# HKUST-Aerial-Robotics/A-LOAM

Measured on AMD Instinct MI355X. Metric: HDL-64 scans/sec (whole node), higher is better.
Workload: dtype f32 features / f64 solve

## Files before the change

a-loam_amd/csrc/aloam_capi.hip:

```cpp
#include <algorithm>
#include <cstdio>
#include <cstdlib>
#include <cstring>

#include "capi_internal.hpp"

namespace aloam {

hipEvent_t prof_event(aloam_ctx* c) {
  if (!c->prof_free.empty()) { hipEvent_t e = c->prof_free.back(); c->prof_free.pop_back(); return e; }
  Event e;
  (void)hipEventCreate(&e.h);
  c->prof_events.push_back(std::move(e));
  return c->prof_events.back();
}

int stage_ints(aloam_ctx* c, const int* src, int n, int* dst) {
  const int ns = c->h_nin_slot;
  c->h_nin_slot = (ns + 1) % kNinSlots;
  int* slot = c->h_nin.get() + (size_t)ns * c->B;
  if (c->nin_used[ns]) HIP_TRY(c, hipEventSynchronize(c->nin_done[ns]));
  std::memcpy(slot, src, sizeof(int) * n);
  HIP_TRY(c, hipMemcpyAsync(dst, slot, sizeof(int) * n, hipMemcpyHostToDevice, c->stream));
  HIP_TRY(c, hipEventRecord(c->nin_done[ns], c->stream));
  c->nin_used[ns] = true;
  return ALOAM_OK;
}

int stage_mask(aloam_ctx* c, DevBuf<int>& dst, const int** out) {
  *out = nullptr;
  if (c->all_active) return ALOAM_OK;
  if (!dst && dmalloc(c, dst, c->B)) return ALOAM_E_HIP;
  if (const int rc = stage_ints(c, c->active.data(), c->B, dst.get())) return rc;
  *out = dst.get();
  return ALOAM_OK;
}

int check_seq(aloam_ctx* c, int seq) {
  if (!c) return ALOAM_E_ARG;
  if (seq < 0 || seq >= c->B) { c->err = "sequence index out of range"; return ALOAM_E_ARG; }
  return ALOAM_OK;
}

int require_stage(aloam_ctx* c, int stage) {
  if (c->stages & stage) return ALOAM_OK;
  c->err = std::string("this context was created without ") +
           (stage == ALOAM_STAGE_REGISTRATION ? "ALOAM_STAGE_REGISTRATION" : stage == ALOAM_STAGE_ODOMETRY ? "ALOAM_STAGE_ODOMETRY" : "ALOAM_STAGE_MAPPING");
  return ALOAM_E_STATE;
}

int check_ids(aloam_ctx* c, const int* ids, int n) {
  if (n < 0 || n > c->B || (n > 0 && !ids)) { c->err = "bad sequence list"; return ALOAM_E_ARG; }
  std::vector<char> seen(c->B, 0);
  for (int i = 0; i < n; ++i) {
    if (ids[i] < 0 || ids[i] >= c->B || seen[ids[i]]) { c->err = "sequence index out of range or repeated"; return ALOAM_E_ARG; }
    seen[ids[i]] = 1;
  }
  return ALOAM_OK;
}

int queue_reset(aloam_ctx* c, const int* seqs, int n) {
  if (n == 0) return ALOAM_OK;
  if (!c->d_reset_ids && dmalloc(c, c->d_reset_ids, c->B)) return ALOAM_E_HIP;
  if (const int rc = stage_ints(c, seqs, n, c->d_reset_ids.get())) return rc;
  ResetArgs r{};
  r.seqs = c->d_reset_ids.get(); r.n = n; r.R = c->R;
  r.meta = c->d_meta.get(); r.ringstart = c->d_ringstart.get(); r.state = c->d_state.get();
  r.edges = c->d_edges.get(); r.planes = c->d_planes.get();
  for (int k = 0; k < 2; ++k) r.grid_flags[k] = c->d_grid_flags[k].get();
  for (int k = 0; k < 2; ++k) { r.less_sharp[k] = c->d_less_sharp[k].get(); r.less_flat[k] = c->d_less_flat[k].get(); }
  r.cap = c->cap;
  if (c->map_on) { r.mapseq = c->d_mapseq.get(); r.cubes = c->d_cubes.get(); r.addcnt = c->d_addcnt.get(); r.live = c->d_map_live.get(); r.grid_sig = c->d_grid_sig.get(); }
  launch_reset_sequences(r, c->stream);
  HIP_TRY(c, hipGetLastError());
  for (int i = 0; i < n; ++i) { c->parity[seqs[i]] = 0; c->inited[seqs[i]] = 0; c->needs_odom[seqs[i]] = 0; c->map_err_seen[seqs[i]] = 0; clear_scorable(c, seqs[i]); place_sweep_dropped(c, seqs[i]); }
  for (int i = 0; i < n; ++i) if (const int rc = mark_window_stale(c, seqs[i])) return rc;
  return ALOAM_OK;
}

}

namespace {

void prof_resolve(aloam_ctx* c) {
  for (ProfRec& r : c->prof_pending) {
    float ms = 0.f;
    (void)hipEventSynchronize(r.e1);
    (void)hipEventElapsedTime(&ms, r.e0, r.e1);
    c->prof_ms[r.kernel] += ms;
    c->prof_launches[r.kernel] += 1;
    c->prof_free.push_back(r.e0);
    c->prof_free.push_back(r.e1);
  }
  c->prof_pending.clear();
}

}

extern "C" {

void aloam_default_config(aloam_config* cfg) {
  cfg->n_scans = 64;
  cfg->min_range = 5.0f;
  cfg->ring_from_field = 0;
  cfg->batch = 1;
  cfg->max_points = 140000;
  cfg->max_ring_points = 4107;
  cfg->device = 0;
  cfg->lm_max_iterations = 4;
  cfg->outer_iterations = 2;
  cfg->distortion = 0;
}

int aloam_create(const aloam_config* cfg, aloam_ctx** out) { return aloam_create_stages(cfg, ALOAM_STAGE_ALL, out); }

int aloam_create_stages(const aloam_config* cfg, int stages, aloam_ctx** out) {
  if (!cfg || !out) return ALOAM_E_ARG;
  *out = nullptr;
  aloam_ctx* c = new aloam_ctx();
  c->cfg = *cfg;
  c->stages = stages;
  { const char* e = std::getenv("ALOAM_DEBUG_SYNC"); c->debug_sync = e && e[0] == '1'; }
  *out = c;
  if ((stages & ~ALOAM_STAGE_ALL) || !(stages & ALOAM_STAGE_ALL)) { c->err = "stages must be a non-empty combination of ALOAM_STAGE_*"; return ALOAM_E_ARG; }
  if (cfg->batch < 1 || cfg->max_points < 32 || cfg->max_points > 400000 || cfg->lm_max_iterations < 0 || cfg->outer_iterations < 1 ||
      cfg->outer_iterations > 64) { c->err = "bad configuration value"; return ALOAM_E_ARG; }
  if (!cfg->ring_from_field && cfg->n_scans != 16 && cfg->n_scans != 32 && cfg->n_scans != 64) {
    c->err = "only support velodyne with 16, 32 or 64 scan line (or ring_from_field)";
    return ALOAM_E_SCAN_LINES;
  }
  if (cfg->n_scans < 1 || cfg->n_scans > kMaxRings) { c->err = "n_scans out of range"; return ALOAM_E_ARG; }
  if (cfg->max_ring_points < 17 || cfg->max_ring_points > 4107) { c->err = "max_ring_points must be in [17, 4107]"; return ALOAM_E_ARG; }
  int ndev = 0;
  if (hipGetDeviceCount(&ndev) != hipSuccess || ndev <= 0) { c->err = "no HIP device available (this library has no CPU fallback)"; return ALOAM_E_HIP; }
  if (cfg->device < 0 || cfg->device >= ndev) { c->err = "device ordinal out of range"; return ALOAM_E_ARG; }
  DeviceScope device_scope(c);
  HIP_TRY(c, hipStreamCreateWithFlags(&c->stream.h, hipStreamNonBlocking));
  HIP_TRY(c, hipStreamCreateWithFlags(&c->copy_stream.h, hipStreamNonBlocking));
  for (int k = 0; k < 2; ++k) {
    HIP_TRY(c, hipEventCreateWithFlags(&c->in_copied[k].h, hipEventDisableTiming));
    HIP_TRY(c, hipEventCreateWithFlags(&c->in_consumed[k].h, hipEventDisableTiming));
  }
  c->B = cfg->batch; c->max_points = cfg->max_points; c->R = cfg->n_scans;
  c->active.assign(c->B, 1); c->parity.assign(c->B, 0); c->inited.assign(c->B, 0); c->needs_odom.assign(c->B, 0); c->frozen.assign(c->B, 0); c->scorable.assign(c->B, 0); c->pl_has_sweep.assign(c->B, 0); c->pl_desc_valid.assign(c->B, 0);
  c->map_err_seen.assign(c->B, 0);
  c->cap = cfg->max_points + (((cfg->max_points / 32 + 15) & ~15) + 16);
  { const char* e = std::getenv("ALOAM_GRAPH_MAX_BATCH"); c->use_graph = c->B <= (e ? std::atoi(e) : 0); }
  c->NB = (c->cap + kBlockPts - 1) / kBlockPts;
  c->npad = cfg->max_ring_points <= 2059 ? 2048 : 4096;
  const size_t B = c->B, cap = c->cap, R = c->R, NB = c->NB;
  int rc = 0;
  { int* p = nullptr; HIP_TRY(c, hipHostMalloc((void**)&p, sizeof(int) * B * kNinSlots, hipHostMallocDefault)); c->h_nin.reset(p); }
  for (Event& e : c->nin_done) HIP_TRY(c, hipEventCreateWithFlags(&e.h, hipEventDisableTiming));
  const bool reg = stages & ALOAM_STAGE_REGISTRATION, odo = stages & ALOAM_STAGE_ODOMETRY, map = stages & ALOAM_STAGE_MAPPING;
  c->grid_H[0] = R > 64 ? 8192 : 4096;
  c->grid_H[1] = c->max_points > 160000 ? 32768 : 16384;
  if ((rc = dmalloc(c, c->d_nin, B))) return rc;
  if ((rc = dmalloc(c, c->d_meta, B))) return rc;
  if ((rc = dmalloc(c, c->d_state, B))) return rc;
  if ((rc = dmalloc(c, c->d_cloud, B * cap))) return rc;
  if ((rc = dmalloc(c, c->d_exp_cnt, B * ALOAM_EXPORT_MAX_IDS))) return rc;
  if ((rc = dmalloc(c, c->d_exp_chunk, B * ALOAM_EXPORT_MAX_IDS + 1))) return rc;
  if ((rc = dmalloc(c, c->d_exp_off, B * ALOAM_EXPORT_MAX_IDS + 1))) return rc;
  { int cus = 0; if (hipDeviceGetAttribute(&cus, hipDeviceAttributeMultiprocessorCount, cfg->device) == hipSuccess && cus > 0) c->gather_blocks = 8 * cus; }
  if (reg) {
    c->slab = c->npad + 16;
    if ((rc = dmalloc(c, c->d_slabs, B * R * (size_t)c->slab))) return rc;
    if ((rc = dmalloc(c, c->d_front_lb, B * NB * (size_t)kFrontSlots))) return rc;
    if ((rc = dmalloc(c, c->d_front_ticket, B))) return rc;
    if ((rc = dmalloc(c, c->d_ringstart, B * (R + 1)))) return rc;
    if ((rc = dmalloc(c, c->d_curv, B * cap))) return rc;
    if ((rc = dmalloc(c, c->d_label, B * cap))) return rc;
    if ((rc = dmalloc(c, c->d_lookback, B * 4 * R))) return rc;
    if ((rc = dmalloc(c, c->d_ring_ticket, B))) return rc;
  }
  if (reg || odo) {
    if ((rc = dmalloc(c, c->d_sharp, B * R * kSharpPerRing))) return rc;
    if ((rc = dmalloc(c, c->d_flat, B * R * kFlatPerRing))) return rc;
  }
  for (int k = 0; k < 2; ++k) {
    if (!(odo || (k == 0 && reg) || (k == 1 && map))) continue;
    if ((rc = dmalloc(c, c->d_less_sharp[k], B * R * kLessSharpPerRing))) return rc;
    if ((rc = dmalloc(c, c->d_less_flat[k], B * cap))) return rc;
  }
  if (odo) {
    for (int k = 0; k < 2; ++k) {
      const size_t per = k == 0 ? R * kLessSharpPerRing : cap;
      if ((rc = dmalloc(c, c->d_grid_sorted3[k], B * per))) return rc;
      if ((rc = dmalloc(c, c->d_grid_sorted2[k], B * per))) return rc;
      if ((rc = dmalloc(c, c->d_grid_start3[k], B * (c->grid_H[k] + 1)))) return rc;
      if ((rc = dmalloc(c, c->d_grid_start2[k], B * (c->grid_H[k] + 1)))) return rc;
      if ((rc = dmalloc(c, c->d_grid_sorted3c[k], B * per))) return rc;
      if ((rc = dmalloc(c, c->d_grid_start3c[k], B * (c->grid_H[k] + 1)))) return rc;
      if ((rc = dmalloc(c, c->d_grid_flags[k], B * 4))) return rc;
      if ((rc = dmalloc(c, c->d_grid_walk[k], B * 2 * (R + 8)))) return rc;
    }
    if ((rc = dmalloc(c, c->d_edges, B * R * kSharpPerRing))) return rc;
    if ((rc = dmalloc(c, c->d_planes, B * R * kFlatPerRing))) return rc;
    if ((rc = dmalloc(c, c->d_sel_sharp, B * R * kSharpPerRing))) return rc;
    if ((rc = dmalloc(c, c->d_sel_flat, B * R * kFlatPerRing))) return rc;
    if ((rc = prepare_build_grids(c->grid_H[1]))) { c->err = "k_build_grids: dynamic LDS size rejected"; return ALOAM_E_HIP; }
  }
  std::vector<OdomState> init(B);
  std::memset(init.data(), 0, sizeof(OdomState) * B);
  for (size_t b = 0; b < B; ++b) { init[b].para_q[3] = 1.0; init[b].q_w[3] = 1.0; }
  HIP_TRY(c, hipMemcpyAsync(c->d_state.get(), init.data(), sizeof(OdomState) * B, hipMemcpyHostToDevice, c->stream));
  HIP_TRY(c, hipStreamSynchronize(c->stream));
  return ALOAM_OK;
}

void aloam_destroy(aloam_ctx* c) {
  DeviceScope device_scope(c);
  if (!c) return;
  if (c->stream) (void)hipStreamSynchronize(c->stream);
  if (c->copy_stream) (void)hipStreamSynchronize(c->copy_stream);
  prof_resolve(c);
  delete c;
}

const char* aloam_last_error(const aloam_ctx* c) { return c ? c->err.c_str() : "null context"; }
void* aloam_stream(aloam_ctx* c) { return c ? (void*)c->stream : nullptr; }

int aloam_synchronize(aloam_ctx* c) {
  DeviceScope device_scope(c);
  if (!c) return ALOAM_E_ARG;
  HIP_TRY(c, hipStreamSynchronize(c->stream));
  std::vector<SeqMeta> m(c->B);
  HIP_TRY(c, hipMemcpy(m.data(), c->d_meta.get(), sizeof(SeqMeta) * c->B, hipMemcpyDeviceToHost));
  for (int b = 0; b < c->B; ++b) {
    if (m[b].err & kErrEmpty) { c->err = "sequence " + std::to_string(b) + ": no point survives the NaN / minimum-range filter"; return ALOAM_E_EMPTY; }
    if (m[b].err & (kErrRingCap | kErrPointCap)) { c->err = "sequence " + std::to_string(b) + ": a ring exceeds max_ring_points or the scan exceeds max_points"; return ALOAM_E_CAPACITY; }
    if (m[b].err & kErrInternal) { c->err = "sequence " + std::to_string(b) + ": internal error, a ring workgroup of k_ring_features never published its counts (look-back wait timed out)"; return ALOAM_E_HIP; }
  }
  if (c->map_on) {
    std::vector<MapSeq> ms(c->B);
    int vc[4] = {0, 0, 0, 0};
    HIP_TRY(c, hipMemcpy(ms.data(), c->d_mapseq.get(), sizeof(MapSeq) * c->B, hipMemcpyDeviceToHost));
    HIP_TRY(c, hipMemcpy(vc, c->d_vox_counters.get(), sizeof(vc), hipMemcpyDeviceToHost));
    long long fresh_pool = 0;
    int first_seq = -1;
    for (int b = 0; b < c->B; ++b) {
      const long long n = ms[b].err_steps + ((ms[b].err & kMapErrPool) ? 1 : 0);
      if (n > c->map_err_seen[b]) { fresh_pool += n - c->map_err_seen[b]; if (first_seq < 0) first_seq = b; }
      c->map_err_seen[b] = n;
    }
    const long long vox = vc[3] + (vc[1] ? 1 : 0), fresh_vox = vox > c->map_err_reported ? vox - c->map_err_reported : 0;
    c->map_err_reported = vox;
    if (fresh_pool + fresh_vox > 0) {
      c->err = "mapping, since the last aloam_synchronize:";
      if (fresh_pool) c->err += " " + std::to_string(fresh_pool) + " (sequence, step) pair(s) ran out of map pool (first: sequence " + std::to_string(first_seq) + ")";
      if (fresh_vox) c->err += std::string(fresh_pool ? " and" : "") + " " + std::to_string(fresh_vox) + " step(s) ran out of voxel-filter scratch";
      c->err += "; the points that did not fit were not inserted (raise pool_points)";
      return ALOAM_E_CAPACITY;
    }
    long long fresh_spill = 0;
    if (const int rc = spill_dropped_since(c, &fresh_spill)) return rc;
    if (fresh_spill > 0) {
      c->err = "map spill full: " + std::to_string(fresh_spill) + " tile(s) dropped since the last aloam_synchronize (drain more often or raise max_tiles / max_points)";
      return ALOAM_E_CAPACITY;
    }
    if (c->d_rl_bad) {
      int bad = 0;
      HIP_TRY(c, hipMemcpy(&bad, c->d_rl_bad.get(), sizeof(bad), hipMemcpyDeviceToHost));
      const long long fresh = bad - c->rl_bad_reported;
      c->rl_bad_reported = bad;
      if (fresh > 0) {
        c->err = "aloam_apply_map_corrections, since the last aloam_synchronize: " + std::to_string(fresh) + " choice(s) outside 0 .. K-1; those sequences were left untouched";
        return ALOAM_E_ARG;
      }
    }
  }
  return ALOAM_OK;
}

int aloam_set_active(aloam_ctx* c, const int* active) {
  DeviceScope device_scope(c);
  if (!c) return ALOAM_E_ARG;
  std::vector<int> m(c->B, 1);
  if (active) for (int b = 0; b < c->B; ++b) m[b] = active[b] != 0 ? 1 : 0;
  if (c->reg_pending && (c->stages & ALOAM_STAGE_REGISTRATION) && m != c->reg_active) {
    c->err = "the mask may not change between a registration and the odometry step that consumes it";
    return ALOAM_E_STATE;
  }
  c->all_active = std::find(m.begin(), m.end(), 0) == m.end();
  c->active = std::move(m);
  return ALOAM_OK;
}

int aloam_reset_sequences(aloam_ctx* c, const int* seqs, int n) {
  DeviceScope device_scope(c);
  if (!c) return ALOAM_E_ARG;
  if (const int rc = check_ids(c, seqs, n)) return rc;
  return queue_reset(c, seqs, n);
}

int aloam_profile_enable(aloam_ctx* c, int on) {
  DeviceScope device_scope(c);
  if (!c) return ALOAM_E_ARG;
  HIP_TRY(c, hipStreamSynchronize(c->stream));
  prof_resolve(c);
  if (on) { for (int k = 0; k < K_COUNT; ++k) { c->prof_ms[k] = 0; c->prof_launches[k] = 0; } }
  c->prof_on = on != 0;
  return ALOAM_OK;
}
int aloam_profile_kernel_count(void) { return K_COUNT; }
const char* aloam_profile_kernel_name(int k) { return (k >= 0 && k < K_COUNT) ? kKernelNames[k] : ""; }

int aloam_profile_get(aloam_ctx* c, int kernel, double* total_ms, long long* launches, double* algorithmic_bytes) {
  DeviceScope device_scope(c);
  if (!c || kernel < 0 || kernel >= K_COUNT) return ALOAM_E_ARG;
  HIP_TRY(c, hipStreamSynchronize(c->stream));
  prof_resolve(c);
  if (total_ms) *total_ms = c->prof_ms[kernel];
  if (launches) *launches = c->prof_launches[kernel];
  if (algorithmic_bytes && kernel == K_EXPORT) {
    long long total = 0;
    HIP_TRY(c, hipMemcpy(&total, c->d_exp_off.get() + c->exp_last_segs, sizeof(total), hipMemcpyDeviceToHost));
    *algorithmic_bytes = 32.0 * total + 16.0 * c->exp_last_segs;
  } else if (algorithmic_bytes && (kernel == K_SAVE || kernel == K_LOAD)) {
    long long units = 0;
    if (kernel == K_SAVE && c->d_ck_uoff) HIP_TRY(c, hipMemcpy(&units, c->d_ck_uoff.get() + c->ck_save_n, sizeof(units), hipMemcpyDeviceToHost));
    *algorithmic_bytes = 2.0 * (kernel == K_SAVE ? 16.0 * units : (double)c->ck_load_bytes);
  } else if (algorithmic_bytes) {
    std::vector<SeqMeta> m(c->B);
    HIP_TRY(c, hipMemcpy(m.data(), c->d_meta.get(), sizeof(SeqMeta) * c->B, hipMemcpyDeviceToHost));
    std::vector<MapSeq> ms(c->map_on ? c->B : 0);
    if (c->map_on) HIP_TRY(c, hipMemcpy(ms.data(), c->d_mapseq.get(), sizeof(MapSeq) * c->B, hipMemcpyDeviceToHost));
    double bytes = 0;
    for (int b = 0; b < c->B; ++b) {
      const double Nin = m[b].n_in, N = m[b].n_cloud, Fc = m[b].n_sharp, Lc = m[b].n_less_sharp, Fs = m[b].n_flat, Ls = m[b].n_less_flat;
      const double Lcl = m[b].n_corner_last, Lsl = m[b].n_surf_last;
      switch (kernel) {
        case K_FIND_ENDS: bytes += 2 * 256 * 16; break;
        case K_FRONT: bytes += 16 * Nin + 16 * N + 16.0 * (c->R + 1) * ((Nin + kBlockPts - 1) / kBlockPts); break;
        case K_RING_STARTS: bytes += 12.0 * c->R; break;
        case K_DENSE_CLOUD: bytes += 32 * N; break;
        case K_RING_FEATURES: bytes += 16 * N + (c->debug_arrays ? 5 * N : 0) + 16 * (Fc + Lc + Fs + Ls); break;
        case K_BUILD_GRIDS: bytes += 16 * (Lcl + Lsl) + 48 * (Lcl + Lsl) + 12.0 * (c->grid_H[0] + c->grid_H[1]); break;
        case K_TRANSFORM: bytes += 32 * (Fc + Fs); break;
        case K_ASSOC_CORNER: bytes += 16 * (Fc + Lcl) + 48 * Fc; break;
        case K_ASSOC_PLANE: bytes += 16 * (Fs + Lsl) + 64 * Fs; break;
        case K_SOLVE: bytes += 9.0 * (48 * Fc + 64 * Fs); break;
        default: break;
      }
      if (c->map_on && kernel >= K_MAP_BEGIN) {
        const double Sc = ms[b].n_stack[0], Ss = ms[b].n_stack[1], Mc = ms[b].from_total[0], Ms = ms[b].from_total[1];
        const double Fc = ms[b].factor_num[1][0], Fs = ms[b].factor_num[1][1];
        switch (kernel) {
          case K_MAP_BEGIN: bytes += 2.0 * kMapValidMax * sizeof(CubeDesc) + sizeof(MapSeq); break;
          case K_MAP_VOXEL_STACK: bytes += 16 * (Lcl + Lsl) + 16 * (Sc + Ss); break;
          case K_MAP_GRID: bytes += 32 * (Mc + Ms) + 16.0 * c->map.H; break;
          case K_MAP_ASSOC: bytes += 16 * (Sc + Ss) + 80 * (Sc + Ss) + sizeof(MapEdgeRec) * Sc + sizeof(MapNormRec) * Ss; break;
          case K_MAP_SOLVE: bytes += 9.0 * (sizeof(MapEdgeRec) * Fc + sizeof(MapNormRec) * Fs); break;
          case K_MAP_INSERT: bytes += 32 * (Sc + Ss); break;
          case K_MAP_VOXEL_CUBES: bytes += 32 * (Mc + Ms + Sc + Ss); break;
          case K_MAP_REGISTER: bytes += 32 * N; break;
          default: break;
        }
      }
    }
    if (c->map_on && kernel == K_SCORE) {
      bytes = 64.0 * c->rl_last_K + 32.0 * c->rl_last_seqs.size() * c->rl_last_K;
      for (const int b : c->rl_last_seqs) bytes += 16.0 * (ms[b].n_stack[0] + ms[b].n_stack[1]) + 16.0 * (ms[b].from_total[0] + ms[b].from_total[1]) + 8.0 * c->map.H;
    }
    if (kernel == K_APPLY) bytes = c->rl_apply_n * (4.0 + 4.0 + 64.0 + 56.0);
    *algorithmic_bytes = bytes;
  }
  return ALOAM_OK;
}

}
```

a-loam_amd/csrc/aloam_device.hpp:

```cpp
#pragma once
#include <hip/hip_runtime.h>
#include <stdint.h>
#include "aloam_atan.hpp"

namespace aloam {

constexpr int kFrontSlots = 128 + 8;
constexpr int kBlockPts = 1024;
constexpr int kMaxRings = 128;
constexpr int kSectors = 6;
constexpr int kSharpPerSector = 2;
constexpr int kLessSharpPerSector = 20;
constexpr int kFlatPerSector = 4;
constexpr int kSharpPerRing = kSectors * kSharpPerSector;
constexpr int kLessSharpPerRing = kSectors * kLessSharpPerSector;
constexpr int kFlatPerRing = kSectors * kFlatPerSector;
constexpr int kNnTile = 1024;

enum ErrBits { kErrEmpty = 1, kErrRingCap = 2, kErrPointCap = 4, kErrInternal = 8 };

struct alignas(16) SeqMeta {
  int n_in;
  int first_kept, last_kept;
  int half_idx;
  float start_ori, end_ori;
  int n_cloud;
  int err;
  int n_sharp, n_less_sharp, n_flat, n_less_flat;
  int n_corner_last, n_surf_last;
  int parity;
  int pad1;
};

struct alignas(16) OdomState {
  double para_q[4];
  double para_t[3];
  double q_w[4];
  double t_w[3];
  int corner_corr[2], plane_corr[2];
  int lm_iterations[2], lm_successful[2];
  double initial_cost[2], final_cost[2];
  int termination[2];
  int inited;
  int pad;
};

enum SeqBits { kSeqActive = 1, kSeqSolve = 2, kSeqMapGrow = 4 };
__device__ __forceinline__ bool seq_idle(const int* active, int b, int bit = kSeqActive) { return active && !(active[b] & bit); }

struct EdgeRec { float cp[3], a[3], b[3]; int valid; int pad[2]; };
struct PlaneRec { float cp[3], j[3], l[3], m[3]; int valid; int pad[3]; };

struct RegArgs {
  const char* in;
  long long seq_stride;
  int pt_stride;
  int B, cap, R, NB;
  int ring_from_field;
  float min_range;
  SeqMeta* meta;
  float4* slabs;
  int slab;
  unsigned long long* front_lb;
  int* front_ticket;
  int* ringstart;
  float4* cloud;
  float* curv;
  int8_t* label;
  unsigned long long* lookback;
  unsigned epoch;
  int* ring_ticket;
  int store_debug;
  float4* sharp;
  float4* less_sharp[2];
  float4* flat;
  float4* less_flat[2];
  const int* active;
};

struct OdomArgs {
  int B, cap, R;
  SeqMeta* meta;
  OdomState* state;
  const float4* sharp;
  const float4* flat;
  const float4* less_sharp[2];
  const float4* less_flat[2];
  const int* active;
  float4* grid_sorted3[2];
  float4* grid_sorted2[2];
  int* grid_start3[2];
  int* grid_start2[2];
  float4* grid_sorted3c[2];
  int* grid_start3c[2];
  int* grid_flags[2];
  int* grid_walk[2];
  int grid_H_corner, grid_H_surf;
  float4* sel_sharp;
  float4* sel_flat;
  EdgeRec* edges;
  PlaneRec* planes;
  int outer;
  int last_outer;
  int lm_max_iterations;
  int distortion;
};

template <typename T>
__device__ __forceinline__ T* row_of(T* const (&buf)[2], int k, int b, long long per) { return (k ? buf[1] : buf[0]) + b * per; }
__device__ __forceinline__ const float4* corner_last(const OdomArgs& a, int b, int parity) { return row_of(a.less_sharp, parity ^ 1, b, (long long)a.R * kLessSharpPerRing); }
__device__ __forceinline__ const float4* surf_last(const OdomArgs& a, int b, int parity) { return row_of(a.less_flat, parity ^ 1, b, (long long)a.cap); }

struct GridView {
  int H;
  float4 *sorted3, *sorted2, *sorted3c;
  int *start3, *start2, *start3c, *flags, *walk;
};
__device__ __forceinline__ GridView grid_view(const OdomArgs& a, int b, int which) {
  GridView g;
  g.H = which == 0 ? a.grid_H_corner : a.grid_H_surf;
  const long long per = which == 0 ? (long long)a.R * kLessSharpPerRing : (long long)a.cap;
  g.sorted3 = a.grid_sorted3[which] + b * per;
  g.sorted2 = a.grid_sorted2[which] + b * per;
  g.start3 = a.grid_start3[which] + (long long)b * (g.H + 1);
  g.start2 = a.grid_start2[which] + (long long)b * (g.H + 1);
  g.sorted3c = a.grid_sorted3c[which] + b * per;
  g.start3c = a.grid_start3c[which] + (long long)b * (g.H + 1);
  g.flags = a.grid_flags[which] + b * 4;
  g.walk = a.grid_walk[which] + (long long)b * 2 * (a.R + 8);
  return g;
}

__device__ __forceinline__ float4 load_point(const char* base, long long i, int stride) {
  const float* p = reinterpret_cast<const float*>(base + i * (long long)stride);
  if ((stride & 15) == 0) return *reinterpret_cast<const float4*>(p);
  if (stride == 12) return make_float4(p[0], p[1], p[2], 0.f);
  return make_float4(p[0], p[1], p[2], p[3]);
}

__device__ __forceinline__ bool point_kept(const float4& p, float thres) {
  if (!(isfinite(p.x) && isfinite(p.y) && isfinite(p.z))) return false;
  const float r2 = p.x * p.x + p.y * p.y + p.z * p.z;
  return !(r2 < thres * thres);
}

__device__ __forceinline__ double shfl_down_f64(double v, int d) {
  int lo = __double2loint(v), hi = __double2hiint(v);
  lo = __shfl_down(lo, d, 64);
  hi = __shfl_down(hi, d, 64);
  return __hiloint2double(hi, lo);
}

template <int D>
__device__ __forceinline__ unsigned xor_lane_u32(unsigned v, int lane) {
  if constexpr (D == 1) return (unsigned)__builtin_amdgcn_mov_dpp((int)v, 0xB1, 0xF, 0xF, true);
  else if constexpr (D == 2) return (unsigned)__builtin_amdgcn_mov_dpp((int)v, 0x4E, 0xF, 0xF, true);
  else {
    const unsigned up = (unsigned)__builtin_amdgcn_mov_dpp((int)v, 0x100 + D, 0xF, 0xF, true);
    const unsigned dn = (unsigned)__builtin_amdgcn_mov_dpp((int)v, 0x110 + D, 0xF, 0xF, true);
    return (lane & D) ? dn : up;
  }
}
template <int D, bool MAX>
__device__ __forceinline__ unsigned long long row_step_u64(unsigned long long v, int lane) {
  const unsigned lo = xor_lane_u32<D>((unsigned)v, lane), hi = xor_lane_u32<D>((unsigned)(v >> 32), lane);
  const unsigned long long o = ((unsigned long long)hi << 32) | lo;
  return MAX ? (o > v ? o : v) : (o < v ? o : v);
}
template <bool MAX>
__device__ __forceinline__ unsigned long long wave_extreme_u64(unsigned long long v, int lane) {
  v = row_step_u64<1, MAX>(v, lane);
  v = row_step_u64<2, MAX>(v, lane);
  v = row_step_u64<4, MAX>(v, lane);
  v = row_step_u64<8, MAX>(v, lane);
  unsigned long long best = MAX ? 0ull : ~0ull;
#pragma unroll
  for (int q = 0; q < 4; ++q) {
    const unsigned lo = (unsigned)__builtin_amdgcn_readlane((int)(unsigned)v, 16 * q), hi = (unsigned)__builtin_amdgcn_readlane((int)(unsigned)(v >> 32), 16 * q);
    const unsigned long long o = ((unsigned long long)hi << 32) | lo;
    best = MAX ? (o > best ? o : best) : (o < best ? o : best);
  }
  return best;
}

template <bool MAX>
__device__ __forceinline__ unsigned wave_reduce_u32(unsigned v) {
  constexpr int identity = MAX ? 0 : -1;
  auto op = [](unsigned a, unsigned b) { return MAX ? (a > b ? a : b) : (a < b ? a : b); };
  v = op(v, (unsigned)__builtin_amdgcn_update_dpp(identity, (int)v, 0x111, 0xF, 0xF, false));
  v = op(v, (unsigned)__builtin_amdgcn_update_dpp(identity, (int)v, 0x112, 0xF, 0xF, false));
  v = op(v, (unsigned)__builtin_amdgcn_update_dpp(identity, (int)v, 0x114, 0xF, 0xF, false));
  v = op(v, (unsigned)__builtin_amdgcn_update_dpp(identity, (int)v, 0x118, 0xF, 0xF, false));
  v = op(v, (unsigned)__builtin_amdgcn_update_dpp(identity, (int)v, 0x142, 0xA, 0xF, false));
  v = op(v, (unsigned)__builtin_amdgcn_update_dpp(identity, (int)v, 0x143, 0xC, 0xF, false));
  return (unsigned)__builtin_amdgcn_readlane((int)v, 63);
}
__device__ __forceinline__ unsigned long long wave_min_packed(unsigned long long v) {
  const unsigned hi = (unsigned)(v >> 32), lo = (unsigned)v;
  const unsigned mh = wave_reduce_u32<false>(hi);
  const unsigned long long tie = __ballot(hi == mh);
  unsigned ml;
  if (__popcll(tie) == 1) ml = (unsigned)__builtin_amdgcn_readlane((int)lo, __ffsll((long long)tie) - 1);
  else ml = wave_reduce_u32<false>(hi == mh ? lo : 0xffffffffu);
  return ((unsigned long long)mh << 32) | ml;
}

template <bool MAX>
__device__ __forceinline__ int wave_scan_i32(int v) {
  constexpr int identity = MAX ? (int)0x80000000 : 0;
  auto op = [](int a, int b) { return MAX ? (a > b ? a : b) : a + b; };
  v = op(v, __builtin_amdgcn_update_dpp(identity, v, 0x111, 0xF, 0xF, false));
  v = op(v, __builtin_amdgcn_update_dpp(identity, v, 0x112, 0xF, 0xF, false));
  v = op(v, __builtin_amdgcn_update_dpp(identity, v, 0x114, 0xF, 0xF, false));
  v = op(v, __builtin_amdgcn_update_dpp(identity, v, 0x118, 0xF, 0xF, false));
  v = op(v, __builtin_amdgcn_update_dpp(identity, v, 0x142, 0xA, 0xF, false));
  v = op(v, __builtin_amdgcn_update_dpp(identity, v, 0x143, 0xC, 0xF, false));
  return v;
}


__device__ __forceinline__ int pow2ceil(int v) { int p = 1; while (p < v) p <<= 1; return p; }
template <typename K>
__device__ __forceinline__ void bitonic_cx(K& a, K& b) {
  const K lo = a < b ? a : b, hi = a < b ? b : a;
  a = lo; b = hi;
}
template <bool FIRST, typename K>
__device__ __forceinline__ void bitonic_groups_of_eight(K* keys, int n, int tid) {
  constexpr K kInf = (K)~(K)0;
  for (int g = tid * 8; g < n; g += 2048) {
    K v[8];
#pragma unroll
    for (int u = 0; u < 8; ++u) v[u] = g + u < n ? keys[g + u] : kInf;
    if (FIRST) {
#pragma unroll
      for (int b = 0; b < 8; b += 2) bitonic_cx(v[b], v[b + 1]);
#pragma unroll
      for (int b = 0; b < 8; b += 4) { bitonic_cx(v[b], v[b + 3]); bitonic_cx(v[b + 1], v[b + 2]); }
#pragma unroll
      for (int b = 0; b < 8; b += 2) bitonic_cx(v[b], v[b + 1]);
#pragma unroll
      for (int o = 0; o < 4; ++o) bitonic_cx(v[o], v[7 - o]);
    } else {
#pragma unroll
      for (int o = 0; o < 4; ++o) bitonic_cx(v[o], v[o + 4]);
    }
#pragma unroll
    for (int b = 0; b < 8; b += 4) { bitonic_cx(v[b], v[b + 2]); bitonic_cx(v[b + 1], v[b + 3]); }
#pragma unroll
    for (int b = 0; b < 8; b += 2) bitonic_cx(v[b], v[b + 1]);
#pragma unroll
    for (int u = 0; u < 8; ++u) if (g + u < n) keys[g + u] = v[u];
  }
  __syncthreads();
}
template <typename K>
__device__ __forceinline__ void bitonic_sort_keys(K* keys, int n, int tid) {
  const int npad = pow2ceil(n);
  bitonic_groups_of_eight<true, K>(keys, n, tid);
  for (int k = 16; k <= npad; k <<= 1) {
    const int hk = k >> 1;
    for (int t = tid; t < (npad >> 1); t += 256) {
      const int base = (t / hk) * k, off = t & (hk - 1);
      const int i = base + off, l = base + (k - 1 - off);
      if (l < n) {
        const K x = keys[i], y = keys[l];
        if (x > y) { keys[i] = y; keys[l] = x; }
      }
    }
    __syncthreads();
    for (int j = k >> 2; j > 4; j >>= 1) {
      for (int t = tid; t < (npad >> 1); t += 256) {
        const int i = ((t & ~(j - 1)) << 1) | (t & (j - 1));
        const int l = i + j;
        if (l < n) {
          const K x = keys[i], y = keys[l];
          if (x > y) { keys[i] = y; keys[l] = x; }
        }
      }
      __syncthreads();
    }
    bitonic_groups_of_eight<false, K>(keys, n, tid);
  }
}
__device__ __forceinline__ void bitonic_sort_u64(unsigned long long* keys, int n, int tid) { bitonic_sort_keys<unsigned long long>(keys, n, tid); }


}
```

a-loam_amd/csrc/capi_internal.hpp:

```cpp
#pragma once
#include <hip/hip_runtime.h>

#include <cstdio>
#include <memory>
#include <string>
#include <utility>
#include <vector>

#include "../../include/aloam_mi355x.h"
#include "aloam_device.hpp"
#include "atlas_kernels.hpp"
#include "checkpoint_kernels.hpp"
#include "export_kernels.hpp"
#include "mapping_kernels.hpp"
#include "odometry_kernels.hpp"
#include "places_kernels.hpp"
#include "registration_kernels.hpp"
#include "relocalize_kernels.hpp"

using namespace aloam;

namespace aloam {
enum KernelId { K_FIND_ENDS = 0, K_FRONT, K_RING_STARTS, K_DENSE_CLOUD, K_RING_FEATURES, K_BUILD_GRIDS, K_TRANSFORM, K_ASSOC_CORNER,
                K_ASSOC_PLANE, K_SOLVE, K_ADVANCE, K_MAP_BEGIN, K_MAP_VOXEL_STACK, K_MAP_GRID, K_MAP_ASSOC, K_MAP_SOLVE, K_MAP_INSERT,
                K_MAP_VOXEL_CUBES, K_MAP_REGISTER, K_EXPORT, K_SAVE, K_LOAD, K_SCORE, K_APPLY, K_COUNT };
const char* const kKernelNames[] = {"k_find_ends", "k_front", "k_ring_starts", "k_dense_cloud", "k_ring_features",
                                    "k_build_grids", "k_transform_queries", "k_associate[corner]", "k_associate[plane]",
                                    "k_solve", "k_advance", "map_begin", "map_voxel[stacks]", "map_grid", "map_associate", "map_solve",
                                    "map_insert", "map_voxel[cubes]", "map_register", "export_clouds", "save_sequences",
                                    "load_sequences", "score_corrections", "apply_corrections"};
static_assert(sizeof(kKernelNames) / sizeof(kKernelNames[0]) == K_COUNT, "one name per KernelId, in the same order");
struct ProfRec { int kernel; hipEvent_t e0, e1; };
constexpr int kNinSlots = 8;

struct DeviceFree { void operator()(void* p) const { (void)hipFree(p); } };
struct PinnedFree { void operator()(const volatile void* p) const { (void)hipHostFree(const_cast<void*>(p)); } };
template <typename T> using DevBuf = std::unique_ptr<T[], DeviceFree>;
template <typename T> using PinnedBuf = std::unique_ptr<T[], PinnedFree>;
template <typename H, hipError_t (*Destroy)(H)>
struct Handle {
  H h = nullptr;
  Handle() = default;
  Handle(Handle&& o) noexcept : h(std::exchange(o.h, nullptr)) {}
  ~Handle() { reset(); }
  void reset() { if (h) (void)Destroy(h); h = nullptr; }
  operator H() const { return h; }
};
using Stream = Handle<hipStream_t, hipStreamDestroy>;
using Event = Handle<hipEvent_t, hipEventDestroy>;
using GraphExec = Handle<hipGraphExec_t, hipGraphExecDestroy>;

template <typename T>
hipError_t dalloc(DevBuf<T>& p, size_t count) {
  T* raw = nullptr;
  const hipError_t e = hipMalloc((void**)&raw, count * sizeof(T));
  p.reset(raw);
  return e;
}

struct MapPool {
  int points = 0, H = 0;
  int cube_levels = 0, tile_cap = 0, tile_bound = 0;
  long long key_cap = 0;
  DevBuf<float4> pool[2], grid_sorted[2], voxtmp;
  DevBuf<int> grid_start[2], tile_seg, tile_heads, tile_pref;
  DevBuf<unsigned long long> keys[2];
};
}

struct aloam_ctx {
  Stream stream, copy_stream;
  Event in_copied[2], in_consumed[2], nin_done[kNinSlots], map_step_done[4];
  std::vector<Event> prof_events;
  GraphExec odom_graph[2];
  aloam_config cfg{};
  int stages = ALOAM_STAGE_ALL;
  int B = 0, cap = 0, R = 0, NB = 0, npad = 0;
  int max_points = 0;
  std::string err;
  DevBuf<char> d_in[2]; size_t d_in_bytes[2] = {0, 0};
  int in_slot = 0;
  bool in_used[2] = {false, false};
  DevBuf<int> d_nin;
  PinnedBuf<int> h_nin; int h_nin_slot = 0;
  bool nin_used[kNinSlots] = {};
  std::vector<int> active;
  bool all_active = true;
  std::vector<int> reg_active;
  bool reg_pending = false;
  const int* reg_mask = nullptr;
  std::vector<int> parity, inited;
  std::vector<char> needs_odom;
  std::vector<char> frozen;
  bool any_frozen = false;
  DevBuf<int> d_mask_reg, d_mask_odo, d_mask_map, d_reset_ids;
  DevBuf<SeqMeta> d_meta;
  DevBuf<float4> d_slabs; int slab = 0;
  DevBuf<unsigned long long> d_front_lb; DevBuf<int> d_front_ticket;
  bool dense_valid = true;
  DevBuf<int> d_ringstart;
  DevBuf<float4> d_cloud; DevBuf<float> d_curv; DevBuf<int8_t> d_label;
  DevBuf<unsigned long long> d_lookback; unsigned reg_epoch = 0;
  DevBuf<int> d_ring_ticket;
  bool debug_arrays = false;
  DevBuf<float4> d_sharp, d_flat;
  DevBuf<float4> d_less_sharp[2], d_less_flat[2];
  DevBuf<OdomState> d_state;
  DevBuf<float4> d_grid_sorted3[2], d_grid_sorted2[2];
  DevBuf<int> d_grid_start3[2], d_grid_start2[2];
  DevBuf<float4> d_grid_sorted3c[2];
  DevBuf<int> d_grid_start3c[2];
  DevBuf<int> d_grid_flags[2], d_grid_walk[2];
  int grid_H[2] = {4096, 16384};
  DevBuf<EdgeRec> d_edges; DevBuf<PlaneRec> d_planes;
  DevBuf<float4> d_sel_sharp, d_sel_flat;
  bool map_on = false;
  long long map_err_reported = 0;
  std::vector<long long> map_err_seen;
  float map_line_res = 0.4f, map_plane_res = 0.8f;
  int map_levels = 0, map_stack_tile_bound = 0, map_nsegs_max = 0;
  MapPool map;
  int map_pool_limit = 1 << 26;
  int map_growths = 0;
  long long map_steps = 0;
  int nin_max = 0;
  int inject_max = 0;
  PinnedBuf<volatile int> h_map_report;
  int* d_map_report_host = nullptr;
  DevBuf<int> d_map_report, d_map_live;
  DevBuf<MapSeq> d_mapseq; DevBuf<CubeDesc> d_cubes; DevBuf<int> d_maptab;
  DevBuf<MapGridSig> d_grid_sig;
  DevBuf<float4> d_stack[2], d_stack_world[2]; DevBuf<int> d_stack_cube[2];
  DevBuf<int> d_addcnt, d_cursor, d_compact_flag;
  DevBuf<MapEdgeRec> d_medges; DevBuf<MapNormRec> d_mnorms; DevBuf<float4> d_registered, d_knn;
  DevBuf<int> d_vox_lists;
  DevBuf<int> d_rec_tiles; int rec_tiles_corner = 0, rec_tiles_per_seq = 0;
  DevBuf<VoxSeg> d_segs; DevBuf<int> d_vox_counters, d_bbox;
  DevBuf<int> d_exp_cnt, d_exp_chunk; DevBuf<long long> d_exp_off;
  DevBuf<int> d_exp_pref[2];
  int exp_last_segs = 0;
  int gather_blocks = 2048;
  DevBuf<float4> d_exp_tmp; long long exp_tmp_cap = 0;
  DevBuf<long long> d_exp_tmp_off;
  DevBuf<int> d_ck_seqs, d_ck_info, d_ck_units, d_ck_chunk, d_ck_pref; DevBuf<long long> d_ck_uoff;
  PinnedBuf<char> h_ck; char* d_ck_host = nullptr;
  DevBuf<char> d_ck_load;
  DevBuf<char> d_ck_stage; size_t ck_stage_bytes = 0;
  int ck_save_n = 0; long long ck_load_bytes = 0;
  std::vector<char> scorable;
  DevBuf<int> d_rl_seqs, d_rl_bad;
  DevBuf<ScorePartial> d_rl_part; long long rl_part_cap = 0;
  DevBuf<aloam_map_correction> d_rl_cand; long long rl_cand_cap = 0;
  long long rl_bad_reported = 0;
  std::vector<int> rl_last_seqs; int rl_last_K = 0;
  int rl_apply_n = 0;
  bool spill_on = false;
  int spill_max_tiles = 0, spill_max_points = 0;
  DevBuf<aloam_map_tile> d_sp_tiles; DevBuf<float4> d_sp_points;
  DevBuf<int> d_sp_counters;
  DevBuf<int> d_sp_seqs, d_sp_cnt, d_sp_chunk; DevBuf<long long> d_sp_off;
  bool atlas_on = false;
  std::vector<char> attached; bool any_attached = false;
  DevBuf<int> d_at_attached, d_at_stale;
  DevBuf<AtlasEntry> d_at_dir[2]; int at_dir_mask[2] = {0, 0};
  DevBuf<float4> d_at_points[2];
  long long at_info[12] = {0};
  long long spill_dropped_reported = 0;
  bool places_on = false;
  int pl_capacity = 0, pl_count = 0;
  float pl_max_range = 80.f, pl_height = 2.f;
  std::vector<char> pl_has_sweep, pl_desc_valid;
  DevBuf<PlaceDesc> d_pl_desc;
  DevBuf<aloam_place> d_pl_store;
  DevBuf<float> d_pl_unit; DevBuf<unsigned long long> d_pl_masks;
  DevBuf<int> d_pl_seqs, d_pl_wanted, d_pl_lo, d_pl_hi;
  DevBuf<int2> d_pl_pairs; long long pl_pairs_cap = 0;
  int sum_order = 0;
  bool use_graph = false;
  bool have_features = false;
  bool prof_on = false;
  bool debug_sync = false;
  std::vector<ProfRec> prof_pending;
  std::vector<hipEvent_t> prof_free;
  double prof_ms[K_COUNT] = {0};
  long long prof_launches[K_COUNT] = {0};
};

#define HIP_TRY(ctx, expr)                                                                                   \
  do {                                                                                                       \
    hipError_t e__ = (expr);                                                                                 \
    if (e__ != hipSuccess) {                                                                                 \
      (ctx)->err = std::string(#expr) + ": " + hipGetErrorString(e__);                                       \
      return ALOAM_E_HIP;                                                                                    \
    }                                                                                                        \
  } while (0)

namespace aloam {

template <typename T>
int dmalloc(aloam_ctx* c, DevBuf<T>& p, size_t count) {
  HIP_TRY(c, dalloc(p, count));
  HIP_TRY(c, hipMemsetAsync(p.get(), 0, count * sizeof(T), c->stream));
  return ALOAM_OK;
}

hipEvent_t prof_event(aloam_ctx* c);
struct ProfScope {
  aloam_ctx* c; int k; hipEvent_t e0 = nullptr;
  ProfScope(aloam_ctx* c_, int k_) : c(c_), k(k_) {
    if (c->prof_on) { e0 = prof_event(c); (void)hipEventRecord(e0, c->stream); }
  }
  ~ProfScope() {
    if (c->prof_on) { hipEvent_t e1 = prof_event(c); (void)hipEventRecord(e1, c->stream); c->prof_pending.push_back({k, e0, e1}); }
    if (c->debug_sync) {
      const hipError_t e = hipStreamSynchronize(c->stream);
      std::fprintf(stderr, "[aloam] %-22s %s\n", kKernelNames[k], e == hipSuccess ? "ok" : hipGetErrorString(e));
    }
  }
};
struct DeviceScope {
  int prev = -1;
  explicit DeviceScope(const aloam_ctx* c) {
    int cur = -1;
    if (c && hipGetDevice(&cur) == hipSuccess && cur != c->cfg.device && hipSetDevice(c->cfg.device) == hipSuccess) prev = cur;
  }
  ~DeviceScope() { if (prev >= 0) (void)hipSetDevice(prev); }
  DeviceScope(const DeviceScope&) = delete;
  DeviceScope& operator=(const DeviceScope&) = delete;
};

template <typename T>
int read_seq(aloam_ctx* c, const T* dev, T* out) {
  HIP_TRY(c, hipStreamSynchronize(c->stream));
  HIP_TRY(c, hipMemcpy(out, dev, sizeof(T), hipMemcpyDeviceToHost));
  return ALOAM_OK;
}

template <typename T, typename Edit>
int edit_seq(aloam_ctx* c, T* dev, Edit edit) {
  T v;
  if (const int rc = read_seq(c, dev, &v)) return rc;
  edit(v);
  HIP_TRY(c, hipMemcpy(dev, &v, sizeof(T), hipMemcpyHostToDevice));
  return ALOAM_OK;
}

template <typename T, typename N>
int grow_scratch(aloam_ctx* c, DevBuf<T>& p, N& have, N need) {
  if (have >= need) return ALOAM_OK;
  have = 0;
  p.reset();
  HIP_TRY(c, dalloc(p, (size_t)need));
  have = need;
  return ALOAM_OK;
}

inline float4* cloud_row(const aloam_ctx* c, const ExportSrc& s, int seq) {
  const int r = s.sel == kSelFixed ? 0 : s.sel == kSelCurrent ? c->parity[seq] : 1 - c->parity[seq];
  return s.base[r] ? const_cast<float4*>(s.base[r]) + (size_t)seq * s.stride : nullptr;
}

int stage_ints(aloam_ctx* c, const int* src, int n, int* dst);
int stage_mask(aloam_ctx* c, DevBuf<int>& dst, const int** out);
int check_seq(aloam_ctx* c, int seq);
int require_stage(aloam_ctx* c, int stage);
int check_ids(aloam_ctx* c, const int* ids, int n);
int queue_reset(aloam_ctx* c, const int* seqs, int n);
int ensure_dense(aloam_ctx* c);
long long cloud_desc(const aloam_ctx* c, int id, ExportSrc* s);
int find_cloud(aloam_ctx* c, int seq, int id, const float4** ptr, int* n);
inline void clear_scorable(aloam_ctx* c, int seq) { c->scorable[seq] = 0; }
int grow_map_pool(aloam_ctx* c, long long want, bool clamp);
void queue_map_spill(aloam_ctx* c, const int* mask);
int spill_dropped_since(aloam_ctx* c, long long* fresh);
int mark_window_stale(aloam_ctx* c, int seq);
int atlas_step_check(aloam_ctx* c);
bool queue_atlas_window(aloam_ctx* c, const int* mask);
inline void place_sweep_registered(aloam_ctx* c, int seq) { c->pl_has_sweep[seq] = 1; c->pl_desc_valid[seq] = 0; }
inline void place_sweep_dropped(aloam_ctx* c, int seq) { c->pl_has_sweep[seq] = 0; c->pl_desc_valid[seq] = 0; }
VoxArgs vox_args(aloam_ctx* c, int n_segs, int levels);
enum CallerMem { kMemPageable, kMemDevice, kMemPinned, kMemManaged, kMemOtherDevice };
CallerMem classify_pointer(const aloam_ctx* c, const void* p, void** dev);
int export_target(aloam_ctx* c, const void* p, size_t align, const char* what, void** out);
int get_cube_list(aloam_ctx* c, int seq, int which, float* out, int cap_points);

}
```

a-loam_amd/csrc/capi_odometry.hip:

```cpp
#include <algorithm>
#include <cstring>

#include "capi_internal.hpp"

namespace {

RegArgs reg_args(aloam_ctx* c, const void* d_scans, long long seq_stride, int pt_stride) {
  RegArgs a{};
  a.in = (const char*)d_scans; a.seq_stride = seq_stride; a.pt_stride = pt_stride;
  a.B = c->B; a.cap = c->cap; a.R = c->R; a.NB = c->NB;
  a.ring_from_field = c->cfg.ring_from_field; a.min_range = c->cfg.min_range;
  a.meta = c->d_meta.get(); a.slabs = c->d_slabs.get(); a.slab = c->slab; a.front_lb = c->d_front_lb.get(); a.front_ticket = c->d_front_ticket.get();
  a.ringstart = c->d_ringstart.get(); a.cloud = c->d_cloud.get(); a.curv = c->d_curv.get(); a.label = c->d_label.get();
  a.lookback = c->d_lookback.get(); a.epoch = c->reg_epoch; a.store_debug = c->debug_arrays ? 1 : 0; a.ring_ticket = c->d_ring_ticket.get();
  a.sharp = c->d_sharp.get(); a.flat = c->d_flat.get();
  for (int k = 0; k < 2; ++k) { a.less_sharp[k] = c->d_less_sharp[k].get(); a.less_flat[k] = c->d_less_flat[k].get(); }
  a.active = c->reg_mask;
  return a;
}

OdomArgs odom_args(aloam_ctx* c) {
  OdomArgs a{};
  a.B = c->B; a.cap = c->cap; a.R = c->R;
  a.meta = c->d_meta.get(); a.state = c->d_state.get();
  a.sharp = c->d_sharp.get(); a.flat = c->d_flat.get();
  for (int k = 0; k < 2; ++k) { a.less_sharp[k] = c->d_less_sharp[k].get(); a.less_flat[k] = c->d_less_flat[k].get(); }
  for (int k = 0; k < 2; ++k) {
    a.grid_sorted3[k] = c->d_grid_sorted3[k].get(); a.grid_sorted2[k] = c->d_grid_sorted2[k].get(); a.grid_start3[k] = c->d_grid_start3[k].get();
    a.grid_sorted3c[k] = c->d_grid_sorted3c[k].get(); a.grid_start3c[k] = c->d_grid_start3c[k].get();
    a.grid_start2[k] = c->d_grid_start2[k].get();
    a.grid_flags[k] = c->d_grid_flags[k].get(); a.grid_walk[k] = c->d_grid_walk[k].get();
  }
  a.grid_H_corner = c->grid_H[0]; a.grid_H_surf = c->grid_H[1];
  a.edges = c->d_edges.get(); a.planes = c->d_planes.get();
  a.sel_sharp = c->d_sel_sharp.get(); a.sel_flat = c->d_sel_flat.get();
  a.lm_max_iterations = c->cfg.lm_max_iterations;
  a.distortion = c->cfg.distortion != 0;
  return a;
}

int check_batch(aloam_ctx* c, const int* n_in, int stride_bytes) {
  if (const int rc = require_stage(c, ALOAM_STAGE_REGISTRATION)) return rc;
  if (stride_bytes < 12 || (stride_bytes & 3)) { c->err = "stride_bytes must be 12 (x, y, z only) or >= 16, and a multiple of 4"; return ALOAM_E_ARG; }
  if (stride_bytes == 12 && c->cfg.ring_from_field) { c->err = "ring_from_field needs the 4th float of every record: stride_bytes >= 16"; return ALOAM_E_ARG; }
  for (int b = 0; b < c->B; ++b) {
    if (n_in[b] < 0) { c->err = "negative point count"; return ALOAM_E_ARG; }
    if (n_in[b] > c->max_points) { c->err = "scan exceeds max_points"; return ALOAM_E_CAPACITY; }
  }
  return ALOAM_OK;
}

int register_launch(aloam_ctx* c, const void* d_scans, long long seq_stride, const int* n_in, int stride_bytes, int slot = -1, bool debug_arrays = true) {
  int rc = ALOAM_OK;
  if (!c->all_active && (rc = ensure_dense(c))) return rc;
  c->nin_max = 0;
  for (int b = 0; b < c->B; ++b) if (c->all_active || c->active[b]) c->nin_max = std::max(c->nin_max, n_in[b]);
  if ((rc = stage_ints(c, n_in, c->B, c->d_nin.get()))) return rc;
  if ((rc = stage_mask(c, c->d_mask_reg, &c->reg_mask))) return rc;
  if (c->stages & ALOAM_STAGE_ODOMETRY) { c->reg_active = c->active; c->reg_pending = true; }
  c->debug_arrays = debug_arrays || c->sum_order != 0;
  if (((++c->reg_epoch) & 0x7fffffffu) == 0) ++c->reg_epoch;
  const RegArgs a = reg_args(c, d_scans, seq_stride, stride_bytes);
  { ProfScope p(c, K_FIND_ENDS); launch_find_ends(a, c->d_nin.get(), c->stream); }
  { ProfScope p(c, K_FRONT); launch_front(a, c->stream); }
  { ProfScope p(c, K_RING_STARTS); launch_ring_starts(a, c->stream); }
  c->dense_valid = false;
  for (int b = 0; b < c->B; ++b) if (c->all_active || c->active[b]) place_sweep_registered(c, b);
  if (slot >= 0) { HIP_TRY(c, hipEventRecord(c->in_consumed[slot], c->stream)); c->in_used[slot] = true; }
  { ProfScope p(c, K_RING_FEATURES); launch_ring_features(a, c->npad, 0.2f, c->stream);
    if (c->sum_order) launch_less_flat_reference_order(reg_args(c, d_scans, seq_stride, stride_bytes), c->npad, 0.2f, c->stream); }
  HIP_TRY(c, hipGetLastError());
  c->have_features = true;
  return ALOAM_OK;
}

}

namespace aloam {

int ensure_dense(aloam_ctx* c) {
  if (c->dense_valid) return ALOAM_OK;
  { ProfScope p(c, K_DENSE_CLOUD); launch_dense_cloud(reg_args(c, nullptr, 0, 16), c->stream); }
  HIP_TRY(c, hipGetLastError());
  c->dense_valid = true;
  return ALOAM_OK;
}

long long cloud_desc(const aloam_ctx* c, int id, ExportSrc* s) {
  const int* meta = reinterpret_cast<const int*>(c->d_meta.get());
  const int* mseq = reinterpret_cast<const int*>(c->d_mapseq.get());
  const int meta_ints = sizeof(SeqMeta) / sizeof(int), map_ints = sizeof(MapSeq) / sizeof(int);
  const long long sharp = (long long)c->R * kSharpPerRing, flat = (long long)c->R * kFlatPerRing, feat = (long long)c->R * kLessSharpPerRing;
  const long long cap = c->cap, pts = c->max_points;
  long long capacity = 0;
  auto set = [&](const float4* b0, const float4* b1, long long stride, long long row_cap, const int* count, int count_stride, int sel) {
    *s = ExportSrc{{b0, b1}, stride, count, count_stride, sel, kExportPlain, 0};
    capacity = row_cap;
  };
#define META_FIELD(f) (meta + offsetof(SeqMeta, f) / sizeof(int)), meta_ints
  switch (id) {
    case ALOAM_CLOUD_FULL: set(c->d_cloud.get(), nullptr, cap, pts, META_FIELD(n_cloud), kSelFixed); break;
    case ALOAM_CLOUD_SHARP: set(c->d_sharp.get(), nullptr, sharp, sharp, META_FIELD(n_sharp), kSelFixed); break;
    case ALOAM_CLOUD_FLAT: set(c->d_flat.get(), nullptr, flat, flat, META_FIELD(n_flat), kSelFixed); break;
    case ALOAM_CLOUD_LESS_SHARP: set(c->d_less_sharp[0].get(), c->d_less_sharp[1].get(), feat, feat, META_FIELD(n_less_sharp), kSelCurrent); break;
    case ALOAM_CLOUD_LESS_FLAT: set(c->d_less_flat[0].get(), c->d_less_flat[1].get(), cap, pts, META_FIELD(n_less_flat), kSelCurrent); break;
    case ALOAM_CLOUD_CORNER_LAST: set(c->d_less_sharp[0].get(), c->d_less_sharp[1].get(), feat, feat, META_FIELD(n_corner_last), kSelLast); break;
    case ALOAM_CLOUD_SURF_LAST: set(c->d_less_flat[0].get(), c->d_less_flat[1].get(), cap, pts, META_FIELD(n_surf_last), kSelLast); break;
    case ALOAM_EXPORT_MAP + ALOAM_MAP_REGISTERED: set(c->d_registered.get(), nullptr, cap, pts, META_FIELD(n_cloud), kSelFixed); break;
    case ALOAM_EXPORT_MAP + ALOAM_MAP_CORNER_STACK: set(c->d_stack[0].get(), nullptr, feat, feat, mseq + offsetof(MapSeq, n_stack) / sizeof(int), map_ints, kSelFixed); break;
    case ALOAM_EXPORT_MAP + ALOAM_MAP_SURF_STACK: set(c->d_stack[1].get(), nullptr, cap, pts, mseq + offsetof(MapSeq, n_stack) / sizeof(int) + 1, map_ints, kSelFixed); break;
    default: break;
  }
#undef META_FIELD
  return capacity;
}

int find_cloud(aloam_ctx* c, int seq, int id, const float4** ptr, int* n) {
  int rc = check_seq(c, seq);
  if (rc || (id == ALOAM_CLOUD_FULL && (rc = ensure_dense(c)))) return rc;
  ExportSrc s;
  if (!cloud_desc(c, id, &s)) { c->err = "unknown cloud id"; return ALOAM_E_ARG; }
  if ((rc = read_seq(c, s.count + (size_t)seq * s.count_stride, n))) return rc;
  if (!(*ptr = cloud_row(c, s, seq))) { c->err = "this context holds no such cloud (see aloam_create_stages)"; return ALOAM_E_STATE; }
  return ALOAM_OK;
}

}

extern "C" {

int aloam_scan_register_device(aloam_ctx* c, const void* d_scans, long long seq_stride_bytes, const int* n_in, int stride_bytes) {
  DeviceScope device_scope(c);
  if (!c || !d_scans || !n_in) return ALOAM_E_ARG;
  if (const int rc = check_batch(c, n_in, stride_bytes)) return rc;
  return register_launch(c, d_scans, seq_stride_bytes, n_in, stride_bytes);
}

static int acquire_slab(aloam_ctx* c, size_t need, int* slot_out) {
  const int s = c->in_slot;
  c->in_slot ^= 1;
  if (c->in_used[s]) HIP_TRY(c, hipEventSynchronize(c->in_consumed[s]));
  if (const int rc = grow_scratch(c, c->d_in[s], c->d_in_bytes[s], need)) return rc;
  *slot_out = s;
  return ALOAM_OK;
}

int aloam_scan_register(aloam_ctx* c, const void* const* scans, const int* n_in, int stride_bytes) {
  DeviceScope device_scope(c);
  if (!c || !scans || !n_in) return ALOAM_E_ARG;
  int rc = check_batch(c, n_in, stride_bytes);
  if (rc) return rc;
  const size_t seq_stride = (size_t)c->cap * stride_bytes;
  int slot = 0;
  if ((rc = acquire_slab(c, seq_stride * c->B, &slot))) return rc;
  char* d_in = c->d_in[slot].get();
  for (int b = 0; b < c->B; ++b)
    if (n_in[b] > 0) HIP_TRY(c, hipMemcpyAsync(d_in + b * seq_stride, scans[b], (size_t)n_in[b] * stride_bytes, hipMemcpyHostToDevice, c->stream));
  if ((rc = register_launch(c, d_in, (long long)seq_stride, n_in, stride_bytes, slot))) return rc;
  HIP_TRY(c, hipStreamSynchronize(c->stream));
  return ALOAM_OK;
}

static int stage_and_register(aloam_ctx* c, const void* h_scans, long long seq_stride_bytes, const int* n_in, int stride_bytes, bool debug_arrays) {
  if (!c || !h_scans || !n_in) return ALOAM_E_ARG;
  int rc = check_batch(c, n_in, stride_bytes);
  if (rc) return rc;
  if (seq_stride_bytes < 0) { c->err = "bad stride"; return ALOAM_E_ARG; }
  const size_t row = (size_t)*std::max_element(n_in, n_in + c->B) * stride_bytes;
  if (c->B > 1 && (size_t)seq_stride_bytes < row) { c->err = "seq_stride_bytes smaller than a scan"; return ALOAM_E_ARG; }
  const size_t d_seq_stride = (size_t)c->cap * stride_bytes;
  int slot = 0;
  if ((rc = acquire_slab(c, d_seq_stride * c->B, &slot))) return rc;
  char* d_in = c->d_in[slot].get();
  if (row > 0) {
    if (c->B > 1) HIP_TRY(c, hipMemcpy2DAsync(d_in, d_seq_stride, h_scans, (size_t)seq_stride_bytes, row, (size_t)c->B - 1, hipMemcpyHostToDevice, c->copy_stream));
    const size_t last = (size_t)n_in[c->B - 1] * stride_bytes;
    if (last > 0) HIP_TRY(c, hipMemcpyAsync(d_in + (size_t)(c->B - 1) * d_seq_stride, (const char*)h_scans + (size_t)(c->B - 1) * (size_t)seq_stride_bytes, last, hipMemcpyHostToDevice, c->copy_stream));
  }
  HIP_TRY(c, hipEventRecord(c->in_copied[slot], c->copy_stream));
  HIP_TRY(c, hipStreamWaitEvent(c->stream, c->in_copied[slot], 0));
  return register_launch(c, d_in, (long long)d_seq_stride, n_in, stride_bytes, slot, debug_arrays);
}

int aloam_scan_register_host(aloam_ctx* c, const void* h_scans, long long seq_stride_bytes, const int* n_in, int stride_bytes) {
  DeviceScope device_scope(c);
  return stage_and_register(c, h_scans, seq_stride_bytes, n_in, stride_bytes, true);
}

int aloam_process_host(aloam_ctx* c, const void* h_scans, long long seq_stride_bytes, const int* n_in, int stride_bytes) {
  DeviceScope device_scope(c);
  const int rc = stage_and_register(c, h_scans, seq_stride_bytes, n_in, stride_bytes, false);
  if (rc) return rc;
  return aloam_odometry_step(c);
}

int aloam_input_consumed(aloam_ctx* c) {
  DeviceScope device_scope(c);
  if (!c) return ALOAM_E_ARG;
  for (int s = 0; s < 2; ++s) if (c->in_used[s]) HIP_TRY(c, hipEventSynchronize(c->in_consumed[s]));
  return ALOAM_OK;
}

int aloam_odometry_step(aloam_ctx* c) {
  DeviceScope device_scope(c);
  if (!c) return ALOAM_E_ARG;
  if (const int rc = require_stage(c, ALOAM_STAGE_ODOMETRY)) return rc;
  if (!c->have_features) { c->err = "aloam_odometry_step before any features were registered / set"; return ALOAM_E_STATE; }
  std::vector<int> bits(c->B);
  bool any_solve = false, all_solve = true;
  for (int b = 0; b < c->B; ++b) {
    const bool on = c->all_active || c->active[b];
    bits[b] = on ? (kSeqActive | (c->inited[b] ? kSeqSolve : 0)) : 0;
    any_solve |= (bits[b] & kSeqSolve) != 0;
    all_solve &= (bits[b] & kSeqSolve) != 0;
  }
  const int* mask = nullptr;
  if (!all_solve && (any_solve || !c->all_active)) {
    if (!c->d_mask_odo && dmalloc(c, c->d_mask_odo, c->B)) return ALOAM_E_HIP;
    if (const int rc = stage_ints(c, bits.data(), c->B, c->d_mask_odo.get())) return rc;
    mask = c->d_mask_odo.get();
  }
  auto launch_all = [&]() {
    OdomArgs a = odom_args(c);
    a.active = mask;
    { ProfScope p(c, K_BUILD_GRIDS); launch_build_grids(a, c->stream); }
    for (int outer = 0; outer < c->cfg.outer_iterations; ++outer) {
      a.outer = outer;
      a.last_outer = outer == c->cfg.outer_iterations - 1;
      { ProfScope p(c, K_TRANSFORM); launch_transform_queries(a, c->stream); }
      { ProfScope p(c, K_ASSOC_CORNER); launch_associate(a, false, c->stream); }
      { ProfScope p(c, K_ASSOC_PLANE); launch_associate(a, true, c->stream); }
      { ProfScope p(c, K_SOLVE); launch_solve(a, c->stream); }
    }
    { ProfScope p(c, K_ADVANCE); launch_advance(a, c->stream); }
  };
  if (!any_solve) {
    OdomArgs a = odom_args(c);
    a.active = mask;
    { ProfScope p(c, K_ADVANCE); launch_advance(a, c->stream); }
  } else if (c->use_graph && !c->prof_on && !c->debug_sync) {
    GraphExec& ge = c->odom_graph[mask ? 1 : 0];
    if (!ge) {
      hipGraph_t g = nullptr;
      hipError_t e = hipStreamBeginCapture(c->stream, hipStreamCaptureModeThreadLocal);
      if (e == hipSuccess) {
        launch_all();
        e = hipStreamEndCapture(c->stream, &g);
        if (e == hipSuccess) e = hipGraphInstantiate(&ge.h, g, nullptr, nullptr, 0);
        if (g) (void)hipGraphDestroy(g);
      }
      if (e != hipSuccess) {
        (void)hipGetLastError();
        ge.reset();
        c->use_graph = false;
      }
    }
    if (ge) HIP_TRY(c, hipGraphLaunch(ge, c->stream));
    else launch_all();
  } else {
    launch_all();
  }
  HIP_TRY(c, hipGetLastError());
  for (int b = 0; b < c->B; ++b) if (bits[b] & kSeqActive) { c->parity[b] ^= 1; c->inited[b] = 1; c->needs_odom[b] = 0; }
  c->reg_pending = false;
  return ALOAM_OK;
}

int aloam_process_device(aloam_ctx* c, const void* d_scans, long long seq_stride_bytes, const int* n_in, int stride_bytes) {
  DeviceScope device_scope(c);
  if (!c || !d_scans || !n_in) return ALOAM_E_ARG;
  int rc = check_batch(c, n_in, stride_bytes);
  if (rc || (rc = register_launch(c, d_scans, seq_stride_bytes, n_in, stride_bytes, -1, false))) return rc;
  return aloam_odometry_step(c);
}

int aloam_cloud_size(aloam_ctx* c, int seq, int which) {
  DeviceScope device_scope(c);
  const float4* p; int n;
  const int rc = find_cloud(c, seq, which < ALOAM_EXPORT_MAP ? which : -1, &p, &n);
  return rc ? rc : n;
}

int aloam_get_cloud(aloam_ctx* c, int seq, int which, float* out, int cap_points) {
  DeviceScope device_scope(c);
  const float4* p; int n;
  if (const int rc = find_cloud(c, seq, which < ALOAM_EXPORT_MAP ? which : -1, &p, &n)) return rc;
  const int k = n < cap_points ? n : cap_points;
  if (k > 0) HIP_TRY(c, hipMemcpy(out, p, sizeof(float4) * k, hipMemcpyDeviceToHost));
  return n;
}

int aloam_get_pose(aloam_ctx* c, int seq, double q_w[4], double t_w[3], double q_lc[4], double t_lc[3]) {
  DeviceScope device_scope(c);
  int rc = check_seq(c, seq);
  if (rc) return rc;
  OdomState s;
  if ((rc = read_seq(c, c->d_state.get() + seq, &s))) return rc;
  for (int k = 0; k < 4; ++k) { q_w[k] = s.q_w[k]; q_lc[k] = s.para_q[k]; }
  for (int k = 0; k < 3; ++k) { t_w[k] = s.t_w[k]; t_lc[k] = s.para_t[k]; }
  return ALOAM_OK;
}

int aloam_get_odom_stats(aloam_ctx* c, int seq, aloam_odom_stats* out) {
  DeviceScope device_scope(c);
  int rc = check_seq(c, seq);
  if (rc) return rc;
  OdomState s;
  if ((rc = read_seq(c, c->d_state.get() + seq, &s))) return rc;
  for (int k = 0; k < 2; ++k) {
    out->corner_corr[k] = s.corner_corr[k]; out->plane_corr[k] = s.plane_corr[k];
    out->lm_iterations[k] = s.lm_iterations[k]; out->lm_successful[k] = s.lm_successful[k];
    out->initial_cost[k] = s.initial_cost[k]; out->final_cost[k] = s.final_cost[k]; out->termination[k] = s.termination[k];
  }
  return ALOAM_OK;
}

int aloam_set_features(aloam_ctx* c, int seq, const float* sharp, int n_sharp, const float* less_sharp, int n_less_sharp,
                       const float* flat, int n_flat, const float* less_flat, int n_less_flat) {
  DeviceScope device_scope(c);
  int rc = check_seq(c, seq);
  if (rc) return rc;
  struct { int id, n; const float* pts; ExportSrc s; } in[4] = {
      {ALOAM_CLOUD_SHARP, n_sharp, sharp}, {ALOAM_CLOUD_LESS_SHARP, n_less_sharp, less_sharp}, {ALOAM_CLOUD_FLAT, n_flat, flat}, {ALOAM_CLOUD_LESS_FLAT, n_less_flat, less_flat}};
  for (auto& x : in) if (x.n < 0 || x.n > cloud_desc(c, x.id, &x.s)) { c->err = "feature cloud larger than the selection rules allow"; return ALOAM_E_CAPACITY; }
  for (auto& x : in) if (!cloud_row(c, x.s, seq)) { c->err = "this context has no feature buffers (created for the mapping stage only)"; return ALOAM_E_STATE; }
  c->inject_max = std::max(c->inject_max, std::max(n_less_sharp, n_less_flat));
  HIP_TRY(c, hipStreamSynchronize(c->stream));
  for (auto& x : in) if (x.n) HIP_TRY(c, hipMemcpy(cloud_row(c, x.s, seq), x.pts, sizeof(float4) * x.n, hipMemcpyHostToDevice));
  if ((rc = edit_seq(c, c->d_meta.get() + seq, [&](SeqMeta& m) { m.n_sharp = n_sharp; m.n_less_sharp = n_less_sharp; m.n_flat = n_flat; m.n_less_flat = n_less_flat; m.err = 0; }))) return rc;
  c->have_features = true;
  return ALOAM_OK;
}

int aloam_set_last(aloam_ctx* c, int seq, const float* corner_last, int n_corner, const float* surf_last, int n_surf) {
  DeviceScope device_scope(c);
  int rc = check_seq(c, seq);
  if (rc) return rc;
  struct { int id, n; const float* pts; ExportSrc s; } in[2] = {{ALOAM_CLOUD_CORNER_LAST, n_corner, corner_last}, {ALOAM_CLOUD_SURF_LAST, n_surf, surf_last}};
  for (auto& x : in) if (x.n < 0 || x.n > cloud_desc(c, x.id, &x.s)) { c->err = "last cloud too large"; return ALOAM_E_CAPACITY; }
  for (auto& x : in) if (!cloud_row(c, x.s, seq)) { c->err = "this context has no buffers for the last clouds (created for the registration stage only)"; return ALOAM_E_STATE; }
  c->inject_max = std::max(c->inject_max, std::max(n_corner, n_surf));
  HIP_TRY(c, hipStreamSynchronize(c->stream));
  for (auto& x : in) if (x.n) HIP_TRY(c, hipMemcpy(cloud_row(c, x.s, seq), x.pts, sizeof(float4) * x.n, hipMemcpyHostToDevice));
  return edit_seq(c, c->d_meta.get() + seq, [&](SeqMeta& m) { m.n_corner_last = n_corner; m.n_surf_last = n_surf; });
}

int aloam_set_state(aloam_ctx* c, int seq, const double para_q[4], const double para_t[3], const double q_w[4], const double t_w[3]) {
  DeviceScope device_scope(c);
  int rc = check_seq(c, seq);
  if (rc) return rc;
  return edit_seq(c, c->d_state.get() + seq, [&](OdomState& s) {
    for (int k = 0; k < 4; ++k) { s.para_q[k] = para_q[k]; s.q_w[k] = q_w[k]; }
    for (int k = 0; k < 3; ++k) { s.para_t[k] = para_t[k]; s.t_w[k] = t_w[k]; }
  });
}

int aloam_set_system_inited(aloam_ctx* c, int inited) {
  DeviceScope device_scope(c);
  if (!c) return ALOAM_E_ARG;
  std::fill(c->inited.begin(), c->inited.end(), inited != 0 ? 1 : 0);
  launch_set_inited(c->d_state.get(), c->B, inited != 0 ? 1 : 0, c->stream);
  HIP_TRY(c, hipGetLastError());
  return ALOAM_OK;
}

int aloam_set_full_cloud(aloam_ctx* c, int seq, const float* cloud, int n) {
  DeviceScope device_scope(c);
  int rc = check_seq(c, seq);
  if (rc) return rc;
  ExportSrc s;
  if (n < 0 || n > cloud_desc(c, ALOAM_CLOUD_FULL, &s)) { c->err = "cloud too large"; return ALOAM_E_CAPACITY; }
  if ((rc = ensure_dense(c))) return rc;
  HIP_TRY(c, hipStreamSynchronize(c->stream));
  if (n) HIP_TRY(c, hipMemcpy(cloud_row(c, s, seq), cloud, sizeof(float4) * n, hipMemcpyHostToDevice));
  return edit_seq(c, c->d_meta.get() + seq, [&](SeqMeta& m) { m.n_cloud = n; });
}

int aloam_get_ring_ranges(aloam_ctx* c, int seq, int* start, int* count) {
  DeviceScope device_scope(c);
  int rc = check_seq(c, seq);
  if (rc) return rc;
  if ((rc = require_stage(c, ALOAM_STAGE_REGISTRATION))) return rc;
  HIP_TRY(c, hipStreamSynchronize(c->stream));
  std::vector<int> rs(c->R + 1);
  HIP_TRY(c, hipMemcpy(rs.data(), c->d_ringstart.get() + (size_t)seq * (c->R + 1), sizeof(int) * (c->R + 1), hipMemcpyDeviceToHost));
  for (int r = 0; r < c->R; ++r) { start[r] = rs[r]; count[r] = rs[r + 1] - rs[r]; }
  return c->R;
}

int aloam_get_curvature(aloam_ctx* c, int seq, float* out, int cap) {
  DeviceScope device_scope(c);
  int rc = check_seq(c, seq);
  if (rc) return rc;
  if ((rc = require_stage(c, ALOAM_STAGE_REGISTRATION))) return rc;
  if (!c->debug_arrays) { c->err = "curvature is only kept by aloam_scan_register*; the throughput entries (aloam_process_*) skip it"; return ALOAM_E_STATE; }
  SeqMeta m;
  if ((rc = read_seq(c, c->d_meta.get() + seq, &m))) return rc;
  const int k = m.n_cloud < cap ? m.n_cloud : cap;
  if (k > 0) HIP_TRY(c, hipMemcpy(out, c->d_curv.get() + (size_t)seq * c->cap, sizeof(float) * k, hipMemcpyDeviceToHost));
  return m.n_cloud;
}

int aloam_get_labels(aloam_ctx* c, int seq, int* out, int cap) {
  DeviceScope device_scope(c);
  int rc = check_seq(c, seq);
  if (rc) return rc;
  if ((rc = require_stage(c, ALOAM_STAGE_REGISTRATION))) return rc;
  if (!c->debug_arrays) { c->err = "labels are only kept by aloam_scan_register*; the throughput entries (aloam_process_*) skip them"; return ALOAM_E_STATE; }
  SeqMeta m;
  if ((rc = read_seq(c, c->d_meta.get() + seq, &m))) return rc;
  const int k = m.n_cloud < cap ? m.n_cloud : cap;
  std::vector<int8_t> tmp(k > 0 ? k : 1);
  if (k > 0) HIP_TRY(c, hipMemcpy(tmp.data(), c->d_label.get() + (size_t)seq * c->cap, k, hipMemcpyDeviceToHost));
  for (int i = 0; i < k; ++i) out[i] = tmp[i];
  return m.n_cloud;
}

int aloam_get_last_cloud_order(aloam_ctx* c, int seq, int out[2]) {
  DeviceScope device_scope(c);
  int rc = check_seq(c, seq);
  if (rc) return rc;
  if (!c->d_grid_flags[0]) { c->err = "this context has no odometry stage"; return ALOAM_E_STATE; }
  HIP_TRY(c, hipStreamSynchronize(c->stream));
  for (int k = 0; k < 2; ++k) {
    int f[4];
    HIP_TRY(c, hipMemcpy(f, c->d_grid_flags[k].get() + (size_t)seq * 4, sizeof(f), hipMemcpyDeviceToHost));
    out[k] = f[0] ? -1 : f[1];
  }
  return ALOAM_OK;
}

int aloam_get_correspondences(aloam_ctx* c, int seq, float* edges, int cap_edges, int* n_edges, int* edge_query,
                              float* planes, int cap_planes, int* n_planes, int* plane_query) {
  DeviceScope device_scope(c);
  int rc = check_seq(c, seq);
  if (rc) return rc;
  SeqMeta m;
  if ((rc = read_seq(c, c->d_meta.get() + seq, &m))) return rc;
  std::vector<EdgeRec> E(m.n_sharp > 0 ? m.n_sharp : 1);
  std::vector<PlaneRec> P(m.n_flat > 0 ? m.n_flat : 1);
  if (m.n_sharp > 0) HIP_TRY(c, hipMemcpy(E.data(), c->d_edges.get() + (size_t)seq * c->R * kSharpPerRing, sizeof(EdgeRec) * m.n_sharp, hipMemcpyDeviceToHost));
  if (m.n_flat > 0) HIP_TRY(c, hipMemcpy(P.data(), c->d_planes.get() + (size_t)seq * c->R * kFlatPerRing, sizeof(PlaneRec) * m.n_flat, hipMemcpyDeviceToHost));
  int ne = 0, np = 0;
  for (int i = 0; i < m.n_sharp; ++i) {
    if (!E[i].valid) continue;
    if (ne < cap_edges) {
      float* o = edges + (size_t)ne * 9;
      for (int k = 0; k < 3; ++k) { o[k] = E[i].cp[k]; o[3 + k] = E[i].a[k]; o[6 + k] = E[i].b[k]; }
      if (edge_query) edge_query[ne] = i;
    }
    ++ne;
  }
  for (int i = 0; i < m.n_flat; ++i) {
    if (!P[i].valid) continue;
    if (np < cap_planes) {
      float* o = planes + (size_t)np * 12;
      for (int k = 0; k < 3; ++k) { o[k] = P[i].cp[k]; o[3 + k] = P[i].j[k]; o[6 + k] = P[i].l[k]; o[9 + k] = P[i].m[k]; }
      if (plane_query) plane_query[np] = i;
    }
    ++np;
  }
  *n_edges = ne;
  *n_planes = np;
  return ALOAM_OK;
}

}
```

a-loam_amd/csrc/mapping_kernels.hip:

```cpp
#include "mapping_kernels.hpp"

#include "lm_device.hpp"
#include "map_search_device.hpp"
#include "map_window_device.hpp"

namespace aloam {

namespace {

__device__ __forceinline__ int f2o(float f) { const int i = __float_as_int(f); return i >= 0 ? i : i ^ 0x7fffffff; }
__device__ __forceinline__ float o2f(int i) { return __int_as_float(i >= 0 ? i : i ^ 0x7fffffff); }

__device__ __forceinline__ float4 submap_point(const MapArgs& a, int b, int cls, const int* tab, int n_valid, int g) {
  const int* pref = tab + 80 + cls * 80;
  int lo = 0, hi = n_valid - 1;
  while (lo < hi) { const int mid = (lo + hi + 1) >> 1; if (pref[mid] <= g) lo = mid; else hi = mid - 1; }
  const CubeDesc d = cube_table(a, b, cls)[tab[lo]];
  return a.pool[cls][(long long)b * a.pool_cap + d.off + (g - pref[lo])];
}

}

__device__ __forceinline__ int compact_cap(int n, int mode) { return n <= 0 ? 0 : (mode == 1 ? n + n / 2 + 64 : n); }

// ... 1044 lines not shown
    return (lo << 8) + (d - pre[lo]);
  };
  for (int d0 = tid; d0 < n0; d0 += U * kMapSolveThreads) {
    MapEdgeRec e[U];
#pragma unroll
    for (int u = 0; u < U; ++u) { const int d = d0 + u * kMapSolveThreads; e[u] = E[locate(pre0, nt0, d < n0 ? d : d0)]; }
#pragma unroll
    for (int u = 0; u < U; ++u) if (d0 + u * kMapSolveThreads < n0) edge_term(e[u]);
  }
  auto norm_term = [&](const MapNormRec& p) {
    ++np;
    double rcp[3];
    quat_rotate(q, p.cp[0], p.cp[1], p.cp[2], rcp);
    const double r = (p.n[0] * (rcp[0] + t[0]) + p.n[1] * (rcp[1] + t[1]) + p.n[2] * (rcp[2] + t[2])) + p.d;
    double rho0, rho1;
    huber(r * r, &rho0, &rho1);
    acc[27] += 0.5 * rho0;
    if (WITH_JAC) {
      const double J[6] = {2.0 * (p.n[2] * rcp[1] - p.n[1] * rcp[2]), 2.0 * (p.n[0] * rcp[2] - p.n[2] * rcp[0]), 2.0 * (p.n[1] * rcp[0] - p.n[0] * rcp[1]),
                           p.n[0], p.n[1], p.n[2]};
      add_row(acc, J, r, rho1);
    }
  };
  for (int d0 = tid; d0 < n1; d0 += U * kMapSolveThreads) {
    MapNormRec pr[U];
#pragma unroll
    for (int u = 0; u < U; ++u) { const int d = d0 + u * kMapSolveThreads; pr[u] = P[locate(pre1, nt1, d < n1 ? d : d0)]; }
#pragma unroll
    for (int u = 0; u < U; ++u) if (d0 + u * kMapSolveThreads < n1) norm_term(pr[u]);
  }
  *n_edge = ne;
  *n_norm = np;
}

__global__ __launch_bounds__(kMapSolveThreads) void k_map_solve(MapArgs a, int iter, int last) {
  const int b = blockIdx.x, tid = threadIdx.x;
  __shared__ double s_red[(kMapSolveThreads / 64) * 28];
  extern __shared__ int s_pref[];
  if (seq_idle(a.active, b)) return;
  MapSeq& ms = a.seq[b];
  {
    const int nt0 = (ms.n_stack[0] + 255) >> 8, nt1 = (ms.n_stack[1] + 255) >> 8;
    const int* tc = a.rec_tiles + (long long)b * a.rec_tiles_per_seq;
    if (tid == 0) {
      int run = 0;
      for (int k = 0; k < nt0; ++k) { s_pref[k] = run; run += ms.gate ? tc[k] : 0; }
      s_pref[nt0] = run;
      run = 0;
      for (int k = 0; k < nt1; ++k) { s_pref[nt0 + 1 + k] = run; run += ms.gate ? tc[a.rec_tiles_corner + k] : 0; }
      s_pref[nt0 + 1 + nt1] = run;
    }
    __syncthreads();
  }
  double q[4] = {ms.par[0], ms.par[1], ms.par[2], ms.par[3]};
  double t[3] = {ms.par[4], ms.par[5], ms.par[6]};
  const LmResult lm = lm_solve_block<kMapSolveThreads / 64>([&](bool with_jac, const double* qq, const double* tt, double* acc, int* ne, int* np) {
    if (with_jac) map_evaluate<true>(a, b, s_pref, qq, tt, acc, ne, np); else map_evaluate<false>(a, b, s_pref, qq, tt, acc, ne, np);
  }, q, t, a.lm_max_iterations, s_red);
  if (tid == 0) {
    if (lm.termination == 5) {
      for (int k = 0; k < 4; ++k) q[k] = ms.par[k];
      for (int k = 0; k < 3; ++k) t[k] = ms.par[4 + k];
    }
    for (int k = 0; k < 4; ++k) ms.par[k] = q[k];
    for (int k = 0; k < 3; ++k) ms.par[4 + k] = t[k];
    ms.factor_num[iter][0] = lm.n_a;
    ms.factor_num[iter][1] = lm.n_b;
    ms.lm_iterations[iter] = lm.iterations;
    ms.lm_termination[iter] = lm.termination;
    if (last) {
      const double qo[4] = {ms.q_wodom[0], ms.q_wodom[1], ms.q_wodom[2], ms.q_wodom[3]};
      const double n2 = qo[0] * qo[0] + qo[1] * qo[1] + qo[2] * qo[2] + qo[3] * qo[3];
      const double inv[4] = {-qo[0] / n2, -qo[1] / n2, -qo[2] / n2, qo[3] / n2};
      double qm[4], rt[3];
      quat_mul(q, inv, qm);
      quat_rotate(qm, ms.t_wodom[0], ms.t_wodom[1], ms.t_wodom[2], rt);
      for (int k = 0; k < 4; ++k) ms.q_wmap_wodom[k] = qm[k];
      for (int k = 0; k < 3; ++k) ms.t_wmap_wodom[k] = t[k] - rt[k];
      ms.frame_count += 1;
    }
  }
}

__global__ __launch_bounds__(256) void k_map_cubeid(MapArgs a) {
  const int b = blockIdx.y, cls = blockIdx.z;
  if (seq_idle(a.active, b, kSeqMapGrow)) return;
  const MapSeq& ms = a.seq[b];
  const long long sb = (long long)b * (cls == 0 ? a.R * kLessSharpPerRing : a.cap);
  double par[7];
#pragma unroll
  for (int k = 0; k < 7; ++k) par[k] = ms.par[k];
  for (int i0 = blockIdx.x * 256; i0 < ms.n_stack[cls]; i0 += gridDim.x * 256) {
  const int i = i0 + threadIdx.x;
  const bool live = i < ms.n_stack[cls];
  const float4 w = associate_to_map(a.stack[cls][sb + (live ? i : 0)], par);
  const int ci = cube_coord((double)w.x, ms.cen[0]), cj = cube_coord((double)w.y, ms.cen[1]), ck = cube_coord((double)w.z, ms.cen[2]);
  int id = -1;
  if (live && ci >= 0 && ci < kMapW && cj >= 0 && cj < kMapH && ck >= 0 && ck < kMapD) id = ci + kMapW * cj + kMapW * kMapH * ck;
  unsigned long long todo = __ballot(id >= 0);
  while (todo) {
    const int leader = __ffsll((long long)todo) - 1;
    const int c = __shfl(id, leader, 64);
    const unsigned long long same = __ballot(id == c);
    if ((int)(threadIdx.x & 63) == leader) atomicAdd(&a.addcnt[((long long)b * 2 + cls) * kMapCubes + c], __popcll(same));
    todo &= ~same;
  }
  if (live) { a.stack_world[cls][sb + i] = w; a.stack_cube[cls][sb + i] = id; }
  }
}

__global__ __launch_bounds__(256) void k_map_reserve(MapArgs a) {
  const int b = blockIdx.x, cls = blockIdx.y, tid = threadIdx.x;
  if (seq_idle(a.active, b, kSeqMapGrow)) return;
  CubeDesc* T = cube_table(a, b, cls);
  int* add = a.addcnt + ((long long)b * 2 + cls) * kMapCubes;
  int* cur = a.cursor + ((long long)b * 2 + cls) * kMapCubes;
  float4* pool = a.pool[cls] + (long long)b * a.pool_cap;
  MapSeq& ms = a.seq[b];
  __shared__ int s_n;
  __shared__ int s_list[256][4];
  for (int base = 0; base < kMapCubes; base += 256) {
    if (tid == 0) s_n = 0;
    __syncthreads();
    const int c = base + tid;
    if (c < kMapCubes) {
      const int ad = add[c];
      if (ad > 0) {
        CubeDesc d = T[c];
        if (d.cnt + ad > d.cap) {
          int want = 2 * (d.cnt + ad);
          if (want < 256) want = 256;
          int off = atomicAdd(&ms.pool_used[cls], 0);
          for (;;) {
            if (off + want > a.pool_cap) { off = -1; break; }
            const int seen = atomicCAS(&ms.pool_used[cls], off, off + want);
            if (seen == off) break;
            off = seen;
          }
          if (off < 0) {
            atomicOr(&ms.err, kMapErrPool);
            add[c] = -1;
          } else {
            const int k = atomicAdd(&s_n, 1);
            s_list[k][0] = c; s_list[k][1] = d.off; s_list[k][2] = off; s_list[k][3] = d.cnt;
            d.off = off; d.cap = want;
            T[c] = d;
          }
        }
      }
    }
    __syncthreads();
    const int nmove = s_n;
    for (int k = 0; k < nmove; ++k)
      for (int i = tid; i < s_list[k][3]; i += 256) pool[s_list[k][2] + i] = pool[s_list[k][1] + i];
    __syncthreads();
    if (c < kMapCubes) {
      const int ad = add[c];
      cur[c] = T[c].cnt;
      if (ad > 0) T[c].cnt += ad;
    }
    __syncthreads();
  }
}

__global__ __launch_bounds__(64) void k_map_scatter(MapArgs a) {
  const int b = blockIdx.x, cls = blockIdx.y, lane = threadIdx.x;
  if (seq_idle(a.active, b, kSeqMapGrow)) return;
  const MapSeq& ms = a.seq[b];
  const int n = ms.n_stack[cls];
  const CubeDesc* T = cube_table(a, b, cls);
  int* add = a.addcnt + ((long long)b * 2 + cls) * kMapCubes;
  const int* cur = a.cursor + ((long long)b * 2 + cls) * kMapCubes;
  float4* pool = a.pool[cls] + (long long)b * a.pool_cap;
  const long long sb = (long long)b * (cls == 0 ? a.R * kLessSharpPerRing : a.cap);
  __shared__ int s_cur[kMapCubes];
  for (int c = lane; c < kMapCubes; c += 64) {
    const int ad = add[c];
    s_cur[c] = ad > 0 ? T[c].off + cur[c] : -1;
  }
  __syncthreads();
  constexpr int U = 4;
  for (int base0 = 0; base0 < n; base0 += 64 * U) {
    int ids[U];
    float4 ws[U];
#pragma unroll
    for (int u = 0; u < U; ++u) {
      const int i = base0 + u * 64 + lane;
      ids[u] = -1;
      ws[u] = make_float4(0.f, 0.f, 0.f, 0.f);
      if (i < n) { ids[u] = a.stack_cube[cls][sb + i]; ws[u] = a.stack_world[cls][sb + i]; }
    }
#pragma unroll
    for (int u = 0; u < U; ++u) {
      const int id = ids[u];
      const float4 w = ws[u];
      unsigned long long todo = __ballot(id >= 0);
      while (todo) {
        const int leader = __ffsll((long long)todo) - 1;
        const int c = __shfl(id, leader, 64);
        const unsigned long long same = __ballot(id == c);
        const int start = s_cur[c];
        if (id == c && start >= 0) pool[start + __popcll(same & ((1ull << lane) - 1ull))] = w;
        __syncthreads();
        if (lane == leader && start >= 0) s_cur[c] = start + __popcll(same);
        __syncthreads();
        todo &= ~same;
      }
    }
  }
  __syncthreads();
  for (int c = lane; c < kMapCubes; c += 64) add[c] = 0;
}

__global__ __launch_bounds__(256) void k_map_register(MapArgs a) {
  const int b = blockIdx.y, i = blockIdx.x * 256 + threadIdx.x;
  if (seq_idle(a.active, b) || i >= a.meta[b].n_cloud) return;
  const MapSeq& ms = a.seq[b];
  double par[7];
#pragma unroll
  for (int k = 0; k < 7; ++k) par[k] = ms.par[k];
  a.registered[(long long)b * a.cap + i] = associate_to_map(a.full[(long long)b * a.cap + i], par);
}

__global__ __launch_bounds__(256) void k_map_register_slabs(MapArgs a) {
  const int r = blockIdx.x, b = blockIdx.y;
  if (seq_idle(a.active, b)) return;
  const int start = a.ringstart[b * (a.R + 1) + r], n = a.ringstart[b * (a.R + 1) + r + 1] - start;
  const MapSeq& ms = a.seq[b];
  double par[7];
#pragma unroll
  for (int k = 0; k < 7; ++k) par[k] = ms.par[k];
  const float4* src = a.slabs + ((long long)b * a.R + r) * a.slab;
  float4* dst = a.registered + (long long)b * a.cap + start;
  for (int i = threadIdx.x; i < n; i += 256) dst[i] = associate_to_map(src[i], par);
}

__global__ __launch_bounds__(256) void k_map_report(MapArgs a, int step) {
  const int b = blockIdx.x, cls = blockIdx.y, tid = threadIdx.x;
  const CubeDesc* T = cube_table(a, b, cls);
  __shared__ int s_red[4][4];
  __shared__ int s_last;
  const bool idle = seq_idle(a.active, b);
  int live = 0;
  if (!idle) for (int c = tid; c < kMapCubes; c += 256) live += T[c].cnt;
#pragma unroll
  for (int d = 32; d >= 1; d >>= 1) live += __shfl_xor(live, d, 64);
  if ((tid & 63) == 0) s_red[0][tid >> 6] = live;
  __syncthreads();
  if (tid == 0) {
    live = s_red[0][0] + s_red[0][1] + s_red[0][2] + s_red[0][3];
    if (!idle) atomicExch(&a.live[b * 2 + cls], live);
    __threadfence();
    s_last = atomicAdd(&a.report_dev[0], 1) == (int)(gridDim.x * gridDim.y) - 1;
  }
  __syncthreads();
  if (!s_last) return;
  int m[4] = {0, 0, 0, 0};
  for (int i = tid; i < a.B; i += 256) {
    m[0] = max(m[0], atomicAdd(&a.live[i * 2], 0)); m[1] = max(m[1], atomicAdd(&a.live[i * 2 + 1], 0));
    m[2] = max(m[2], a.seq[i].n_stack[0]); m[3] = max(m[3], a.seq[i].n_stack[1]);
  }
#pragma unroll
  for (int k = 0; k < 4; ++k) {
#pragma unroll
    for (int d = 32; d >= 1; d >>= 1) m[k] = max(m[k], __shfl_xor(m[k], d, 64));
    if ((tid & 63) == 0) s_red[k][tid >> 6] = m[k];
  }
  __syncthreads();
  if (tid == 0) {
    for (int k = 0; k < 4; ++k) m[k] = max(max(s_red[k][0], s_red[k][1]), max(s_red[k][2], s_red[k][3]));
    a.report_dev[0] = 0;
    a.report_dev[1] = max(a.report_dev[1], m[2]);
    a.report_dev[2] = max(a.report_dev[2], m[3]);
    volatile int* h = a.report_host;
    h[1] = m[0]; h[2] = m[1]; h[3] = a.report_dev[1]; h[4] = a.report_dev[2];
    __threadfence_system();
    h[0] = step;
  }
}

__global__ __launch_bounds__(256) void k_reset_sequences(ResetArgs r) {
  const int b = r.seqs[blockIdx.x], tid = threadIdx.x;
  if (tid == 0) {
    r.meta[b] = SeqMeta{};
    OdomState st{};
    st.para_q[3] = 1.0; st.q_w[3] = 1.0;
    r.state[b] = st;
    if (r.mapseq) {
      MapSeq ms{};
      ms.par[3] = 1.0; ms.q_wmap_wodom[3] = 1.0;
      ms.cen[0] = 10; ms.cen[1] = 10; ms.cen[2] = 5;
      r.mapseq[b] = ms;
      r.live[2 * b] = 0; r.live[2 * b + 1] = 0;
    }
  }
  if (r.ringstart) for (int i = tid; i <= r.R; i += 256) r.ringstart[(long long)b * (r.R + 1) + i] = 0;
  for (int k = 0; k < 2; ++k) {
    if (r.less_sharp[k]) for (int i = tid; i < r.R * kLessSharpPerRing; i += 256) r.less_sharp[k][(long long)b * r.R * kLessSharpPerRing + i] = make_float4(0.f, 0.f, 0.f, 0.f);
    if (r.less_flat[k]) for (long long i = tid; i < r.cap; i += 256) r.less_flat[k][(long long)b * r.cap + i] = make_float4(0.f, 0.f, 0.f, 0.f);
  }
  if (r.edges) {
    for (int i = tid; i < r.R * kSharpPerRing; i += 256) r.edges[(long long)b * r.R * kSharpPerRing + i] = EdgeRec{};
    for (int i = tid; i < r.R * kFlatPerRing; i += 256) r.planes[(long long)b * r.R * kFlatPerRing + i] = PlaneRec{};
    if (tid < 8) r.grid_flags[tid >> 2][b * 4 + (tid & 3)] = 0;
  }
  if (r.mapseq) {
    for (int i = tid; i < 2 * kMapCubes; i += 256) {
      r.cubes[(long long)b * 2 * kMapCubes + i] = CubeDesc{0, 0, 0, 0};
      r.addcnt[(long long)b * 2 * kMapCubes + i] = 0;
    }
    if (tid < 2) { r.grid_sig[(long long)b * 2 + tid].valid = 0; r.grid_sig[(long long)b * 2 + tid].reuse = 0; }
  }
}
void launch_reset_sequences(const ResetArgs& r, hipStream_t s) { if (r.n > 0) hipLaunchKernelGGL(k_reset_sequences, dim3(r.n), dim3(256), 0, s, r); }

void launch_map_begin(const MapArgs& a, hipStream_t s) { hipLaunchKernelGGL(k_map_begin, dim3(a.B), dim3(256), 0, s, a); }
void launch_map_stack_segments(const MapArgs& a, const VoxArgs& v, hipStream_t s) {
  hipLaunchKernelGGL(k_map_stack_segments, dim3((a.B * 2 + 255) / 256), dim3(256), 0, s, a, v);
}
void launch_map_cube_segments(const MapArgs& a, const VoxArgs& v, hipStream_t s) {
  hipLaunchKernelGGL(k_map_cube_segments, dim3((a.B * 2 * kMapValidMax + 255) / 256), dim3(256), 0, s, a, v);
}
constexpr int kVoxSmallRuns = 8192, kVoxBigRuns = 24576;
constexpr int kVoxBigThreads = 1024;
constexpr size_t vox_lds_bytes(int nt, int capr, int capn) { return (size_t)capr * 6 + (size_t)capn / 8 + 2 * 128 * (size_t)(nt / 64) + sizeof(int) * ((size_t)(capr / nt) * (nt / 64) + 1 + 48) + sizeof(float) * 6 * (nt / 64) + 64; }
static_assert(vox_lds_bytes(kVoxBigThreads, kVoxBigRuns, kVoxBigN) <= 163840, "one workgroup may use the whole 160 KiB of a CU, not more");
int prepare_voxel_filter() {
  return hipFuncSetAttribute((const void*)k_vox_lds<kVoxBigThreads, kVoxBigRuns, kVoxBigN>, hipFuncAttributeMaxDynamicSharedMemorySize,
                             (int)vox_lds_bytes(kVoxBigThreads, kVoxBigRuns, kVoxBigN)) == hipSuccess ? 0 : -1;
}
void launch_voxel_filter(const VoxArgs& v, int tile_bound, hipStream_t s) {
  const int nsmall = v.n_segs < 4096 ? v.n_segs : 4096, nbig = v.n_segs < 1024 ? v.n_segs : 1024;
  hipLaunchKernelGGL((k_vox_lds<kVoxBigThreads, kVoxBigRuns, kVoxBigN>), dim3(nbig), dim3(kVoxBigThreads), vox_lds_bytes(kVoxBigThreads, kVoxBigRuns, kVoxBigN), s, v, 1);
  hipLaunchKernelGGL((k_vox_lds<256, kVoxSmallRuns, kVoxSmallN>), dim3(nsmall), dim3(256), vox_lds_bytes(256, kVoxSmallRuns, kVoxSmallN), s, v, 0);
  hipLaunchKernelGGL((k_vox_lds<64, kVoxTinyN, kVoxTinyN>), dim3(v.n_segs < 16384 ? v.n_segs : 16384), dim3(64), vox_lds_bytes(64, kVoxTinyN, kVoxTinyN), s, v, 2);
  if (tile_bound > 1024) tile_bound = 1024;
  hipLaunchKernelGGL(k_vox_setup, dim3(1), dim3(1024), 0, s, v);
  hipLaunchKernelGGL(k_vox_bbox, dim3(tile_bound), dim3(256), 0, s, v);
  hipLaunchKernelGGL(k_vox_keys_sort, dim3(tile_bound), dim3(256), 0, s, v);
  for (int level = 0; level < v.levels; ++level) hipLaunchKernelGGL(k_vox_merge, dim3(tile_bound), dim3(256), 0, s, v, level);
  hipLaunchKernelGGL(k_vox_heads, dim3(tile_bound), dim3(256), 0, s, v);
  hipLaunchKernelGGL(k_vox_scan, dim3(1), dim3(1024), 0, s, v);
  hipLaunchKernelGGL(k_vox_emit, dim3(tile_bound), dim3(256), 0, s, v);
  hipLaunchKernelGGL(k_vox_copyback, dim3(tile_bound), dim3(256), 0, s, v);
}
static size_t mapgrid_lds_bytes(int H) { return sizeof(int) * ((size_t)H + 1024 + 160); }
static_assert(sizeof(int) * ((size_t)kMapGridMaxH + 1024 + 160) <= 163840, "the bucket table of k_mapgrid_build must fit one CU's LDS");
int prepare_map_grid(int H) {
  if (H > kMapGridMaxH || H < 1024 || (H & (H - 1))) return -1;
  return hipFuncSetAttribute((const void*)k_mapgrid_build, hipFuncAttributeMaxDynamicSharedMemorySize, (int)mapgrid_lds_bytes(H)) == hipSuccess ? 0 : -1;
}
void launch_map_grid(const MapArgs& a, hipStream_t s) {
  hipLaunchKernelGGL(k_mapgrid_build, dim3(a.B, 2), dim3(1024), mapgrid_lds_bytes(a.grid_H), s, a);
}
void launch_map_associate(const MapArgs& a, int iter, hipStream_t s) {
  const int by = (a.B + 7) / 8 * 8;
  (void)iter;
  hipLaunchKernelGGL(k_map_search<0>, dim3(kMapSearchBlocks[0] * by), dim3(kMapSearchThreads), 0, s, a, kMapSearchBlocks[0]);
  hipLaunchKernelGGL(k_map_fit<0>, dim3(16, a.B), dim3(256), 0, s, a);
  hipLaunchKernelGGL(k_map_search<1>, dim3(kMapSearchBlocks[1] * by), dim3(kMapSearchThreads), 0, s, a, kMapSearchBlocks[1]);
  hipLaunchKernelGGL(k_map_fit<1>, dim3(48, a.B), dim3(256), 0, s, a);
}
void launch_map_solve(const MapArgs& a, int iter, bool last, hipStream_t s) {
  hipLaunchKernelGGL(k_map_solve, dim3(a.B), dim3(kMapSolveThreads), sizeof(int) * (size_t)(a.rec_tiles_per_seq + 2), s, a, iter, last ? 1 : 0);
}
void launch_map_insert(const MapArgs& a, float4* staging, hipStream_t s) {
  hipLaunchKernelGGL(k_map_cubeid, dim3(32, a.B, 2), dim3(256), 0, s, a);
  hipLaunchKernelGGL(k_map_compact_plan, dim3(a.B, 2), dim3(256), 0, s, a);
  hipLaunchKernelGGL(k_map_compact_move<0>, dim3(64, a.B, 2), dim3(256), 0, s, a, staging);
  hipLaunchKernelGGL(k_map_compact_move<1>, dim3(64, a.B, 2), dim3(256), 0, s, a, staging);
  hipLaunchKernelGGL(k_map_reserve, dim3(a.B, 2), dim3(256), 0, s, a);
  hipLaunchKernelGGL(k_map_scatter, dim3(a.B, 2), dim3(64), 0, s, a);
}
void launch_map_register(const MapArgs& a, hipStream_t s) {
  if (a.slabs) hipLaunchKernelGGL(k_map_register_slabs, dim3(a.R, a.B), dim3(256), 0, s, a);
  else hipLaunchKernelGGL(k_map_register, dim3((a.cap + 255) / 256, a.B), dim3(256), 0, s, a);
}
void launch_map_report(const MapArgs& a, int step, hipStream_t s) { hipLaunchKernelGGL(k_map_report, dim3(a.B, 2), dim3(256), 0, s, a, step); }

}
```

a-loam_amd/csrc/mapping_kernels.hpp:

```cpp
#pragma once
#include "aloam_device.hpp"

namespace aloam {

constexpr int kMapW = 21, kMapH = 21, kMapD = 11, kMapCubes = kMapW * kMapH * kMapD;
constexpr int kMapValidMax = 75;
constexpr int kMapGridMaxH = 32768;
constexpr int kVoxTile = 2048;
constexpr int kVoxTinyN = 2048, kVoxSmallN = 8192, kVoxBigN = 65536;

enum MapErrBits { kMapErrPool = 1, kMapErrKeys = 2, kMapErrSegment = 4 };

struct CubeDesc { int off, cnt, cap, pad; };

struct MapGridSig {
  int valid;
  int reuse;
  int n;
  int pad;
  int2 cube[kMapValidMax];
};

struct alignas(16) MapSeq {
  double par[7];
  double q_wmap_wodom[4], t_wmap_wodom[3];
  double q_wodom[4], t_wodom[3];
  int cen[3];
  int center[3];
  int frame_count;
  int n_valid;
  int from_total[2];
  int gate;
  int n_stack[2];
  int factor_num[2][2];
  int lm_iterations[2], lm_termination[2];
  int pool_used[2];
  int err;
  int compactions;
  int err_steps;
  int pad;
};

struct MapEdgeRec { double a[3], b[3]; float cp[3]; int pad; };
struct MapNormRec { double n[3], d; float cp[3]; int pad; };
static_assert(sizeof(MapEdgeRec) == 64 && sizeof(MapNormRec) == 48, "record sizes");

struct VoxSeg {
  const float4* in;
  float4* out;
  int* out_count;
  float4* final_out;
  int* final_count;
  int n;
  float leaf;
  int key_off, tile0, ntiles, pad;
};

struct VoxArgs {
  VoxSeg* segs;
  int n_segs;
  int* tile_seg;
  int* tile_heads;
  int* tile_pref;
  int* counters;
  int* lists;
  unsigned long long* keys[2];
  float4* tmp;
  int* bbox;
  int tile_cap;
  long long key_cap;
  int levels;
};

struct MapArgs {
  int B, cap, R;
  SeqMeta* meta;
  OdomState* odom;
  MapSeq* seq;
  float line_res, plane_res;
  const float4* less_sharp[2];
  const float4* less_flat[2];
  const int* active;
  const float4* full;
  const float4* slabs; int slab; const int* ringstart;
  float4* registered;
  CubeDesc* cubes;
  float4* pool[2];
  int pool_cap;
  int* tab;
  float4* stack[2];
  float4* stack_world[2];
  int* stack_cube[2];
  int* addcnt;
  int* cursor;
  int* compact_flag;
  float4* grid_sorted[2];
  int* grid_start[2];
  int grid_H;
  int* live;
  int* report_dev;
  int* report_host;
  float4* knn;
  MapEdgeRec* edges;
  MapNormRec* norms;
  int lm_max_iterations;
  int* rec_tiles;
  int rec_tiles_per_seq, rec_tiles_corner;
  int* vox_counters;
  MapGridSig* grid_sig;
};
constexpr int kTabInts = 256;

void launch_map_begin(const MapArgs& a, hipStream_t s);
void launch_map_stack_segments(const MapArgs& a, const VoxArgs& v, hipStream_t s);
void launch_map_cube_segments(const MapArgs& a, const VoxArgs& v, hipStream_t s);
void launch_voxel_filter(const VoxArgs& v, int tile_bound, hipStream_t s);
int prepare_voxel_filter();
int prepare_map_grid(int H);
void launch_map_grid(const MapArgs& a, hipStream_t s);
void launch_map_associate(const MapArgs& a, int iter, hipStream_t s);
void launch_map_solve(const MapArgs& a, int iter, bool last, hipStream_t s);
void launch_map_insert(const MapArgs& a, float4* staging, hipStream_t s);
void launch_map_register(const MapArgs& a, hipStream_t s);
void launch_map_report(const MapArgs& a, int step, hipStream_t s);

struct ResetArgs {
  const int* seqs; int n;
  int R;
  SeqMeta* meta; int* ringstart;
  OdomState* state;
  EdgeRec* edges; PlaneRec* planes;
  int* grid_flags[2];
  float4* less_sharp[2]; float4* less_flat[2]; int cap;
  MapSeq* mapseq; CubeDesc* cubes; int* addcnt; int* live;
  MapGridSig* grid_sig;
};
void launch_reset_sequences(const ResetArgs& r, hipStream_t s);
int prepare_reference_order();
void launch_voxel_filter_reference_order(const VoxArgs& v, const MapArgs& a, bool stacks, hipStream_t s);

}
```

a-loam_amd/csrc/odometry_kernels.hip:

```cpp
#include "aloam_device.hpp"
#include "aloam_trig.hpp"
#include "lm_device.hpp"
#include "odometry_kernels.hpp"

namespace aloam {

#define ALOAM_PHASE(name) asm volatile("; ##PHASE " name)
#ifdef ALOAM_PHASE_CLOCK
__device__ unsigned long long g_phase_clock_odo[2][32];
#define ALOAM_BG_CLOCK(slot) do { if (threadIdx.x == 0 && blockIdx.x == 1) { atomicAdd(&g_phase_clock_odo[0][slot], (unsigned long long)__builtin_readcyclecounter()); atomicAdd(&g_phase_clock_odo[1][slot], 1ull); } } while (0)
#else
#define ALOAM_BG_CLOCK(slot) do { } while (0)
#endif
#ifdef ALOAM_ASSOC_STATS
__device__ unsigned long long g_assoc_stats[2][32];
#define ALOAM_STAT(cls, i, v) do { if ((threadIdx.x & 63) == 0) atomicAdd(&g_assoc_stats[cls][i], (unsigned long long)(v)); } while (0)
#else
#define ALOAM_STAT(cls, i, v) do { } while (0)
#endif

__device__ __forceinline__ float4 transform_to_start(const float4& p, const OdomState& st) {
  double q[4] = {st.para_q[0], st.para_q[1], st.para_q[2], st.para_q[3]};
  if (q[3] < 0.0) { q[0] = -q[0]; q[1] = -q[1]; q[2] = -q[2]; q[3] = -q[3]; }
  double o[3];
  quat_rotate(q, (double)p.x, (double)p.y, (double)p.z, o);
  return make_float4((float)(o[0] + st.para_t[0]), (float)(o[1] + st.para_t[1]), (float)(o[2] + st.para_t[2]), p.w);
}

__device__ __forceinline__ double interpolation_ratio(float frac) { return (double)frac / 0.1; }

__device__ __forceinline__ void slerp_scales(double w, double s, double* c0, double* c1, double* dc0, double* dc1) {
  const double one = 1.0 - 2.220446049250313e-16;
  const double absD = fabs(w);
  if (absD >= one) { *c0 = 1.0 - s; *c1 = s; *dc0 = 0.0; *dc1 = 0.0; }
  else {
    const double theta = acos_port(absD), st = sin_port(theta), ct = cos_port(theta);
    const double a0 = (1.0 - s) * theta, a1 = s * theta;
    const double s0 = sin_port(a0), s1 = sin_port(a1);
    *c0 = s0 / st;
    *c1 = s1 / st;
    const double g = (w < 0.0 ? 1.0 : -1.0) / st;
    *dc0 = ((1.0 - s) * cos_port(a0) * st - s0 * ct) / (st * st) * g;
    *dc1 = (s * cos_port(a1) * st - s1 * ct) / (st * st) * g;
  }
  if (w < 0.0) { *c1 = -*c1; *dc1 = -*dc1; }
}

__device__ __forceinline__ void deskew_point(const double q[4], const double t[3], double s, double vx, double vy, double vz,
                                             double lp[3], double (*M)[4]) {
  double c0, c1, dc0, dc1;
  slerp_scales(q[3], s, &c0, &c1, &dc0, &dc1);
  const double u[3] = {c1 * q[0], c1 * q[1], c1 * q[2]}, w = c0 + c1 * q[3];
  const double v[3] = {vx, vy, vz};
  const double uv[3] = {2.0 * (u[1] * v[2] - u[2] * v[1]), 2.0 * (u[2] * v[0] - u[0] * v[2]), 2.0 * (u[0] * v[1] - u[1] * v[0])};
  lp[0] = v[0] + w * uv[0] + (u[1] * uv[2] - u[2] * uv[1]) + s * t[0];
  lp[1] = v[1] + w * uv[1] + (u[2] * uv[0] - u[0] * uv[2]) + s * t[1];
  lp[2] = v[2] + w * uv[2] + (u[0] * uv[1] - u[1] * uv[0]) + s * t[2];
  if (!M) return;
  double Du[3][3];
#pragma unroll
  for (int k = 0; k < 3; ++k) {
    double e[3] = {0.0, 0.0, 0.0};
    e[k] = 1.0;
    const double ev[3] = {2.0 * (e[1] * v[2] - e[2] * v[1]), 2.0 * (e[2] * v[0] - e[0] * v[2]), 2.0 * (e[0] * v[1] - e[1] * v[0])};
    Du[0][k] = w * ev[0] + (e[1] * uv[2] - e[2] * uv[1]) + (u[1] * ev[2] - u[2] * ev[1]);
    Du[1][k] = w * ev[1] + (e[2] * uv[0] - e[0] * uv[2]) + (u[2] * ev[0] - u[0] * ev[2]);
    Du[2][k] = w * ev[2] + (e[0] * uv[1] - e[1] * uv[0]) + (u[0] * ev[1] - u[1] * ev[0]);
  }
  const double dw = dc0 + dc1 * q[3] + c1;
#pragma unroll
  for (int r = 0; r < 3; ++r) {
    M[r][0] = c1 * Du[r][0];
    M[r][1] = c1 * Du[r][1];
    M[r][2] = c1 * Du[r][2];
    M[r][3] = dc1 * (Du[r][0] * q[0] + Du[r][1] * q[1] + Du[r][2] * q[2]) + uv[r] * dw;
  }
}

__device__ __forceinline__ void deskew_jacobian_row(const double a[3], const double (*M)[4], const double q[4], double s, double J[6]) {
  double g[4];
#pragma unroll
  for (int j = 0; j < 4; ++j) g[j] = a[0] * M[0][j] + a[1] * M[1][j] + a[2] * M[2][j];
  J[0] = g[0] * q[3] - g[1] * q[2] + g[2] * q[1] - g[3] * q[0];
  J[1] = g[0] * q[2] + g[1] * q[3] - g[2] * q[0] - g[3] * q[1];
  J[2] = -g[0] * q[1] + g[1] * q[0] + g[2] * q[3] - g[3] * q[2];
  J[3] = a[0] * s; J[4] = a[1] * s; J[5] = a[2] * s;
}

constexpr float kCell3Surf = 0.5f;
constexpr float kCell3Corner = 0.75f;
constexpr float kCell3CoarseFactor = 4.0f, kCell2 = 2.625f;
constexpr unsigned kIdxMask = (1u << 20) - 1u;
__device__ __forceinline__ float cell3_of(int which) { return which == 0 ? kCell3Corner : kCell3Surf; }

__device__ __forceinline__ unsigned hash3(int a, int b, int c) {
  return ((unsigned)a * 73856093u) ^ ((unsigned)b * 19349663u) ^ ((unsigned)c * 83492791u);
}

constexpr int kFusedMaxN = 65535, kFusedMaxH = 16384;
constexpr int kWalkKeys = kMaxRings + 8;

__device__ __forceinline__ void walk_tables(const float4* __restrict__ pts, int n, int R, int* __restrict__ walk, int* s_walk, int* s_flag, int tid) {
  const int S = R + 8, lane = tid & 63;
  int* s_first = s_walk;
  int* s_last = s_walk + kWalkKeys;
  for (int k = tid; k < kWalkKeys; k += 1024) { s_first[k] = 0x7fffffff; s_last[k] = -1; }
  __syncthreads();
  for (int base = 0; base < n; base += 1024) {
    const int i = base + tid;
    const int key = i < n ? (int)pts[i].w : -1;
    const int prev = __shfl_up(key, 1, 64), next = __shfl_down(key, 1, 64);
    if (key >= 0 && key < S) {
      if (lane == 0 || prev != key) atomicMin(&s_first[key], i);
      if (lane == 63 || next != key) atomicMax(&s_last[key], i);
    }
  }
  __syncthreads();
  if (tid == 0) {
    int run = n;
    for (int k = S - 1; k >= 0; --k) { run = min(run, s_first[k]); s_first[k] = run; walk[k] = run; }
    run = -1;
    for (int k = 0; k < S; ++k) { run = max(run, s_last[k]); s_last[k] = run; walk[S + k] = run; }
    bool nearly = true;
    for (int k = 3; k < S; ++k) nearly = nearly && s_last[k - 3] < s_first[k];
    s_flag[1] = nearly ? 1 : 2;
  }
  __syncthreads();
}
__host__ __device__ __forceinline__ bool fused_takes(int n, int H) { return n <= kFusedMaxN && H <= kFusedMaxH; }

__global__ __launch_bounds__(1024) void k_build_grids_fused(OdomArgs a) {
  constexpr int U = 4;
  const int b = blockIdx.y, which = blockIdx.x, tid = threadIdx.x, lane = tid & 63, wave = tid >> 6;
  if (seq_idle(a.active, b, kSeqSolve)) return;
  const SeqMeta m = a.meta[b];
  const int n = which == 0 ? m.n_corner_last : m.n_surf_last;
  const float4* pts = which == 0 ? corner_last(a, b, m.parity) : surf_last(a, b, m.parity);
  const GridView g = grid_view(a, b, which);
  const int H = g.H;
  if (!fused_takes(n, H)) return;
  extern __shared__ __attribute__((aligned(16))) int lds[];
  unsigned* tab = reinterpret_cast<unsigned*>(lds);
  int* s_part = lds + 3 * (H / 2);
  int* s_flag = s_part + 48;
  int* s_walk = s_flag + 8;
  int* const starts[3] = {g.start3, g.start3c, g.start2};
  if (n == 0) {
    for (int t = 0; t < 3; ++t) for (int h = tid; h <= H; h += 1024) starts[t][h] = 0;
    if (tid < 3) g.flags[tid] = 0;
    return;
  }
  ALOAM_BG_CLOCK(0);
  for (int w = tid; w < 3 * (H / 2); w += 1024) tab[w] = 0u;
  if (tid < 2) s_flag[tid] = 0;
  __syncthreads();
  ALOAM_BG_CLOCK(1);
  const float inv0 = 1.0f / cell3_of(which), inv1 = 1.0f / (cell3_of(which) * kCell3CoarseFactor), inv2 = 1.0f / kCell2;
  const unsigned hm = (unsigned)(H - 1);
  auto buckets = [&](const float4& p, int key, unsigned* h) {
    h[0] = hash3((int)floorf(p.x * inv0), (int)floorf(p.y * inv0), (int)floorf(p.z * inv0)) & hm;
    h[1] = hash3((int)floorf(p.x * inv1), (int)floorf(p.y * inv1), (int)floorf(p.z * inv1)) & hm;
    h[2] = hash3((int)floorf(p.x * inv2), (int)floorf(p.y * inv2), key) & hm;
  };
  auto fetch = [&](int base, float4* p) {
#pragma unroll
    for (int u = 0; u < U; ++u) { const int i = base + u * 1024 + tid; p[u] = pts[i < n ? i : n - 1]; }
  };
  {
    int bad = 0, unsorted = 0;
    for (int base = 0; base < n; base += U * 1024) {
      float4 p[U];
      float pw[U];
      fetch(base, p);
#pragma unroll
      for (int u = 0; u < U; ++u) { const int i = base + u * 1024 + tid; pw[u] = pts[i < n ? (i > 0 ? i - 1 : 0) : n - 1].w; }
#pragma unroll
      for (int u = 0; u < U; ++u) {
        if (base + u * 1024 + tid >= n) continue;
        const int key = (int)p[u].w;
        if (key < 0 || key > a.R || !(fabsf(p[u].x) < 4096.f && fabsf(p[u].y) < 4096.f && fabsf(p[u].z) < 4096.f)) bad = 1;
        if (key < (int)pw[u]) unsorted = 1;
        unsigned h[3];
        buckets(p[u], key, h);
#pragma unroll
        for (int t = 0; t < 3; ++t) atomicAdd(&tab[t * (H / 2) + (h[t] >> 1)], 1u << ((h[t] & 1u) * 16));
      }
    }
    if (bad) atomicOr(&s_flag[0], 1);
    if (unsorted) atomicOr(&s_flag[1], 1);
  }
  __syncthreads();
  ALOAM_BG_CLOCK(2);
  if (s_flag[1] && !s_flag[0]) walk_tables(pts, n, a.R, g.walk, s_walk, s_flag, tid);
  if (tid < 3) g.flags[tid] = tid == 2 ? 0 : s_flag[tid];
  ALOAM_BG_CLOCK(3);
  {
    const int wpt = H / 2048;
    int local[3], inc[3];
#pragma unroll
    for (int t = 0; t < 3; ++t) {
      local[t] = 0;
      for (int k = 0; k < wpt; ++k) { const unsigned w = tab[t * (H / 2) + tid * wpt + k]; local[t] += (int)(w & 0xffffu) + (int)(w >> 16); }
      inc[t] = wave_scan_i32<false>(local[t]);
      if (lane == 63) s_part[t * 16 + wave] = inc[t];
    }
    __syncthreads();
#pragma unroll
    for (int t = 0; t < 3; ++t) {
      int run = inc[t] - local[t];
#pragma unroll 1
      for (int w = 0; w < wave; ++w) run += s_part[t * 16 + w];
      int* st = starts[t] + tid * wpt * 2;
      for (int k = 0; k < wpt; ++k) {
        const unsigned w = tab[t * (H / 2) + tid * wpt + k];
        const int c0 = (int)(w & 0xffffu), c1 = (int)(w >> 16);
        st[2 * k] = run; st[2 * k + 1] = run + c0;
        tab[t * (H / 2) + tid * wpt + k] = (unsigned)run | ((unsigned)(run + c0) << 16);
        run += c0 + c1;
      }
      if (tid == 1023) starts[t][H] = run;
    }
  }
  __syncthreads();
  ALOAM_BG_CLOCK(4);
  for (int base = 0; base < n; base += U * 1024) {
    float4 p[U];
    fetch(base, p);
#pragma unroll
    for (int u = 0; u < U; ++u) {
      const int i = base + u * 1024 + tid;
      if (i >= n) continue;
      const int key = (int)p[u].w;
      unsigned h[3];
      buckets(p[u], key, h);
      unsigned pos[3];
#pragma unroll
      for (int t = 0; t < 3; ++t) {
        const unsigned sh = (h[t] & 1u) * 16;
        pos[t] = (atomicAdd(&tab[t * (H / 2) + (h[t] >> 1)], 1u << sh) >> sh) & 0xffffu;
      }
      const float4 e = make_float4(p[u].x, p[u].y, p[u].z, __uint_as_float((unsigned)i | ((unsigned)(key + 1) << 20)));
      g.sorted3[pos[0]] = e;
      g.sorted3c[pos[1]] = e;
      g.sorted2[pos[2]] = e;
    }
  }
  ALOAM_BG_CLOCK(5);
#ifdef ALOAM_PHASE_CLOCK
  __syncthreads();
  ALOAM_BG_CLOCK(6);
#endif
}

constexpr int kBgWaves = 4;
constexpr int kBgUnroll = 4;
__global__ __launch_bounds__(1024, kBgWaves) void k_build_grids(OdomArgs a) {
  constexpr int U = kBgUnroll;
  const int b = blockIdx.y, which = blockIdx.x / 3, tid = threadIdx.x;
  const int pass_lo = blockIdx.x % 3, pass_hi = pass_lo + 1;
  if (seq_idle(a.active, b, kSeqSolve)) return;
  const SeqMeta m = a.meta[b];
  const int n = which == 0 ? m.n_corner_last : m.n_surf_last;
  const float4* pts = which == 0 ? corner_last(a, b, m.parity) : surf_last(a, b, m.parity);
  const GridView g = grid_view(a, b, which);
  if (fused_takes(n, g.H)) return;
  extern __shared__ __attribute__((aligned(16))) int lds[];
  int* cnt = lds;
  int* part = lds + g.H;
  int* s_flag = part + 1024;
  if (tid < 2) s_flag[tid] = n >= (1 << 20) && tid == 0 ? 1 : 0;
  if (n == 0) {
    for (int pass = pass_lo; pass < pass_hi; ++pass) { int* st = pass == 0 ? g.start3 : pass == 1 ? g.start3c : g.start2; for (int h = tid; h <= g.H; h += 1024) st[h] = 0; }
    if (tid < 3 && pass_lo == 0) g.flags[tid] = 0;
    return;
  }
  auto fetch = [&](int base, float4* p) {
#pragma unroll
    for (int u = 0; u < U; ++u) { const int i = base + u * 1024 + tid; p[u] = pts[i < n ? i : n - 1]; }
  };
  for (int pass = pass_lo; pass < pass_hi; ++pass) {
    const bool g3 = pass < 2;
    const float cell = pass == 0 ? cell3_of(which) : pass == 1 ? cell3_of(which) * kCell3CoarseFactor : kCell2;
    const float inv = 1.0f / cell;
    int* start = pass == 0 ? g.start3 : pass == 1 ? g.start3c : g.start2;
    float4* sorted = pass == 0 ? g.sorted3 : pass == 1 ? g.sorted3c : g.sorted2;
    __syncthreads();
    for (int h = tid; h < g.H; h += 1024) cnt[h] = 0;
    __syncthreads();
    float4 p[U], pn[U];
    float pw[U], pwn[U];
    fetch(0, p);
    if (pass == 0) {
#pragma unroll
      for (int u = 0; u < U; ++u) { const int i = u * 1024 + tid; pw[u] = pts[i < n ? (i > 0 ? i - 1 : 0) : n - 1].w; }
    }
    int bad = 0, unsorted = 0;
    for (int base = 0; base < n; base += U * 1024) {
      if (base + U * 1024 < n) {
        fetch(base + U * 1024, pn);
        if (pass == 0) {
#pragma unroll
          for (int u = 0; u < U; ++u) { const int i = base + U * 1024 + u * 1024 + tid; pwn[u] = pts[i < n ? i - 1 : n - 1].w; }
        }
      }
#pragma unroll
      for (int u = 0; u < U; ++u) {
        if (base + u * 1024 + tid >= n) continue;
        const int key = (int)p[u].w;
        if (pass == 0) {
          if (key < 0 || key > a.R || !(fabsf(p[u].x) < 4096.f && fabsf(p[u].y) < 4096.f && fabsf(p[u].z) < 4096.f)) bad = 1;
          if (key < (int)pw[u]) unsorted = 1;
        }
        const int ix = (int)floorf(p[u].x * inv), iy = (int)floorf(p[u].y * inv);
        const int iz = g3 ? (int)floorf(p[u].z * inv) : key;
        atomicAdd(&cnt[hash3(ix, iy, iz) & (g.H - 1)], 1);
      }
#pragma unroll
      for (int u = 0; u < U; ++u) { p[u] = pn[u]; pw[u] = pwn[u]; }
    }
    if (pass == 0) {
      if (bad) atomicOr(&s_flag[0], 1);
      if (unsorted) atomicOr(&s_flag[1], 1);
    }
    __syncthreads();
    if (pass == 0 && tid < 3) g.flags[tid] = tid == 2 ? 0 : (tid == 1 ? 2 * s_flag[1] : s_flag[0]);
    const int per = g.H / 1024;
    int local = 0;
    for (int k = 0; k < per; ++k) local += cnt[tid * per + k];
    part[tid] = local;
    __syncthreads();
    for (int d = 1; d < 1024; d <<= 1) {
      const int v = tid >= d ? part[tid - d] : 0;
      __syncthreads();
      part[tid] += v;
      __syncthreads();
    }
    int run = part[tid] - local;
    for (int k = 0; k < per; ++k) { const int c = cnt[tid * per + k]; cnt[tid * per + k] = run; start[tid * per + k] = run; run += c; }
    if (tid == 1023) start[g.H] = run;
    __syncthreads();
    fetch(0, p);
    for (int base = 0; base < n; base += U * 1024) {
      if (base + U * 1024 < n) fetch(base + U * 1024, pn);
#pragma unroll
      for (int u = 0; u < U; ++u) {
        const int i = base + u * 1024 + tid;
        if (i >= n) continue;
        const int key = (int)p[u].w;
        const int ix = (int)floorf(p[u].x * inv), iy = (int)floorf(p[u].y * inv);
        const int iz = g3 ? (int)floorf(p[u].z * inv) : key;
        const int pos = atomicAdd(&cnt[hash3(ix, iy, iz) & (g.H - 1)], 1);
        sorted[pos] = make_float4(p[u].x, p[u].y, p[u].z, __uint_as_float((unsigned)i | ((unsigned)(key + 1) << 20)));
      }
#pragma unroll
      for (int u = 0; u < U; ++u) p[u] = pn[u];
    }
  }
}

__device__ __forceinline__ float walk_dist(const float4& p, const float4& sel) {
  return (p.x - sel.x) * (p.x - sel.x) + (p.y - sel.y) * (p.y - sel.y) + (p.z - sel.z) * (p.z - sel.z);
}

__device__ __forceinline__ unsigned long long wave_min_u64(unsigned long long v) {
  return wave_min_packed(v);
}

__device__ __forceinline__ void ring2d(int r, int t, int* dx, int* dy) {
  const int w = 2 * r + 1;
  if (t < w) { *dx = -r + t; *dy = -r; }
  else if (t < 2 * w) { *dx = -r + (t - w); *dy = r; }
  else { const int u = t - 2 * w, side = u / (w - 2); *dy = -r + 1 + u % (w - 2); *dx = side ? r : -r; }
}
__device__ __forceinline__ void shell3d(int r, int c, int* dx, int* dy, int* dz) {
  const int w = 2 * r + 1, nface = w * w;
  if (c < 2 * nface) { const int f = c / nface, q = c % nface; *dz = f ? r : -r; *dy = q / w - r; *dx = q % w - r; }
  else { const int q = c - 2 * nface; *dz = -r + 1 + q / (8 * r); ring2d(r, q % (8 * r), dx, dy); }
}

template <int kSweep> struct Kept { float4 p[kSweep]; bool a[kSweep]; bool ok; };

template <int kSweep, class F>
__device__ __forceinline__ void wave_sweep(const float4* __restrict__ sorted, int s0, int cnt, int lane, int* row, F&& f, Kept<kSweep>* keep = nullptr) {
  const int incl = wave_scan_i32<false>(cnt);
  const int total = __builtin_amdgcn_readlane(incl, 63);
  const int excl = incl - cnt;
  int carry = 0;
  for (int base = 0; base < total; base += kSweep * 64) {
    const int slot = excl - base;
    const int rows = total - base > (kSweep - 1) * 64 ? kSweep : (total - base + 63) >> 6;
#pragma unroll
    for (int u = 0; u < kSweep; ++u) if (u < rows) row[u * 64 + lane] = 0;
    __builtin_amdgcn_wave_barrier();
    if (cnt > 0 && slot >= 0 && slot < rows * 64) row[slot] = lane + 1;
    __builtin_amdgcn_wave_barrier();
    int own[kSweep];
#pragma unroll
    for (int u = 0; u < kSweep; ++u) own[u] = u < rows ? row[u * 64 + lane] : 0;
    __builtin_amdgcn_wave_barrier();
    float4 p[kSweep];
#pragma unroll
    for (int u = 0; u < kSweep; ++u) {
      p[u] = make_float4(0.f, 0.f, 0.f, 0.f);
      if (u < rows) {
        if (lane == 0 && carry > own[u]) own[u] = carry;
        own[u] = wave_scan_i32<true>(own[u]);
        carry = __builtin_amdgcn_readlane(own[u], 63);
        const int i = base + u * 64 + lane;
        const int os = __shfl(s0, own[u] - 1, 64), oe = __shfl(excl, own[u] - 1, 64);
        const int at = i < total ? os + (i - oe) : 0;
        p[u] = sorted[at];
      }
    }
#pragma unroll
    for (int u = 0; u < kSweep; ++u) {
      const bool act = u < rows && base + u * 64 + lane < total;
      if (keep) { keep->p[u] = p[u]; keep->a[u] = act; }
      if (act) f(p[u]);
    }
  }
  if (keep) keep->ok = total <= kSweep * 64;
}

__device__ __forceinline__ float cell_gap(float s, int c, float cell) {
  const float lo = (float)c * cell, hi = lo + cell;
  const float gap = s < lo ? lo - s : (s > hi ? s - hi : 0.f);
  return gap > 1e-3f ? gap - 1e-3f : 0.f;
}

struct Track { unsigned long long v; float x, y, z; };
__device__ __forceinline__ void track_take(Track& t, bool ok, unsigned long long v, const float4& p) {
  const bool k = ok && v < t.v;
  t.v = k ? v : t.v; t.x = k ? p.x : t.x; t.y = k ? p.y : t.y; t.z = k ? p.z : t.z;
}

template <int kSweep>
__device__ __forceinline__ unsigned long long wave_nn(const GridView& g, bool bad, int which, const float4* pts, int n, const float4& sel, int lane, int* row, Track& mine, Kept<kSweep>& kept) {
  unsigned long long best = ~0ull;
  auto visit = [&](const float4& p) {
    const float ddx = p.x - sel.x, ddy = p.y - sel.y, ddz = p.z - sel.z;
    const float d = (ddx * ddx + ddy * ddy) + ddz * ddz;
    const unsigned wb = __float_as_uint(p.w);
    track_take(mine, true, ((unsigned long long)__float_as_uint(d) << 32) | ((wb & kIdxMask) << 12) | (wb >> 20), p);
  };
  if (!bad) {
    const float cell = cell3_of(which);
    {
      const float inv = 1.0f / cell;
      const int cx = (int)floorf(sel.x * inv), cy = (int)floorf(sel.y * inv), cz = (int)floorf(sel.z * inv);
      int s0 = 0, cnt = 0;
      if (lane < 27) {
        const unsigned h = hash3(cx + lane % 3 - 1, cy + (lane % 9) / 3 - 1, cz + lane / 9 - 1) & (unsigned)(g.H - 1);
        s0 = g.start3[h];
        cnt = g.start3[h + 1] - s0;
      }
      wave_sweep<kSweep>(g.sorted3, s0, cnt, lane, row, visit, &kept);
      best = wave_min_u64(mine.v);
      const float bound = (1.0f - 0.01f) * cell;
      if (best != ~0ull && __uint_as_float((unsigned)(best >> 32)) <= bound * bound) return best;
    }
    const float cellc = cell * kCell3CoarseFactor, invc = 1.0f / cellc;
    const int ux = (int)floorf(sel.x * invc), uy = (int)floorf(sel.y * invc), uz = (int)floorf(sel.z * invc);
    for (int r = 1;; ++r) {
      const int ncell = r == 1 ? 27 : 24 * r * r + 2;
      const float limit = best != ~0ull ? fminf(__uint_as_float((unsigned)(best >> 32)), 25.0f) : 25.0f;
      for (int cb = 0; cb < ncell; cb += 64) {
        const int c = cb + lane;
        int s0 = 0, cnt = 0;
        if (c < ncell) {
          int dx, dy, dz;
          if (r == 1) { dz = c / 9 - 1; dy = (c % 9) / 3 - 1; dx = c % 3 - 1; }
          else shell3d(r, c, &dx, &dy, &dz);
          const float gx = cell_gap(sel.x, ux + dx, cellc), gy = cell_gap(sel.y, uy + dy, cellc), gz = cell_gap(sel.z, uz + dz, cellc);
          if (((gx * gx + gy * gy) + gz * gz) * 0.999f <= limit) {
            const unsigned h = hash3(ux + dx, uy + dy, uz + dz) & (unsigned)(g.H - 1);
            s0 = g.start3c[h];
            cnt = g.start3c[h + 1] - s0;
          }
        }
        wave_sweep<kSweep>(g.sorted3c, s0, cnt, lane, row, visit);
      }
      best = wave_min_u64(mine.v);
      const float bc = ((float)r - 0.01f) * cellc, b2 = bc * bc;
      if (best != ~0ull && __uint_as_float((unsigned)(best >> 32)) <= b2) break;
      if (b2 >= 25.0f) break;
    }
    return best;
  }
  for (int base = 0; base < n; base += 64) {
    const int j = base + lane;
    if (j < n) {
      const float4 p = pts[j];
      visit(make_float4(p.x, p.y, p.z, __uint_as_float((unsigned)j)));
    }
  }
  return wave_min_u64(mine.v);
}

template <bool DISTORT>
__global__ __launch_bounds__(256) void k_transform_queries(OdomArgs a) {
  const int b = blockIdx.y, i = blockIdx.x * 256 + threadIdx.x;
  if (seq_idle(a.active, b, kSeqSolve)) return;
  const SeqMeta m = a.meta[b];
  if (i >= m.n_sharp + m.n_flat) return;
  const bool plane = i >= m.n_sharp;
  const int qi = plane ? i - m.n_sharp : i;
  const long long o = plane ? (long long)b * a.R * kFlatPerRing + qi : (long long)b * a.R * kSharpPerRing + qi;
  const float4 raw = plane ? a.flat[o] : a.sharp[o];
  float4 sel;
  if (DISTORT) {
    const OdomState& st = a.state[b];
    const double q[4] = {st.para_q[0], st.para_q[1], st.para_q[2], st.para_q[3]}, t[3] = {st.para_t[0], st.para_t[1], st.para_t[2]};
    const float frac = raw.w - (float)(int)raw.w;
    double lp[3];
    deskew_point(q, t, interpolation_ratio(frac), (double)raw.x, (double)raw.y, (double)raw.z, lp, nullptr);
    sel = make_float4((float)lp[0], (float)lp[1], (float)lp[2], raw.w);
  } else sel = transform_to_start(raw, a.state[b]);
  (plane ? a.sel_flat : a.sel_sharp)[o] = sel;
}

constexpr int kAssocSweepWide = 6;
constexpr int kAssocSweepPlane = 3;
template <bool PLANE, bool WIDE> struct SweepRows { static constexpr int value = WIDE ? (PLANE ? kAssocSweepWide : 3) : (PLANE ? kAssocSweepPlane : 2); };

template <bool PLANE, bool WIDE>
__device__ __forceinline__ void associate_one(const OdomArgs& a, int b, int qi, const SeqMeta& m, const GridView& g, int lane, int* row) {
  constexpr int kSweep = SweepRows<PLANE, WIDE>::value;
  const int qcap = PLANE ? a.R * kFlatPerRing : a.R * kSharpPerRing;
  const float4* Q = (PLANE ? a.flat : a.sharp) + (long long)b * qcap;
  const float4 raw = Q[qi];
  const float4 sel = ((PLANE ? a.sel_flat : a.sel_sharp) + (long long)b * qcap)[qi];
  const bool bad = g.flags[0] != 0, unsorted = g.flags[1] != 0;
  const float frac = raw.w - (float)(int)raw.w;
  const int nt = PLANE ? m.n_surf_last : m.n_corner_last;
  const float4* T = PLANE ? surf_last(a, b, m.parity) : corner_last(a, b, m.parity);
  int valid = 0;
  Track t1 = {~0ull, 0.f, 0.f, 0.f}, t2 = t1, t3 = t1;
  Kept<kSweep> kept;
  kept.ok = false;
#pragma unroll
  for (int u = 0; u < kSweep; ++u) { kept.a[u] = false; kept.p[u] = make_float4(0.f, 0.f, 0.f, 0.f); }
  unsigned long long best2 = ~0ull, best3 = ~0ull;
  const unsigned long long nn = nt > 0 ? wave_nn(g, bad, PLANE ? 1 : 0, T, nt, sel, lane, row, t1, kept) : ~0ull;
  const float nnd = __uint_as_float((unsigned)(nn >> 32));
  if (nn != ~0ull && (double)nnd < 25.0) {
    const int closest = (int)((unsigned)nn >> 12);
    const int cid = bad ? (int)T[closest].w : (int)((unsigned)nn & 0xfffu) - 1;
    auto consider = [&](const float4& p, int j, int key) {
      if (j == closest) return;
      const bool up = j > closest;
      bool c2, c3;
      if (PLANE) { c2 = up ? key <= cid : key >= cid; c3 = !c2; }
      else { c2 = up ? key > cid : key < cid; c3 = false; }
      const float d = walk_dist(p, sel);
      if (!((double)d < 25.0)) return;
      const unsigned seq = up ? (unsigned)(j - closest) : 0x40000000u + (unsigned)(closest - j);
      const unsigned long long v = ((unsigned long long)__float_as_uint(d) << 32) | seq;
      track_take(t2, c2, v, p);
      if (PLANE) track_take(t3, c3, v, p);
    };
    if (!bad && !unsorted) {
      auto visit = [&](const float4& p) {
        const unsigned wb = __float_as_uint(p.w);
        const int j = (int)(wb & kIdxMask), pk = (int)(wb >> 20) - 1;
        if (pk >= cid - 2 && pk <= cid + 2) consider(p, j, pk);
      };
      bool done2 = false, done3 = !PLANE;
      float lim2 = 25.0f, lim3 = 25.0f;
      if (kept.ok) {
#pragma unroll
        for (int u = 0; u < kSweep; ++u) if (kept.a[u]) visit(kept.p[u]);
        best2 = wave_min_u64(t2.v);
        if (PLANE) best3 = wave_min_u64(t3.v);
        const float bound = (1.0f - 0.01f) * cell3_of(PLANE ? 1 : 0), b2 = bound * bound;
        if (best2 != ~0ull) lim2 = __uint_as_float((unsigned)(best2 >> 32));
        if (PLANE && best3 != ~0ull) lim3 = __uint_as_float((unsigned)(best3 >> 32));
        done2 = best2 != ~0ull && lim2 <= b2;
        done3 = !PLANE || (best3 != ~0ull && lim3 <= b2);
      }
      for (int level = 0; level < 2 && !(done2 && done3); ++level) {
        const float cell = kCell2, inv = 1.0f / cell;
        const int cx = (int)floorf(sel.x * inv), cy = (int)floorf(sel.y * inv);
        const int nlook = level == 0 ? 45 : 80;
        for (int lb = 0; lb < nlook; lb += 64) {
          const int l = lb + lane;
          int s0 = 0, cnt = 0;
          if (l < nlook) {
            const int key = cid + l % 5 - 2, cc = l / 5;
            int ddx, ddy;
            if (level == 0) { ddx = cc % 3 - 1; ddy = cc / 3 - 1; }
            else ring2d(2, cc, &ddx, &ddy);
            const bool second = PLANE ? key == cid : key != cid;
            const bool wanted = second ? !done2 : (PLANE && !done3);
            const float gx = cell_gap(sel.x, cx + ddx, cell), gy = cell_gap(sel.y, cy + ddy, cell);
            if (key >= 0 && wanted && (gx * gx + gy * gy) * 0.999f <= (second ? lim2 : lim3)) {
              const unsigned h = hash3(cx + ddx, cy + ddy, key) & (unsigned)(g.H - 1);
              s0 = g.start2[h];
              cnt = g.start2[h + 1] - s0;
            }
          }
          wave_sweep<kSweep>(g.sorted2, s0, cnt, lane, row, visit);
        }
        best2 = wave_min_u64(t2.v);
        if (PLANE) best3 = wave_min_u64(t3.v);
        const float bound = ((float)(level + 1) - 0.01f) * cell, b2 = bound * bound;
        if (b2 >= 25.0f) break;
        if (best2 != ~0ull) lim2 = __uint_as_float((unsigned)(best2 >> 32));
        if (PLANE && best3 != ~0ull) lim3 = __uint_as_float((unsigned)(best3 >> 32));
        done2 = best2 != ~0ull && lim2 <= b2;
        done3 = !PLANE || (best3 != ~0ull && lim3 <= b2);
      }
    } else {
      for (int base = closest + 1; base < nt; base += 64) {
        const int j = base + lane;
        bool stop = false;
        float4 p = make_float4(0.f, 0.f, 0.f, 0.f);
        int key = 0;
        if (j < nt) { p = T[j]; key = (int)p.w; stop = (double)key > (double)cid + 2.5; }
        const unsigned long long sm = __ballot(stop);
        const int first_stop = sm ? (__ffsll((long long)sm) - 1) : 64;
        if (j < nt && lane < first_stop) consider(p, j, key);
        if (sm) break;
      }
      for (int base = closest - 1; base >= 0; base -= 64) {
        const int j = base - lane;
        bool stop = false;
        float4 p = make_float4(0.f, 0.f, 0.f, 0.f);
        int key = 0;
        if (j >= 0) { p = T[j]; key = (int)p.w; stop = (double)key < (double)cid - 2.5; }
        const unsigned long long sm = __ballot(stop);
        const int first_stop = sm ? (__ffsll((long long)sm) - 1) : 64;
        if (j >= 0 && lane < first_stop) consider(p, j, key);
        if (sm) break;
      }
      best2 = wave_min_u64(t2.v);
      if (PLANE) best3 = wave_min_u64(t3.v);
    }
    valid = best2 != ~0ull && (!PLANE || best3 != ~0ull);
  }
  if (PLANE) {
    PlaneRec* e = a.planes + (long long)b * a.R * kFlatPerRing + qi;
    if (lane == 0) {
      e->cp[0] = raw.x; e->cp[1] = raw.y; e->cp[2] = raw.z;
      e->valid = valid; e->pad[0] = __float_as_int(frac); e->pad[1] = e->pad[2] = 0;
      if (!valid) for (int k = 0; k < 3; ++k) e->j[k] = e->l[k] = e->m[k] = 0.f;
    }
    if (valid) {
      if (t1.v == nn) { e->j[0] = t1.x; e->j[1] = t1.y; e->j[2] = t1.z; }
      if (t2.v == best2) { e->l[0] = t2.x; e->l[1] = t2.y; e->l[2] = t2.z; }
      if (t3.v == best3) { e->m[0] = t3.x; e->m[1] = t3.y; e->m[2] = t3.z; }
    }
  } else {
    EdgeRec* e = a.edges + (long long)b * a.R * kSharpPerRing + qi;
    if (lane == 0) {
      e->cp[0] = raw.x; e->cp[1] = raw.y; e->cp[2] = raw.z;
      e->valid = valid; e->pad[0] = __float_as_int(frac); e->pad[1] = 0;
      if (!valid) for (int k = 0; k < 3; ++k) e->a[k] = e->b[k] = 0.f;
    }
    if (valid) {
      if (t1.v == nn) { e->a[0] = t1.x; e->a[1] = t1.y; e->a[2] = t1.z; }
      if (t2.v == best2) { e->b[0] = t2.x; e->b[1] = t2.y; e->b[2] = t2.z; }
// ... 132 lines not shown
  const int t = j - closest, nt = closest - j;
  const unsigned seq = (unsigned)(t > nt ? t : nt) | ((unsigned)t & 0x80000000u);
  bool ok, own;
  if (NEARLY) {
    ok = j != closest && j > lo && j < hi && d < 25.0f;
    own = t > 0 ? key <= cid : key >= cid;
  } else {
    ok = j != closest && (unsigned)(key - cid + 2) <= 4u && d < 25.0f;
    own = key == cid;
  }
  const unsigned db = __float_as_uint(d);
  if (PLANE) {
    take_min(t2, ((unsigned long long)(ok && own ? db : ~0u) << 32) | seq);
    take_min(t3, ((unsigned long long)(ok && !own ? db : ~0u) << 32) | seq);
  } else take_min(t2, ((unsigned long long)(ok && !own ? db : ~0u) << 32) | seq);
}
__device__ __forceinline__ bool none(unsigned long long best) { return (unsigned)(best >> 32) == ~0u; }
__device__ __forceinline__ int index_of(unsigned long long best, int closest) {
  const unsigned seq = (unsigned)best;
  return (seq & 0x80000000u) ? closest - (int)(seq & 0x7fffffffu) : closest + (int)seq;
}

struct alignas(16) CellOff2 { int dx, dy; float ax, ay; };
struct alignas(16) CellOff3 { int dx, dy, dz; int pad; };
#define ALOAM_C2(x, y) {x, y, (x < 0 ? -x : x) * 2.625f, (y < 0 ? -y : y) * 2.625f}
__device__ __constant__ CellOff2 kRingCells[24] = {
    ALOAM_C2(-1, -1), ALOAM_C2(0, -1), ALOAM_C2(1, -1), ALOAM_C2(-1, 0), ALOAM_C2(1, 0), ALOAM_C2(-1, 1), ALOAM_C2(0, 1), ALOAM_C2(1, 1),
    ALOAM_C2(-2, -2), ALOAM_C2(-1, -2), ALOAM_C2(0, -2), ALOAM_C2(1, -2), ALOAM_C2(2, -2), ALOAM_C2(-2, 2), ALOAM_C2(-1, 2), ALOAM_C2(0, 2), ALOAM_C2(1, 2), ALOAM_C2(2, 2),
    ALOAM_C2(-2, -1), ALOAM_C2(-2, 0), ALOAM_C2(-2, 1), ALOAM_C2(2, -1), ALOAM_C2(2, 0), ALOAM_C2(2, 1)};
#undef ALOAM_C2
static_assert(kCell2 == 2.625f, "kRingCells holds |d| * kCell2");
__device__ __constant__ CellOff3 kBlock27[27] = {
    {-1, -1, -1, 0}, {0, -1, -1, 0}, {1, -1, -1, 0}, {-1, 0, -1, 0}, {0, 0, -1, 0}, {1, 0, -1, 0}, {-1, 1, -1, 0}, {0, 1, -1, 0}, {1, 1, -1, 0},
    {-1, -1, 0, 0},  {0, -1, 0, 0},  {1, -1, 0, 0},  {-1, 0, 0, 0},  {0, 0, 0, 0},  {1, 0, 0, 0},  {-1, 1, 0, 0},  {0, 1, 0, 0},  {1, 1, 0, 0},
    {-1, -1, 1, 0},  {0, -1, 1, 0},  {1, -1, 1, 0},  {-1, 0, 1, 0},  {0, 0, 1, 0},  {1, 0, 1, 0},  {-1, 1, 1, 0},  {0, 1, 1, 0},  {1, 1, 1, 0}};
struct AxisGap { float up, dn; };
__device__ __forceinline__ AxisGap axis_gap_of(float s, int c, float cell) {
  const float lo = (float)c * cell;
  return {((lo + cell) - s) - cell - 1e-3f, (s - lo) - cell - 1e-3f};
}
__device__ __forceinline__ float axis_gap(int d, float ad_cell, const AxisGap& a) { return fmaxf(ad_cell + (d > 0 ? a.up : a.dn), 0.f); }

template <bool HALVES> __device__ __forceinline__ unsigned long long seg_min(unsigned long long v, int last4) { return HALVES ? half_min_packed(v, last4) : wave_min_u64(v); }
template <bool HALVES> __device__ __forceinline__ int seg_max_count(int n) {
  if (!HALVES) return __builtin_amdgcn_readfirstlane(n);
  const int a = __builtin_amdgcn_readlane(n, 0), b = __builtin_amdgcn_readlane(n, 32);
  return a > b ? a : b;
}

template <int kRows, bool HALVES>
__device__ __forceinline__ unsigned long long coarse_shells(const GridView& g, unsigned last_index, float cellc, float sx, float sy, float sz, unsigned long long nn, bool need,
                                                            int lane, int last4, int* lds, int stat_cls = 0) {
  constexpr int W = HALVES ? 32 : 64;
  const int l = lane & (W - 1);
  const float invc = 1.0f / cellc;
  const float2v sxy = {sx, sy};
  const int ux = (int)floorf(sx * invc), uy = (int)floorf(sy * invc), uz = (int)floorf(sz * invc);
  const AxisGap ax = axis_gap_of(sx, ux, cellc), ay = axis_gap_of(sy, uy, cellc), az = axis_gap_of(sz, uz, cellc);
  const unsigned hm = (unsigned)(g.H - 1);
  unsigned long long t1 = nn;
  ALOAM_STAT(stat_cls, 28, 1); (void)stat_cls;
  for (int r = 1;; ++r) {
    const int ncell = r == 1 ? 27 : 24 * r * r + 2;
    const float limit = fminf(__uint_as_float((unsigned)(nn >> 32)), 25.0f);
    for (int cb = 0; cb < ncell; cb += W) {
      const int c = cb + l;
      int s0 = 0, cnt = 0;
      if (need && c < ncell) {
        int dx, dy, dz;
        if (r == 1) { const CellOff3 o = kBlock27[c]; dx = o.dx; dy = o.dy; dz = o.dz; }
        else shell3d(r, c, &dx, &dy, &dz);
        const float gx = axis_gap(dx, fabsf((float)dx) * cellc, ax), gy = axis_gap(dy, fabsf((float)dy) * cellc, ay), gz = axis_gap(dz, fabsf((float)dz) * cellc, az);
        if (((gx * gx + gy * gy) + gz * gz) * 0.999f <= limit) {
          const unsigned hh = hash3(ux + dx, uy + dy, uz + dz) & hm;
          bucket_bounds(g.start3c, hh, s0, cnt);
        }
      }
      sweep2<HALVES, kRows>(g.sorted3c, last_index, s0, cnt, lane, last4, lds, [&](const float4& p, int, bool) { take_min(t1, nn_key(dist_to(p, sxy, sz), __float_as_uint(p.w))); });
    }
    nn = seg_min<HALVES>(t1, last4);
    const float bc = ((float)r - 0.01f) * cellc, b2 = bc * bc;
    if (__uint_as_float((unsigned)(nn >> 32)) <= b2) need = false;
    if (b2 >= 25.0f || !__ballot(need)) break;
  }
  return nn;
}

template <bool PLANE, int kRows, bool HALVES, bool NEARLY>
__device__ __forceinline__ void ring_grid(const GridView& g, unsigned last_index, float sx, float sy, float sz, int closest, int cid, bool want2, bool want3,
                                          unsigned long long& best2, unsigned long long& best3, int lane, int last4, int* lds, int lo, int hi) {
  constexpr bool kOwnFirst = PLANE;
  constexpr int W = HALVES ? 32 : 64;
  const int l = lane & (W - 1);
  const unsigned hm = (unsigned)(g.H - 1);
  const float2v sxy = {sx, sy};
  unsigned long long t2 = best2, t3 = best3;
  float lim2 = !none(best2) ? __uint_as_float((unsigned)(best2 >> 32)) : 25.0f, lim3 = !none(best3) ? __uint_as_float((unsigned)(best3 >> 32)) : 25.0f;
  const float rc = kCell2, inv = 1.0f / rc;
  const int cx = (int)floorf(sx * inv), cy = (int)floorf(sy * inv);
  const AxisGap ax = axis_gap_of(sx, cx, rc), ay = axis_gap_of(sy, cy, rc);
  const bool track2 = __ballot(want2) != 0ull;
  ALOAM_STAT(PLANE ? 1 : 0, 20, 1); ALOAM_STAT(PLANE ? 1 : 0, 21, want2); ALOAM_STAT(PLANE ? 1 : 0, 22, want3); ALOAM_STAT(PLANE ? 1 : 0, 23, !none(best3) || (!PLANE && !none(best2)));
  for (int stage = kOwnFirst ? 0 : 1; stage < 3 && __ballot(want2 || want3); ++stage) {
    ALOAM_STAT(PLANE ? 1 : 0, 24 + stage, 1);
    const bool wo = PLANE ? (NEARLY ? want2 || want3 : want3) : want2, ws = PLANE && (NEARLY ? want2 || want3 : want2);
    const int lc = stage == 0 ? 0 : stage == 1 ? 3 : 4, ncell = 1 << lc, nslot = PLANE ? 5 : 4;
    const int n_look = ncell * nslot + (stage == 1 && !kOwnFirst ? nslot : 0);
    ALOAM_PHASE("ring_lookup");
    for (int lb = 0; lb < n_look; lb += W) {
      const int k = lb + l;
      int s0 = 0, cnt = 0;
      const bool centre = k >= ncell * nslot;
      const int slot = centre ? k - ncell * nslot : k >> lc;
      const bool other = slot < 4;
      if (k < n_look && (other ? wo : ws)) {
        const int key = cid - 2 + (int)((0x2819u >> (slot * 3)) & 7u);
        int ddx = 0, ddy = 0;
        float gx = 0.f, gy = 0.f;
        if (stage > 0 && !centre) {
          const CellOff2 o = kRingCells[(stage == 1 ? 0 : 8) + (k & (ncell - 1))];
          ddx = o.dx; ddy = o.dy;
          gx = axis_gap(ddx, o.ax, ax); gy = axis_gap(ddy, o.ay, ay);
        }
        const bool second = PLANE ? !other : true;
        if (key >= 0 && (gx * gx + gy * gy) * 0.999f <= (second ? lim2 : lim3)) {
          const unsigned hh = hash3(cx + ddx, cy + ddy, key) & hm;
          bucket_bounds(g.start2, hh, s0, cnt);
        }
      }
      ALOAM_PHASE("ring_sweep");
      sweep2<HALVES, kRows>(g.sorted2, last_index, s0, cnt, lane, last4, lds, [&](const float4& p, int, bool) {
        const unsigned wb = __float_as_uint(p.w);
        consider2<PLANE, NEARLY>(dist_to(p, sxy, sz), (int)(wb & kIdxMask), (int)(wb >> 20) - 1, closest, cid, t2, t3, lo, hi);
      }, nullptr, nullptr, PLANE ? 1 : 0, 8 + 4 * stage);
    }
    ALOAM_PHASE("ring_mins");
    if (!PLANE || track2) best2 = seg_min<HALVES>(t2, last4);
    if (PLANE) best3 = seg_min<HALVES>(t3, last4);
    ALOAM_PHASE("ring_bounds");
    if (stage == 2) break;
    float bound;
    if (stage == 0) bound = (1.0f - 0.01f) * fmaxf(fminf(fminf(ax.up, ax.dn), fminf(ay.up, ay.dn)) + rc, 0.f);
    else bound = ((float)stage - 0.01f) * rc;
    const float b2 = bound * bound;
    if (!none(best2)) lim2 = __uint_as_float((unsigned)(best2 >> 32));
    if (PLANE && !none(best3)) lim3 = __uint_as_float((unsigned)(best3 >> 32));
    if (!none(best2) && lim2 <= b2) want2 = false;
    if (PLANE && !none(best3) && lim3 <= b2) want3 = false;
  }
}

__device__ __forceinline__ unsigned long long read_u64(unsigned long long v, int src) {
  return ((unsigned long long)(unsigned)__builtin_amdgcn_readlane((int)(unsigned)(v >> 32), src) << 32) | (unsigned)__builtin_amdgcn_readlane((int)(unsigned)v, src);
}
__device__ __forceinline__ float read_f32(float v, int src) { return __int_as_float(__builtin_amdgcn_readlane(__float_as_int(v), src)); }

template <bool PLANE, int kRows, bool PAIRED_TAILS, bool NEARLY>
__device__ __forceinline__ void associate_pair(const OdomArgs& a, int b, int qi0, int nq, int nt, const GridView& g, int lane, int* lds) {
  constexpr int kRows1 = (kRows + 1) / 2;
  const int l = lane & 31, hsel = lane >> 5, last4 = (lane | 31) << 2;
  const int qi = qi0 + hsel;
  const bool qact = qi < nq;
  const int qcap = PLANE ? a.R * kFlatPerRing : a.R * kSharpPerRing;
  const long long qo = (long long)b * qcap + (qact ? qi : qi0);
  const float4 raw = (PLANE ? a.flat : a.sharp)[qo];
  const float4 sel = (PLANE ? a.sel_flat : a.sel_sharp)[qo];
  const float frac = raw.w - (float)(int)raw.w;
  const int parity = a.meta[b].parity;
  const float4* T = PLANE ? surf_last(a, b, parity) : corner_last(a, b, parity);
  const unsigned hm = (unsigned)(g.H - 1), last_index = (unsigned)(nt - 1);
  const float cell = cell3_of(PLANE ? 1 : 0);
  const float2v selxy = {sel.x, sel.y};

  ALOAM_PHASE("setup");
  unsigned long long t1 = ~0ull;
  KeptPair<kRows> kept;
  int kept_rows = 0;
#pragma unroll
  for (int u = 0; u < kRows; ++u) kept.k[u] = ~0ull;
  {
    const float inv = 1.0f / cell;
    const int cx = (int)floorf(sel.x * inv), cy = (int)floorf(sel.y * inv), cz = (int)floorf(sel.z * inv);
    int s0 = 0, cnt = 0;
    if (l < 27 && qact) {
      const unsigned hh = hash3(cx + l % 3 - 1, cy + (l % 9) / 3 - 1, cz + l / 9 - 1) & hm;
      bucket_bounds(g.start3, hh, s0, cnt);
    }
    sweep2<true, kRows>(g.sorted3, last_index, s0, cnt, lane, last4, lds, [&](const float4& p, int u, bool first) {
      const unsigned long long v = nn_key(dist_to(p, selxy, sel.z), __float_as_uint(p.w));
      if (first) kept.k[u] = v;
      take_min(t1, v);
    }, &kept.ok, &kept_rows, PLANE ? 1 : 0, 4);
  }
  ALOAM_PHASE("nn_min");
  unsigned long long nn = half_min_packed(t1, last4);
  float fine_b2;
  {
    const float inv = 1.0f / cell;
    const float lx = floorf(sel.x * inv) * cell, ly = floorf(sel.y * inv) * cell, lz = floorf(sel.z * inv) * cell;
    const float gap = fminf(fminf(fminf(sel.x - lx, (lx + cell) - sel.x), fminf(sel.y - ly, (ly + cell) - sel.y)), fminf(sel.z - lz, (lz + cell) - sel.z));
    const float b = (1.0f - 0.01f) * (cell + (gap > 1e-3f ? gap - 1e-3f : 0.f));
    fine_b2 = b * b;
  }
  {
    const float bound2 = fine_b2;
    const bool need1 = qact && !(nn != ~0ull && __uint_as_float((unsigned)(nn >> 32)) <= bound2);
    const unsigned long long need = __ballot(need1);
    const bool n0 = need & 1ull, n1 = (need >> 32) & 1ull;
    if (PAIRED_TAILS && n0 && n1) nn = coarse_shells<kRows1, true>(g, last_index, cell * kCell3CoarseFactor, sel.x, sel.y, sel.z, nn, need1, lane, last4, lds, PLANE ? 1 : 0);
    else if (n0 || n1) {
      const int q = n0 ? 0 : 1;
#pragma unroll
      for (int qq = 0; qq < 2; ++qq) {
        if (PAIRED_TAILS ? qq != q : !((need >> (32 * qq)) & 1ull)) continue;
        const unsigned long long r = coarse_shells<kRows1, false>(g, last_index, cell * kCell3CoarseFactor, read_f32(sel.x, 32 * qq), read_f32(sel.y, 32 * qq), read_f32(sel.z, 32 * qq),
                                                                    read_u64(nn, 32 * qq), true, lane, 0, lds, PLANE ? 1 : 0);
        if (hsel == qq) nn = r;
      }
    }
  }
  ALOAM_PHASE("classes");
  const float nnd = __uint_as_float((unsigned)(nn >> 32));
  const bool has1 = qact && nn != ~0ull && nnd < 25.0f;
  const int closest = (int)((unsigned)nn >> 12);
  const int cid = (int)((unsigned)nn & 0xfffu) - 1;
  unsigned long long best2 = ~0ull, best3 = ~0ull;
  int wlo = -1, whi = nt;
  if (NEARLY && has1) {
    const int S = a.R + 8, c = min(max(cid, 0), a.R);
    whi = g.walk[c + 3];
    wlo = c >= 3 ? g.walk[S + c - 3] : -1;
  }
  ALOAM_STAT(PLANE ? 1 : 0, 0, 1); ALOAM_STAT(PLANE ? 1 : 0, 1, (int)((__ballot(qact) & 1) + ((__ballot(qact) >> 32) & 1))); ALOAM_STAT(PLANE ? 1 : 0, 2, (int)((__ballot(has1) & 1) + ((__ballot(has1) >> 32) & 1)));
  ALOAM_STAT(PLANE ? 1 : 0, 3, (int)((__ballot(has1 && kept.ok) & 1) + ((__ballot(has1 && kept.ok) >> 32) & 1)));
  if (__ballot(has1)) {
    bool want2 = has1, want3 = PLANE && has1;
    if (__ballot(has1 && kept.ok)) {
      unsigned long long t2 = ~0ull, t3 = ~0ull;
#pragma unroll
      for (int u = 0; u < kRows; ++u) {
        if (u >= kept_rows) continue;
        const unsigned lo = (unsigned)kept.k[u];
        consider2<PLANE, NEARLY>(__uint_as_float((unsigned)(kept.k[u] >> 32)), (int)(lo >> 12), (int)(lo & 0xfffu) - 1, closest, cid, t2, t3, wlo, whi);
      }
      const bool use = has1 && kept.ok;
      best2 = half_min_packed(use ? t2 : ~0ull, last4);
      if (PLANE) best3 = half_min_packed(use ? t3 : ~0ull, last4);
      const float b2 = fine_b2;
      if (!none(best2) && __uint_as_float((unsigned)(best2 >> 32)) <= b2) want2 = false;
      if (PLANE && !none(best3) && __uint_as_float((unsigned)(best3 >> 32)) <= b2) want3 = false;
    }
    ALOAM_PHASE("ring_tail");
    const unsigned long long w2 = __ballot(want2), w3 = __ballot(want3);
    const bool r0 = (w2 | w3) & 1ull, r1 = ((w2 | w3) >> 32) & 1ull;
    if (PAIRED_TAILS && r0 && r1) ring_grid<PLANE, kRows1, true, NEARLY>(g, last_index, sel.x, sel.y, sel.z, closest, cid, want2, want3, best2, best3, lane, last4, lds, wlo, whi);
    else {
#pragma unroll
      for (int q = 0; q < 2; ++q) {
        const bool q2 = (w2 >> (32 * q)) & 1ull, q3 = (w3 >> (32 * q)) & 1ull;
        if (!(q2 || q3)) continue;
        unsigned long long r2 = read_u64(best2, 32 * q), r3 = read_u64(best3, 32 * q);
        ring_grid<PLANE, kRows1, false, NEARLY>(g, last_index, read_f32(sel.x, 32 * q), read_f32(sel.y, 32 * q), read_f32(sel.z, 32 * q), __builtin_amdgcn_readlane(closest, 32 * q),
                                                __builtin_amdgcn_readlane(cid, 32 * q), q2, q3, r2, r3, lane, 0, lds, __builtin_amdgcn_readlane(wlo, 32 * q), __builtin_amdgcn_readlane(whi, 32 * q));
        if (hsel == q) { best2 = r2; best3 = r3; }
      }
    }
  }
  ALOAM_PHASE("record");
  const bool valid = has1 && !none(best2) && (!PLANE || !none(best3));

  if (qact) {
    constexpr int kPts = PLANE ? 4 : 3;
    float* e = PLANE ? reinterpret_cast<float*>(a.planes + (long long)b * a.R * kFlatPerRing + qi) : reinterpret_cast<float*>(a.edges + (long long)b * a.R * kSharpPerRing + qi);
    if (l < kPts) {
      float x = raw.x, y = raw.y, z = raw.z;
      if (l > 0) {
        x = y = z = 0.f;
        if (valid) {
          const int j = l == 1 ? closest : index_of(l == 2 ? best2 : best3, closest);
          const float4 p = T[j];
          x = p.x; y = p.y; z = p.z;
        }
      }
      e[3 * l] = x; e[3 * l + 1] = y; e[3 * l + 2] = z;
    } else if (l == kPts) {
      int* ei = reinterpret_cast<int*>(e) + 3 * kPts;
      ei[0] = valid ? 1 : 0; ei[1] = __float_as_int(frac); ei[2] = 0;
      if (PLANE) ei[3] = 0;
    }
  }
}

template <bool PLANE, bool WIDE>
__global__ __launch_bounds__(64) void k_associate_pair(OdomArgs a) {
  constexpr int kRows = PairRows<PLANE, WIDE>::value;
  __shared__ int lds[sweep2_lds_ints<kRows>()];
  const int lane = threadIdx.x, L = blockIdx.x, xcd = L & 7, slot = L >> 3;
  const int pairs = PLANE ? a.R * (kFlatPerRing / 2) : a.R * (kSharpPerRing / 2);
  const int b = (slot / pairs) * 8 + xcd, qi0 = (slot % pairs) * 2;
  if (b >= a.B || seq_idle(a.active, b, kSeqSolve)) return;
  const SeqMeta m = a.meta[b];
  const int nq = PLANE ? m.n_flat : m.n_sharp;
  if (qi0 >= nq) return;
  const GridView g = grid_view(a, b, PLANE ? 1 : 0);
  const int nt = PLANE ? m.n_surf_last : m.n_corner_last;
  if (g.flags[0] != 0 || g.flags[1] != 0 || nt <= 0) return;
  associate_pair<PLANE, kRows, !WIDE, false>(a, b, qi0, nq, nt, g, lane, lds);
}

constexpr int kPairsPerWave = 8;
template <bool PLANE, bool WIDE>
__global__ __launch_bounds__(64) void k_associate_nearly(OdomArgs a) {
  constexpr int kRows = PairRows<PLANE, WIDE>::value;
  __shared__ int lds[sweep2_lds_ints<kRows>()];
  const int lane = threadIdx.x, b = blockIdx.y;
  if (seq_idle(a.active, b, kSeqSolve)) return;
  const GridView g = grid_view(a, b, PLANE ? 1 : 0);
  if (g.flags[0] != 0 || g.flags[1] != 1) return;
  const SeqMeta m = a.meta[b];
  const int nq = PLANE ? m.n_flat : m.n_sharp, nt = PLANE ? m.n_surf_last : m.n_corner_last;
  if (nt <= 0) return;
  for (int k = 0; k < kPairsPerWave; ++k) {
    const int qi0 = (blockIdx.x * kPairsPerWave + k) * 2;
    if (qi0 >= nq) return;
    associate_pair<PLANE, kRows, !WIDE, true>(a, b, qi0, nq, nt, g, lane, lds);
  }
}

template <bool PLANE, bool WIDE>
__global__ __launch_bounds__(256) void k_associate_flagged(OdomArgs a) {
  constexpr int kSweep = SweepRows<PLANE, WIDE>::value;
  __shared__ int rows[4][kSweep * 64];
  const int b = blockIdx.x, lane = threadIdx.x & 63, wave = threadIdx.x >> 6;
  if (seq_idle(a.active, b, kSeqSolve)) return;
  const SeqMeta m = a.meta[b];
  const GridView g = grid_view(a, b, PLANE ? 1 : 0);
  const int nt = PLANE ? m.n_surf_last : m.n_corner_last;
  if (!(g.flags[0] != 0 || g.flags[1] == 2 || nt <= 0)) return;
  const int nq = PLANE ? m.n_flat : m.n_sharp;
  for (int qi = wave; qi < nq; qi += 4) associate_one<PLANE, WIDE>(a, b, qi, m, g, lane, rows[wave]);
}

constexpr int kSolveWaves = 2;
constexpr int kSolveThreads = 64 * kSolveWaves;
template <bool WITH_JAC, bool DISTORT>
__device__ void evaluate(const OdomArgs& a, int b, const double q[4], const double t[3], double* acc, int* n_edge, int* n_plane) {
  const int tid = threadIdx.x;
  const SeqMeta m = a.meta[b];
  const EdgeRec* E = a.edges + (long long)b * a.R * kSharpPerRing;
  const PlaneRec* P = a.planes + (long long)b * a.R * kFlatPerRing;
  int ne = 0, np = 0;
  for (int i = tid; i < m.n_sharp; i += kSolveThreads) {
    const EdgeRec e = E[i];
    if (!e.valid) continue;
    ++ne;
    double rcp[3], lp[3], M[3][4];
    const double s = DISTORT ? interpolation_ratio(__int_as_float(e.pad[0])) : 1.0;
    if (DISTORT) deskew_point(q, t, s, (double)e.cp[0], (double)e.cp[1], (double)e.cp[2], lp, WITH_JAC ? M : nullptr);
    else {
      quat_rotate(q, (double)e.cp[0], (double)e.cp[1], (double)e.cp[2], rcp);
      lp[0] = rcp[0] + t[0]; lp[1] = rcp[1] + t[1]; lp[2] = rcp[2] + t[2];
    }
    const double ax = e.a[0], ay = e.a[1], az = e.a[2], bx = e.b[0], by = e.b[1], bz = e.b[2];
    const double dex = ax - bx, dey = ay - by, dez = az - bz;
    const double inv = 1.0 / sqrt(dex * dex + dey * dey + dez * dez);
    const double ux = lp[0] - ax, uy = lp[1] - ay, uz = lp[2] - az, vx = lp[0] - bx, vy = lp[1] - by, vz = lp[2] - bz;
    const double r0 = (uy * vz - uz * vy) * inv, r1 = (uz * vx - ux * vz) * inv, r2 = (ux * vy - uy * vx) * inv;
    double rho0, rho1;
    huber(r0 * r0 + r1 * r1 + r2 * r2, &rho0, &rho1);
    acc[27] += 0.5 * rho0;
    if (WITH_JAC) {
      const double wx = -dex * inv, wy = -dey * inv, wz = -dez * inv;
      const double A[3][3] = {{0, -wz, wy}, {wz, 0, -wx}, {-wy, wx, 0}};
      const double Bm[3][3] = {{0, 2 * rcp[2], -2 * rcp[1]}, {-2 * rcp[2], 0, 2 * rcp[0]}, {2 * rcp[1], -2 * rcp[0], 0}};
      const double rr[3] = {r0, r1, r2};
#pragma unroll
      for (int row = 0; row < 3; ++row) {
        double J[6];
        if (DISTORT) deskew_jacobian_row(A[row], M, q, s, J);
        else {
#pragma unroll
          for (int c = 0; c < 3; ++c) {
            J[c] = A[row][0] * Bm[0][c] + A[row][1] * Bm[1][c] + A[row][2] * Bm[2][c];
            J[3 + c] = A[row][c];
          }
        }
        add_row(acc, J, rr[row], rho1);
      }
    }
  }
  for (int i = tid; i < m.n_flat; i += kSolveThreads) {
    const PlaneRec p = P[i];
    if (!p.valid) continue;
    ++np;
    const double jx = p.j[0], jy = p.j[1], jz = p.j[2];
    const double e1x = jx - (double)p.l[0], e1y = jy - (double)p.l[1], e1z = jz - (double)p.l[2];
    const double e2x = jx - (double)p.m[0], e2y = jy - (double)p.m[1], e2z = jz - (double)p.m[2];
    double nx = e1y * e2z - e1z * e2y, ny = e1z * e2x - e1x * e2z, nz = e1x * e2y - e1y * e2x;
    const double len = sqrt(nx * nx + ny * ny + nz * nz);
    nx /= len; ny /= len; nz /= len;
    double rcp[3] = {0.0, 0.0, 0.0}, lp[3], M[3][4];
    const double s = DISTORT ? interpolation_ratio(__int_as_float(p.pad[0])) : 1.0;
    if (DISTORT) deskew_point(q, t, s, (double)p.cp[0], (double)p.cp[1], (double)p.cp[2], lp, WITH_JAC ? M : nullptr);
    else {
      quat_rotate(q, (double)p.cp[0], (double)p.cp[1], (double)p.cp[2], rcp);
      lp[0] = rcp[0] + t[0]; lp[1] = rcp[1] + t[1]; lp[2] = rcp[2] + t[2];
    }
    const double r = (lp[0] - jx) * nx + (lp[1] - jy) * ny + (lp[2] - jz) * nz;
    double rho0, rho1;
    huber(r * r, &rho0, &rho1);
    acc[27] += 0.5 * rho0;
    if (WITH_JAC) {
      double J[6];
      const double nn[3] = {nx, ny, nz};
      if (DISTORT) deskew_jacobian_row(nn, M, q, s, J);
      else { J[0] = 2.0 * (nz * rcp[1] - ny * rcp[2]); J[1] = 2.0 * (nx * rcp[2] - nz * rcp[0]); J[2] = 2.0 * (ny * rcp[0] - nx * rcp[1]); J[3] = nx; J[4] = ny; J[5] = nz; }
      add_row(acc, J, r, rho1);
    }
  }
  *n_edge = ne;
  *n_plane = np;
}

template <bool DISTORT>
__global__ __launch_bounds__(kSolveThreads) void k_solve(OdomArgs a) {
  const int b = blockIdx.x, tid = threadIdx.x;
  __shared__ double s_red[kSolveWaves * 28];
  if (seq_idle(a.active, b, kSeqSolve)) return;
  OdomState& st = a.state[b];
  double q[4] = {st.para_q[0], st.para_q[1], st.para_q[2], st.para_q[3]};
  double t[3] = {st.para_t[0], st.para_t[1], st.para_t[2]};

  const LmResult lm = lm_solve_block<kSolveWaves>([&](bool with_jac, const double* qq, const double* tt, double* acc, int* ne, int* np) {
    if (with_jac) evaluate<true, DISTORT>(a, b, qq, tt, acc, ne, np); else evaluate<false, DISTORT>(a, b, qq, tt, acc, ne, np);
  }, q, t, a.lm_max_iterations, s_red);
  const int n_edges = lm.n_a, n_planes = lm.n_b, iterations = lm.iterations, successful = lm.successful, termination = lm.termination;
  const double initial_cost = lm.initial_cost, cost = lm.final_cost;

  if (tid == 0) {
    if (termination == 5) {
      for (int k = 0; k < 4; ++k) q[k] = st.para_q[k];
      for (int k = 0; k < 3; ++k) t[k] = st.para_t[k];
    }
    for (int k = 0; k < 4; ++k) st.para_q[k] = q[k];
    for (int k = 0; k < 3; ++k) st.para_t[k] = t[k];
    const int o = a.outer < 2 ? a.outer : 1;
    st.corner_corr[o] = n_edges;
    st.plane_corr[o] = n_planes;
    st.lm_iterations[o] = iterations;
    st.lm_successful[o] = successful;
    st.initial_cost[o] = initial_cost;
    st.final_cost[o] = cost;
    st.termination[o] = termination;
    if (a.last_outer) {
      const double qw[4] = {st.q_w[0], st.q_w[1], st.q_w[2], st.q_w[3]};
      double rt[3];
      quat_rotate(qw, t[0], t[1], t[2], rt);
      st.t_w[0] += rt[0]; st.t_w[1] += rt[1]; st.t_w[2] += rt[2];
      st.q_w[0] = qw[3] * q[0] + qw[0] * q[3] + qw[1] * q[2] - qw[2] * q[1];
      st.q_w[1] = qw[3] * q[1] + qw[1] * q[3] + qw[2] * q[0] - qw[0] * q[2];
      st.q_w[2] = qw[3] * q[2] + qw[2] * q[3] + qw[0] * q[1] - qw[1] * q[0];
      st.q_w[3] = qw[3] * q[3] - qw[0] * q[0] - qw[1] * q[1] - qw[2] * q[2];
    }
  }
}

__global__ void k_advance(SeqMeta* meta, OdomState* state, const int* active, int B) {
  const int b = blockIdx.x * blockDim.x + threadIdx.x;
  if (b >= B || seq_idle(active, b)) return;
  SeqMeta& m = meta[b];
  m.n_corner_last = m.n_less_sharp; m.n_surf_last = m.n_less_flat; m.parity ^= 1;
  state[b].inited = 1;
}
__global__ void k_set_inited(OdomState* state, int B, int inited) {
  const int b = blockIdx.x * blockDim.x + threadIdx.x;
  if (b < B) state[b].inited = inited;
}
void launch_set_inited(OdomState* state, int B, int inited, hipStream_t s) { hipLaunchKernelGGL(k_set_inited, dim3((B + 63) / 64), dim3(64), 0, s, state, B, inited); }
void launch_advance(const OdomArgs& a, hipStream_t s) { hipLaunchKernelGGL(k_advance, dim3((a.B + 63) / 64), dim3(64), 0, s, a.meta, a.state, a.active, a.B); }

size_t build_grids_lds_bytes(int H, int R) { return sizeof(int) * ((size_t)H + 1024 + 2 * (R + 8) + 4); }
static size_t build_grids_fused_lds_bytes(int H) { return sizeof(int) * (3 * (size_t)(H / 2) + 48 + 8 + 2 * kWalkKeys); }
int prepare_build_grids(int H_surf) {
  if (hipFuncSetAttribute((const void*)k_build_grids_fused, hipFuncAttributeMaxDynamicSharedMemorySize, (int)build_grids_fused_lds_bytes(kFusedMaxH)) != hipSuccess) return -1;
  return hipFuncSetAttribute((const void*)k_build_grids, hipFuncAttributeMaxDynamicSharedMemorySize, (int)build_grids_lds_bytes(H_surf, kMaxRings)) == hipSuccess ? 0 : -1;
}
void launch_build_grids(const OdomArgs& a, hipStream_t s) {
  const int hc = a.grid_H_corner <= kFusedMaxH ? a.grid_H_corner : 0, hs = a.grid_H_surf <= kFusedMaxH ? a.grid_H_surf : 0;
  if (hc || hs) hipLaunchKernelGGL(k_build_grids_fused, dim3(2, a.B), dim3(1024), build_grids_fused_lds_bytes(hc > hs ? hc : hs), s, a);
  hipLaunchKernelGGL(k_build_grids, dim3(6, a.B), dim3(1024), build_grids_lds_bytes(a.grid_H_surf, a.R), s, a);
}
void launch_transform_queries(const OdomArgs& a, hipStream_t s) {
  const dim3 grid((a.R * (kSharpPerRing + kFlatPerRing) + 255) / 256, a.B);
  if (a.distortion) hipLaunchKernelGGL(k_transform_queries<true>, grid, dim3(256), 0, s, a);
  else hipLaunchKernelGGL(k_transform_queries<false>, grid, dim3(256), 0, s, a);
}
void launch_associate(const OdomArgs& a, bool plane, hipStream_t s) {
  const int by = (a.B + 7) / 8 * 8;
  const int qcap = plane ? a.R * kFlatPerRing : a.R * kSharpPerRing;
  const bool wide = a.R > 64;
  const dim3 grid((unsigned)(qcap / 2 * by)), block(64), gridf((unsigned)a.B), blockf(256);
  const dim3 gridn((unsigned)((qcap / 2 + kPairsPerWave - 1) / kPairsPerWave), (unsigned)a.B);
  if (wide) {
    if (plane) { hipLaunchKernelGGL((k_associate_pair<true, true>), grid, block, 0, s, a); hipLaunchKernelGGL((k_associate_nearly<true, true>), gridn, block, 0, s, a); hipLaunchKernelGGL((k_associate_flagged<true, true>), gridf, blockf, 0, s, a); }
    else { hipLaunchKernelGGL((k_associate_pair<false, true>), grid, block, 0, s, a); hipLaunchKernelGGL((k_associate_nearly<false, true>), gridn, block, 0, s, a); hipLaunchKernelGGL((k_associate_flagged<false, true>), gridf, blockf, 0, s, a); }
  } else {
    if (plane) { hipLaunchKernelGGL((k_associate_pair<true, false>), grid, block, 0, s, a); hipLaunchKernelGGL((k_associate_nearly<true, false>), gridn, block, 0, s, a); hipLaunchKernelGGL((k_associate_flagged<true, false>), gridf, blockf, 0, s, a); }
    else { hipLaunchKernelGGL((k_associate_pair<false, false>), grid, block, 0, s, a); hipLaunchKernelGGL((k_associate_nearly<false, false>), gridn, block, 0, s, a); hipLaunchKernelGGL((k_associate_flagged<false, false>), gridf, blockf, 0, s, a); }
  }
}
void launch_solve(const OdomArgs& a, hipStream_t s) {
  if (a.distortion) hipLaunchKernelGGL(k_solve<true>, dim3(a.B), dim3(kSolveThreads), 0, s, a);
  else hipLaunchKernelGGL(k_solve<false>, dim3(a.B), dim3(kSolveThreads), 0, s, a);
}

}

#ifdef ALOAM_PHASE_CLOCK
extern "C" int aloam_debug_phase_clock_odo(unsigned long long* out) { return (int)hipMemcpyFromSymbol(out, HIP_SYMBOL(aloam::g_phase_clock_odo), sizeof(unsigned long long) * 64); }
#endif
#ifdef ALOAM_ASSOC_STATS
extern "C" int aloam_debug_assoc_stats(unsigned long long* out) { return (int)hipMemcpyFromSymbol(out, HIP_SYMBOL(aloam::g_assoc_stats), sizeof(unsigned long long) * 64); }
#endif
```

a-loam_amd/csrc/odometry_kernels.hpp:

```cpp
#pragma once
#include "aloam_device.hpp"

namespace aloam {
size_t build_grids_lds_bytes(int H, int R);
int prepare_build_grids(int H_surf);
void launch_build_grids(const OdomArgs& a, hipStream_t s);
void launch_transform_queries(const OdomArgs& a, hipStream_t s);
void launch_associate(const OdomArgs& a, bool plane, hipStream_t s);
void launch_solve(const OdomArgs& a, hipStream_t s);
void launch_advance(const OdomArgs& a, hipStream_t s);
void launch_set_inited(OdomState* state, int B, int inited, hipStream_t s);
}
```

Baseline: 123,300.

## Build next frame's KD grids on a side stream overlapping odometry solve

Double-buffers the odometry search grids by parity and builds the grids for the next frame's targets (the current less-sharp/less-flat clouds) on a separate stream while the current frame's transform/associate/solve iterations run. The current frame's grid build is skipped when a prebuilt set exists, so the sort/bucketing cost moves off the critical path. The next-frame fused build runs in a persistent kernel limited to about half the CUs, so it can run alongside the solve without taking every CU. This costs twice the grid memory, adds cross-stream event synchronisation, and adds built/invalidated state tracking that is reset on sequence reset and on injection.

```diff
diff --git a/a-loam_amd/csrc/aloam_capi.hip b/a-loam_amd/csrc/aloam_capi.hip
--- a/a-loam_amd/csrc/aloam_capi.hip
+++ b/a-loam_amd/csrc/aloam_capi.hip
@@ -67,13 +67,13 @@
   r.seqs = c->d_reset_ids.get(); r.n = n; r.R = c->R;
   r.meta = c->d_meta.get(); r.ringstart = c->d_ringstart.get(); r.state = c->d_state.get();
   r.edges = c->d_edges.get(); r.planes = c->d_planes.get();
-  for (int k = 0; k < 2; ++k) r.grid_flags[k] = c->d_grid_flags[k].get();
+  for (int p = 0; p < 2; ++p) for (int k = 0; k < 2; ++k) r.grid_flags[p][k] = c->d_grid_flags[p][k].get();
   for (int k = 0; k < 2; ++k) { r.less_sharp[k] = c->d_less_sharp[k].get(); r.less_flat[k] = c->d_less_flat[k].get(); }
   r.cap = c->cap;
   if (c->map_on) { r.mapseq = c->d_mapseq.get(); r.cubes = c->d_cubes.get(); r.addcnt = c->d_addcnt.get(); r.live = c->d_map_live.get(); r.grid_sig = c->d_grid_sig.get(); }
   launch_reset_sequences(r, c->stream);
   HIP_TRY(c, hipGetLastError());
-  for (int i = 0; i < n; ++i) { c->parity[seqs[i]] = 0; c->inited[seqs[i]] = 0; c->needs_odom[seqs[i]] = 0; c->map_err_seen[seqs[i]] = 0; clear_scorable(c, seqs[i]); place_sweep_dropped(c, seqs[i]); }
+  for (int i = 0; i < n; ++i) { c->parity[seqs[i]] = 0; c->inited[seqs[i]] = 0; c->grid_built[seqs[i]] = 0; c->needs_odom[seqs[i]] = 0; c->map_err_seen[seqs[i]] = 0; clear_scorable(c, seqs[i]); place_sweep_dropped(c, seqs[i]); }
   for (int i = 0; i < n; ++i) if (const int rc = mark_window_stale(c, seqs[i])) return rc;
   return ALOAM_OK;
 }
@@ -142,10 +142,11 @@
     HIP_TRY(c, hipEventCreateWithFlags(&c->in_consumed[k].h, hipEventDisableTiming));
   }
   c->B = cfg->batch; c->max_points = cfg->max_points; c->R = cfg->n_scans;
-  c->active.assign(c->B, 1); c->parity.assign(c->B, 0); c->inited.assign(c->B, 0); c->needs_odom.assign(c->B, 0); c->frozen.assign(c->B, 0); c->scorable.assign(c->B, 0); c->pl_has_sweep.assign(c->B, 0); c->pl_desc_valid.assign(c->B, 0);
+  c->active.assign(c->B, 1); c->parity.assign(c->B, 0); c->inited.assign(c->B, 0); c->needs_odom.assign(c->B, 0); c->frozen.assign(c->B, 0); c->scorable.assign(c->B, 0); c->grid_built.assign(c->B, 0); c->pl_has_sweep.assign(c->B, 0); c->pl_desc_valid.assign(c->B, 0);
   c->map_err_seen.assign(c->B, 0);
   c->cap = cfg->max_points + (((cfg->max_points / 32 + 15) & ~15) + 16);
   { const char* e = std::getenv("ALOAM_GRAPH_MAX_BATCH"); c->use_graph = c->B <= (e ? std::atoi(e) : 0); }
+  { const char* e = std::getenv("ALOAM_GRID_OVERLAP"); c->grid_overlap = !(e && e[0] == '0') && !c->use_graph && !c->debug_sync; }
   c->NB = (c->cap + kBlockPts - 1) / kBlockPts;
   c->npad = cfg->max_ring_points <= 2059 ? 2048 : 4096;
   const size_t B = c->B, cap = c->cap, R = c->R, NB = c->NB;
@@ -184,16 +185,21 @@
     if ((rc = dmalloc(c, c->d_less_flat[k], B * cap))) return rc;
   }
   if (odo) {
-    for (int k = 0; k < 2; ++k) {
+    for (int p = 0; p < 2; ++p) for (int k = 0; k < 2; ++k) {
       const size_t per = k == 0 ? R * kLessSharpPerRing : cap;
-      if ((rc = dmalloc(c, c->d_grid_sorted3[k], B * per))) return rc;
-      if ((rc = dmalloc(c, c->d_grid_sorted2[k], B * per))) return rc;
-      if ((rc = dmalloc(c, c->d_grid_start3[k], B * (c->grid_H[k] + 1)))) return rc;
-      if ((rc = dmalloc(c, c->d_grid_start2[k], B * (c->grid_H[k] + 1)))) return rc;
-      if ((rc = dmalloc(c, c->d_grid_sorted3c[k], B * per))) return rc;
-      if ((rc = dmalloc(c, c->d_grid_start3c[k], B * (c->grid_H[k] + 1)))) return rc;
-      if ((rc = dmalloc(c, c->d_grid_flags[k], B * 4))) return rc;
-      if ((rc = dmalloc(c, c->d_grid_walk[k], B * 2 * (R + 8)))) return rc;
+      if ((rc = dmalloc(c, c->d_grid_sorted3[p][k], B * per))) return rc;
+      if ((rc = dmalloc(c, c->d_grid_sorted2[p][k], B * per))) return rc;
+      if ((rc = dmalloc(c, c->d_grid_start3[p][k], B * (c->grid_H[k] + 1)))) return rc;
+      if ((rc = dmalloc(c, c->d_grid_start2[p][k], B * (c->grid_H[k] + 1)))) return rc;
+      if ((rc = dmalloc(c, c->d_grid_sorted3c[p][k], B * per))) return rc;
+      if ((rc = dmalloc(c, c->d_grid_start3c[p][k], B * (c->grid_H[k] + 1)))) return rc;
+      if ((rc = dmalloc(c, c->d_grid_flags[p][k], B * 4))) return rc;
+      if ((rc = dmalloc(c, c->d_grid_walk[p][k], B * 2 * (R + 8)))) return rc;
+    }
+    if (c->grid_overlap) {
+      HIP_TRY(c, hipStreamCreateWithFlags(&c->grid_stream.h, hipStreamNonBlocking));
+      HIP_TRY(c, hipEventCreateWithFlags(&c->grid_fork.h, hipEventDisableTiming));
+      HIP_TRY(c, hipEventCreateWithFlags(&c->grids_done.h, hipEventDisableTiming));
     }
     if ((rc = dmalloc(c, c->d_edges, B * R * kSharpPerRing))) return rc;
     if ((rc = dmalloc(c, c->d_planes, B * R * kFlatPerRing))) return rc;
@@ -214,6 +220,7 @@
   if (!c) return;
   if (c->stream) (void)hipStreamSynchronize(c->stream);
   if (c->copy_stream) (void)hipStreamSynchronize(c->copy_stream);
+  if (c->grid_stream) (void)hipStreamSynchronize(c->grid_stream);
   prof_resolve(c);
   delete c;
 }
diff --git a/a-loam_amd/csrc/aloam_device.hpp b/a-loam_amd/csrc/aloam_device.hpp
--- a/a-loam_amd/csrc/aloam_device.hpp
+++ b/a-loam_amd/csrc/aloam_device.hpp
@@ -87,14 +87,14 @@
   const float4* less_sharp[2];
   const float4* less_flat[2];
   const int* active;
-  float4* grid_sorted3[2];
-  float4* grid_sorted2[2];
-  int* grid_start3[2];
-  int* grid_start2[2];
-  float4* grid_sorted3c[2];
-  int* grid_start3c[2];
-  int* grid_flags[2];
-  int* grid_walk[2];
+  float4* grid_sorted3[2][2];
+  float4* grid_sorted2[2][2];
+  int* grid_start3[2][2];
+  int* grid_start2[2][2];
+  float4* grid_sorted3c[2][2];
+  int* grid_start3c[2][2];
+  int* grid_flags[2][2];
+  int* grid_walk[2][2];
   int grid_H_corner, grid_H_surf;
   float4* sel_sharp;
   float4* sel_flat;
@@ -116,18 +116,22 @@
   float4 *sorted3, *sorted2, *sorted3c;
   int *start3, *start2, *start3c, *flags, *walk;
 };
-__device__ __forceinline__ GridView grid_view(const OdomArgs& a, int b, int which) {
+template <typename T>
+__device__ __forceinline__ T* grid_ptr(T* const (&buf)[2][2], int set, int which) {
+  return set ? (which ? buf[1][1] : buf[1][0]) : (which ? buf[0][1] : buf[0][0]);
+}
+__device__ __forceinline__ GridView grid_view(const OdomArgs& a, int b, int which, int set) {
   GridView g;
   g.H = which == 0 ? a.grid_H_corner : a.grid_H_surf;
   const long long per = which == 0 ? (long long)a.R * kLessSharpPerRing : (long long)a.cap;
-  g.sorted3 = a.grid_sorted3[which] + b * per;
-  g.sorted2 = a.grid_sorted2[which] + b * per;
-  g.start3 = a.grid_start3[which] + (long long)b * (g.H + 1);
-  g.start2 = a.grid_start2[which] + (long long)b * (g.H + 1);
-  g.sorted3c = a.grid_sorted3c[which] + b * per;
-  g.start3c = a.grid_start3c[which] + (long long)b * (g.H + 1);
-  g.flags = a.grid_flags[which] + b * 4;
-  g.walk = a.grid_walk[which] + (long long)b * 2 * (a.R + 8);
+  g.sorted3 = grid_ptr(a.grid_sorted3, set, which) + b * per;
+  g.sorted2 = grid_ptr(a.grid_sorted2, set, which) + b * per;
+  g.start3 = grid_ptr(a.grid_start3, set, which) + (long long)b * (g.H + 1);
+  g.start2 = grid_ptr(a.grid_start2, set, which) + (long long)b * (g.H + 1);
+  g.sorted3c = grid_ptr(a.grid_sorted3c, set, which) + b * per;
+  g.start3c = grid_ptr(a.grid_start3c, set, which) + (long long)b * (g.H + 1);
+  g.flags = grid_ptr(a.grid_flags, set, which) + b * 4;
+  g.walk = grid_ptr(a.grid_walk, set, which) + (long long)b * 2 * (a.R + 8);
   return g;
 }
 
diff --git a/a-loam_amd/csrc/capi_internal.hpp b/a-loam_amd/csrc/capi_internal.hpp
--- a/a-loam_amd/csrc/capi_internal.hpp
+++ b/a-loam_amd/csrc/capi_internal.hpp
@@ -70,7 +70,9 @@
 
 struct aloam_ctx {
   Stream stream, copy_stream;
+  Stream grid_stream;
   Event in_copied[2], in_consumed[2], nin_done[kNinSlots], map_step_done[4];
+  Event grid_fork, grids_done;
   std::vector<Event> prof_events;
   GraphExec odom_graph[2];
   aloam_config cfg{};
@@ -106,12 +108,14 @@
   DevBuf<float4> d_sharp, d_flat;
   DevBuf<float4> d_less_sharp[2], d_less_flat[2];
   DevBuf<OdomState> d_state;
-  DevBuf<float4> d_grid_sorted3[2], d_grid_sorted2[2];
-  DevBuf<int> d_grid_start3[2], d_grid_start2[2];
-  DevBuf<float4> d_grid_sorted3c[2];
-  DevBuf<int> d_grid_start3c[2];
-  DevBuf<int> d_grid_flags[2], d_grid_walk[2];
+  DevBuf<float4> d_grid_sorted3[2][2], d_grid_sorted2[2][2];
+  DevBuf<int> d_grid_start3[2][2], d_grid_start2[2][2];
+  DevBuf<float4> d_grid_sorted3c[2][2];
+  DevBuf<int> d_grid_start3c[2][2];
+  DevBuf<int> d_grid_flags[2][2], d_grid_walk[2][2];
   int grid_H[2] = {4096, 16384};
+  bool grid_overlap = false;
+  std::vector<char> grid_built;
   DevBuf<EdgeRec> d_edges; DevBuf<PlaneRec> d_planes;
   DevBuf<float4> d_sel_sharp, d_sel_flat;
   bool map_on = false;
@@ -206,14 +210,14 @@
 
 hipEvent_t prof_event(aloam_ctx* c);
 struct ProfScope {
-  aloam_ctx* c; int k; hipEvent_t e0 = nullptr;
-  ProfScope(aloam_ctx* c_, int k_) : c(c_), k(k_) {
-    if (c->prof_on) { e0 = prof_event(c); (void)hipEventRecord(e0, c->stream); }
+  aloam_ctx* c; int k; hipStream_t s; hipEvent_t e0 = nullptr;
+  ProfScope(aloam_ctx* c_, int k_, hipStream_t on = nullptr) : c(c_), k(k_), s(on ? on : (hipStream_t)c_->stream) {
+    if (c->prof_on) { e0 = prof_event(c); (void)hipEventRecord(e0, s); }
   }
   ~ProfScope() {
-    if (c->prof_on) { hipEvent_t e1 = prof_event(c); (void)hipEventRecord(e1, c->stream); c->prof_pending.push_back({k, e0, e1}); }
+    if (c->prof_on) { hipEvent_t e1 = prof_event(c); (void)hipEventRecord(e1, s); c->prof_pending.push_back({k, e0, e1}); }
     if (c->debug_sync) {
-      const hipError_t e = hipStreamSynchronize(c->stream);
+      const hipError_t e = hipStreamSynchronize(s);
       std::fprintf(stderr, "[aloam] %-22s %s\n", kKernelNames[k], e == hipSuccess ? "ok" : hipGetErrorString(e));
     }
   }
diff --git a/a-loam_amd/csrc/capi_odometry.hip b/a-loam_amd/csrc/capi_odometry.hip
--- a/a-loam_amd/csrc/capi_odometry.hip
+++ b/a-loam_amd/csrc/capi_odometry.hip
@@ -25,11 +25,11 @@
   a.meta = c->d_meta.get(); a.state = c->d_state.get();
   a.sharp = c->d_sharp.get(); a.flat = c->d_flat.get();
   for (int k = 0; k < 2; ++k) { a.less_sharp[k] = c->d_less_sharp[k].get(); a.less_flat[k] = c->d_less_flat[k].get(); }
-  for (int k = 0; k < 2; ++k) {
-    a.grid_sorted3[k] = c->d_grid_sorted3[k].get(); a.grid_sorted2[k] = c->d_grid_sorted2[k].get(); a.grid_start3[k] = c->d_grid_start3[k].get();
-    a.grid_sorted3c[k] = c->d_grid_sorted3c[k].get(); a.grid_start3c[k] = c->d_grid_start3c[k].get();
-    a.grid_start2[k] = c->d_grid_start2[k].get();
-    a.grid_flags[k] = c->d_grid_flags[k].get(); a.grid_walk[k] = c->d_grid_walk[k].get();
+  for (int p = 0; p < 2; ++p) for (int k = 0; k < 2; ++k) {
+    a.grid_sorted3[p][k] = c->d_grid_sorted3[p][k].get(); a.grid_sorted2[p][k] = c->d_grid_sorted2[p][k].get(); a.grid_start3[p][k] = c->d_grid_start3[p][k].get();
+    a.grid_sorted3c[p][k] = c->d_grid_sorted3c[p][k].get(); a.grid_start3c[p][k] = c->d_grid_start3c[p][k].get();
+    a.grid_start2[p][k] = c->d_grid_start2[p][k].get();
+    a.grid_flags[p][k] = c->d_grid_flags[p][k].get(); a.grid_walk[p][k] = c->d_grid_walk[p][k].get();
   }
   a.grid_H_corner = c->grid_H[0]; a.grid_H_surf = c->grid_H[1];
   a.edges = c->d_edges.get(); a.planes = c->d_planes.get();
@@ -220,11 +220,26 @@
     if (const int rc = stage_ints(c, bits.data(), c->B, c->d_mask_odo.get())) return rc;
     mask = c->d_mask_odo.get();
   }
+  const bool overlap = c->grid_overlap;
+  bool build_last = !overlap;
+  if (overlap) for (int b = 0; b < c->B; ++b) build_last |= (bits[b] & kSeqSolve) && !c->grid_built[b];
+  hipError_t join_err = hipSuccess;
+  const int cus = c->gather_blocks / 8;
   auto launch_all = [&]() {
     OdomArgs a = odom_args(c);
     a.active = mask;
-    { ProfScope p(c, K_BUILD_GRIDS); launch_build_grids(a, c->stream); }
-    for (int outer = 0; outer < c->cfg.outer_iterations; ++outer) {
+    if (overlap) {
+      hipError_t e = hipEventRecord(c->grid_fork, c->stream);
+      if (e == hipSuccess) e = hipStreamWaitEvent(c->grid_stream, c->grid_fork, 0);
+      { ProfScope p(c, K_BUILD_GRIDS, c->grid_stream); launch_build_grids(a, true, cus, c->grid_stream); }
+      if (e == hipSuccess) e = hipEventRecord(c->grids_done, c->grid_stream);
+      join_err = e;
+    }
+    if (any_solve && build_last) {
+      if (overlap) launch_build_grids(a, false, cus, c->stream);
+      else { ProfScope p(c, K_BUILD_GRIDS); launch_build_grids(a, false, cus, c->stream); }
+    }
+    for (int outer = 0; any_solve && outer < c->cfg.outer_iterations; ++outer) {
       a.outer = outer;
       a.last_outer = outer == c->cfg.outer_iterations - 1;
       { ProfScope p(c, K_TRANSFORM); launch_transform_queries(a, c->stream); }
@@ -232,12 +247,11 @@
       { ProfScope p(c, K_ASSOC_PLANE); launch_associate(a, true, c->stream); }
       { ProfScope p(c, K_SOLVE); launch_solve(a, c->stream); }
     }
+    if (overlap && join_err == hipSuccess) join_err = hipStreamWaitEvent(c->stream, c->grids_done, 0);
     { ProfScope p(c, K_ADVANCE); launch_advance(a, c->stream); }
   };
   if (!any_solve) {
-    OdomArgs a = odom_args(c);
-    a.active = mask;
-    { ProfScope p(c, K_ADVANCE); launch_advance(a, c->stream); }
+    launch_all();
   } else if (c->use_graph && !c->prof_on && !c->debug_sync) {
     GraphExec& ge = c->odom_graph[mask ? 1 : 0];
     if (!ge) {
@@ -260,8 +274,9 @@
   } else {
     launch_all();
   }
+  HIP_TRY(c, join_err);
   HIP_TRY(c, hipGetLastError());
-  for (int b = 0; b < c->B; ++b) if (bits[b] & kSeqActive) { c->parity[b] ^= 1; c->inited[b] = 1; c->needs_odom[b] = 0; }
+  for (int b = 0; b < c->B; ++b) if (bits[b] & kSeqActive) { c->parity[b] ^= 1; c->inited[b] = 1; c->needs_odom[b] = 0; c->grid_built[b] = overlap; }
   c->reg_pending = false;
   return ALOAM_OK;
 }
@@ -341,6 +356,7 @@
   for (auto& x : in) if (!cloud_row(c, x.s, seq)) { c->err = "this context has no buffers for the last clouds (created for the registration stage only)"; return ALOAM_E_STATE; }
   c->inject_max = std::max(c->inject_max, std::max(n_corner, n_surf));
   HIP_TRY(c, hipStreamSynchronize(c->stream));
+  c->grid_built[seq] = 0;
   for (auto& x : in) if (x.n) HIP_TRY(c, hipMemcpy(cloud_row(c, x.s, seq), x.pts, sizeof(float4) * x.n, hipMemcpyHostToDevice));
   return edit_seq(c, c->d_meta.get() + seq, [&](SeqMeta& m) { m.n_corner_last = n_corner; m.n_surf_last = n_surf; });
 }
@@ -420,11 +436,12 @@
   DeviceScope device_scope(c);
   int rc = check_seq(c, seq);
   if (rc) return rc;
-  if (!c->d_grid_flags[0]) { c->err = "this context has no odometry stage"; return ALOAM_E_STATE; }
-  HIP_TRY(c, hipStreamSynchronize(c->stream));
+  if (!c->d_grid_flags[0][0]) { c->err = "this context has no odometry stage"; return ALOAM_E_STATE; }
+  HIP_TRY(c, hipStreamSynchronize(c->stream));
+  const int set = c->parity[seq];
   for (int k = 0; k < 2; ++k) {
     int f[4];
-    HIP_TRY(c, hipMemcpy(f, c->d_grid_flags[k].get() + (size_t)seq * 4, sizeof(f), hipMemcpyDeviceToHost));
+    HIP_TRY(c, hipMemcpy(f, c->d_grid_flags[set][k].get() + (size_t)seq * 4, sizeof(f), hipMemcpyDeviceToHost));
     out[k] = f[0] ? -1 : f[1];
   }
   return ALOAM_OK;
diff --git a/a-loam_amd/csrc/mapping_kernels.hip b/a-loam_amd/csrc/mapping_kernels.hip
--- a/a-loam_amd/csrc/mapping_kernels.hip
+++ b/a-loam_amd/csrc/mapping_kernels.hip
@@ -1370,7 +1370,7 @@
   if (r.edges) {
     for (int i = tid; i < r.R * kSharpPerRing; i += 256) r.edges[(long long)b * r.R * kSharpPerRing + i] = EdgeRec{};
     for (int i = tid; i < r.R * kFlatPerRing; i += 256) r.planes[(long long)b * r.R * kFlatPerRing + i] = PlaneRec{};
-    if (tid < 8) r.grid_flags[tid >> 2][b * 4 + (tid & 3)] = 0;
+    if (tid < 16) r.grid_flags[tid >> 3][(tid >> 2) & 1][b * 4 + (tid & 3)] = 0;
   }
   if (r.mapseq) {
     for (int i = tid; i < 2 * kMapCubes; i += 256) {
diff --git a/a-loam_amd/csrc/mapping_kernels.hpp b/a-loam_amd/csrc/mapping_kernels.hpp
--- a/a-loam_amd/csrc/mapping_kernels.hpp
+++ b/a-loam_amd/csrc/mapping_kernels.hpp
@@ -130,7 +130,7 @@
   SeqMeta* meta; int* ringstart;
   OdomState* state;
   EdgeRec* edges; PlaneRec* planes;
-  int* grid_flags[2];
+  int* grid_flags[2][2];
   float4* less_sharp[2]; float4* less_flat[2]; int cap;
   MapSeq* mapseq; CubeDesc* cubes; int* addcnt; int* live;
   MapGridSig* grid_sig;
diff --git a/a-loam_amd/csrc/odometry_kernels.hip b/a-loam_amd/csrc/odometry_kernels.hip
--- a/a-loam_amd/csrc/odometry_kernels.hip
+++ b/a-loam_amd/csrc/odometry_kernels.hip
@@ -129,14 +129,27 @@
 }
 __host__ __device__ __forceinline__ bool fused_takes(int n, int H) { return n <= kFusedMaxN && H <= kFusedMaxH; }
 
-__global__ __launch_bounds__(1024) void k_build_grids_fused(OdomArgs a) {
+template <bool NEXT>
+struct BuildSrc {
+  int n, set;
+  const float4* pts;
+  __device__ __forceinline__ BuildSrc(const OdomArgs& a, const SeqMeta& m, int b, int which) {
+    set = NEXT ? m.parity : m.parity ^ 1;
+    n = which == 0 ? (NEXT ? m.n_less_sharp : m.n_corner_last) : (NEXT ? m.n_less_flat : m.n_surf_last);
+    pts = which == 0 ? row_of(a.less_sharp, set, b, (long long)a.R * kLessSharpPerRing) : row_of(a.less_flat, set, b, (long long)a.cap);
+  }
+};
+
+template <bool NEXT>
+__device__ __forceinline__ void build_grids_fused(const OdomArgs& a, int b, int which) {
   constexpr int U = 4;
-  const int b = blockIdx.y, which = blockIdx.x, tid = threadIdx.x, lane = tid & 63, wave = tid >> 6;
-  if (seq_idle(a.active, b, kSeqSolve)) return;
+  const int tid = threadIdx.x, lane = tid & 63, wave = tid >> 6;
+  if (seq_idle(a.active, b, NEXT ? kSeqActive : kSeqSolve)) return;
   const SeqMeta m = a.meta[b];
-  const int n = which == 0 ? m.n_corner_last : m.n_surf_last;
-  const float4* pts = which == 0 ? corner_last(a, b, m.parity) : surf_last(a, b, m.parity);
-  const GridView g = grid_view(a, b, which);
+  const BuildSrc<NEXT> src(a, m, b, which);
+  const int n = src.n;
+  const float4* pts = src.pts;
+  const GridView g = grid_view(a, b, which, src.set);
   const int H = g.H;
   if (!fused_takes(n, H)) return;
   extern __shared__ __attribute__((aligned(16))) int lds[];
@@ -252,17 +265,28 @@
 #endif
 }
 
+__global__ __launch_bounds__(1024) void k_build_grids_fused(OdomArgs a) { build_grids_fused<false>(a, blockIdx.y, blockIdx.x); }
+__global__ __launch_bounds__(1024) void k_build_grids_fused_next(OdomArgs a) {
+  const int G = gridDim.x;
+  for (int r = 0, i = blockIdx.x; i < 2 * a.B; ++r, i += G) {
+    build_grids_fused<true>(a, i >> 1, (i ^ r) & 1);
+    __syncthreads();
+  }
+}
+
 constexpr int kBgWaves = 4;
 constexpr int kBgUnroll = 4;
-__global__ __launch_bounds__(1024, kBgWaves) void k_build_grids(OdomArgs a) {
+template <bool NEXT>
+__device__ __forceinline__ void build_grids(const OdomArgs& a) {
   constexpr int U = kBgUnroll;
   const int b = blockIdx.y, which = blockIdx.x / 3, tid = threadIdx.x;
   const int pass_lo = blockIdx.x % 3, pass_hi = pass_lo + 1;
-  if (seq_idle(a.active, b, kSeqSolve)) return;
+  if (seq_idle(a.active, b, NEXT ? kSeqActive : kSeqSolve)) return;
   const SeqMeta m = a.meta[b];
-  const int n = which == 0 ? m.n_corner_last : m.n_surf_last;
-  const float4* pts = which == 0 ? corner_last(a, b, m.parity) : surf_last(a, b, m.parity);
-  const GridView g = grid_view(a, b, which);
+  const BuildSrc<NEXT> src(a, m, b, which);
+  const int n = src.n;
+  const float4* pts = src.pts;
+  const GridView g = grid_view(a, b, which, src.set);
   if (fused_takes(n, g.H)) return;
   extern __shared__ __attribute__((aligned(16))) int lds[];
   int* cnt = lds;
@@ -357,6 +381,9 @@
     }
   }
 }
+
+__global__ __launch_bounds__(1024, kBgWaves) void k_build_grids(OdomArgs a) { build_grids<false>(a); }
+__global__ __launch_bounds__(1024, kBgWaves) void k_build_grids_next(OdomArgs a) { build_grids<true>(a); }
 
 __device__ __forceinline__ float walk_dist(const float4& p, const float4& sel) {
   return (p.x - sel.x) * (p.x - sel.x) + (p.y - sel.y) * (p.y - sel.y) + (p.z - sel.z) * (p.z - sel.z);
@@ -1095,7 +1122,7 @@
   const SeqMeta m = a.meta[b];
   const int nq = PLANE ? m.n_flat : m.n_sharp;
   if (qi0 >= nq) return;
-  const GridView g = grid_view(a, b, PLANE ? 1 : 0);
+  const GridView g = grid_view(a, b, PLANE ? 1 : 0, m.parity ^ 1);
   const int nt = PLANE ? m.n_surf_last : m.n_corner_last;
   if (g.flags[0] != 0 || g.flags[1] != 0 || nt <= 0) return;
   associate_pair<PLANE, kRows, !WIDE, false>(a, b, qi0, nq, nt, g, lane, lds);
@@ -1108,9 +1135,9 @@
   __shared__ int lds[sweep2_lds_ints<kRows>()];
   const int lane = threadIdx.x, b = blockIdx.y;
   if (seq_idle(a.active, b, kSeqSolve)) return;
-  const GridView g = grid_view(a, b, PLANE ? 1 : 0);
+  const SeqMeta m = a.meta[b];
+  const GridView g = grid_view(a, b, PLANE ? 1 : 0, m.parity ^ 1);
   if (g.flags[0] != 0 || g.flags[1] != 1) return;
-  const SeqMeta m = a.meta[b];
   const int nq = PLANE ? m.n_flat : m.n_sharp, nt = PLANE ? m.n_surf_last : m.n_corner_last;
   if (nt <= 0) return;
   for (int k = 0; k < kPairsPerWave; ++k) {
@@ -1127,7 +1154,7 @@
   const int b = blockIdx.x, lane = threadIdx.x & 63, wave = threadIdx.x >> 6;
   if (seq_idle(a.active, b, kSeqSolve)) return;
   const SeqMeta m = a.meta[b];
-  const GridView g = grid_view(a, b, PLANE ? 1 : 0);
+  const GridView g = grid_view(a, b, PLANE ? 1 : 0, m.parity ^ 1);
   const int nt = PLANE ? m.n_surf_last : m.n_corner_last;
   if (!(g.flags[0] != 0 || g.flags[1] == 2 || nt <= 0)) return;
   const int nq = PLANE ? m.n_flat : m.n_sharp;
@@ -1275,13 +1302,23 @@
 size_t build_grids_lds_bytes(int H, int R) { return sizeof(int) * ((size_t)H + 1024 + 2 * (R + 8) + 4); }
 static size_t build_grids_fused_lds_bytes(int H) { return sizeof(int) * (3 * (size_t)(H / 2) + 48 + 8 + 2 * kWalkKeys); }
 int prepare_build_grids(int H_surf) {
-  if (hipFuncSetAttribute((const void*)k_build_grids_fused, hipFuncAttributeMaxDynamicSharedMemorySize, (int)build_grids_fused_lds_bytes(kFusedMaxH)) != hipSuccess) return -1;
-  return hipFuncSetAttribute((const void*)k_build_grids, hipFuncAttributeMaxDynamicSharedMemorySize, (int)build_grids_lds_bytes(H_surf, kMaxRings)) == hipSuccess ? 0 : -1;
-}
-void launch_build_grids(const OdomArgs& a, hipStream_t s) {
+  const int fused = (int)build_grids_fused_lds_bytes(kFusedMaxH), per_grid = (int)build_grids_lds_bytes(H_surf, kMaxRings);
+  if (hipFuncSetAttribute((const void*)k_build_grids_fused, hipFuncAttributeMaxDynamicSharedMemorySize, fused) != hipSuccess) return -1;
+  if (hipFuncSetAttribute((const void*)k_build_grids_fused_next, hipFuncAttributeMaxDynamicSharedMemorySize, fused) != hipSuccess) return -1;
+  if (hipFuncSetAttribute((const void*)k_build_grids, hipFuncAttributeMaxDynamicSharedMemorySize, per_grid) != hipSuccess) return -1;
+  return hipFuncSetAttribute((const void*)k_build_grids_next, hipFuncAttributeMaxDynamicSharedMemorySize, per_grid) == hipSuccess ? 0 : -1;
+}
+void launch_build_grids(const OdomArgs& a, bool next, int cus, hipStream_t s) {
   const int hc = a.grid_H_corner <= kFusedMaxH ? a.grid_H_corner : 0, hs = a.grid_H_surf <= kFusedMaxH ? a.grid_H_surf : 0;
-  if (hc || hs) hipLaunchKernelGGL(k_build_grids_fused, dim3(2, a.B), dim3(1024), build_grids_fused_lds_bytes(hc > hs ? hc : hs), s, a);
-  hipLaunchKernelGGL(k_build_grids, dim3(6, a.B), dim3(1024), build_grids_lds_bytes(a.grid_H_surf, a.R), s, a);
+  const size_t fused = build_grids_fused_lds_bytes(hc > hs ? hc : hs), per_grid = build_grids_lds_bytes(a.grid_H_surf, a.R);
+  if (next) {
+    const int wgs = cus / 2 >= 2 ? (cus / 2) & ~1 : 2;
+    if (hc || hs) hipLaunchKernelGGL(k_build_grids_fused_next, dim3(2 * a.B < wgs ? 2 * a.B : wgs), dim3(1024), fused, s, a);
+    hipLaunchKernelGGL(k_build_grids_next, dim3(6, a.B), dim3(1024), per_grid, s, a);
+  } else {
+    if (hc || hs) hipLaunchKernelGGL(k_build_grids_fused, dim3(2, a.B), dim3(1024), fused, s, a);
+    hipLaunchKernelGGL(k_build_grids, dim3(6, a.B), dim3(1024), per_grid, s, a);
+  }
 }
 void launch_transform_queries(const OdomArgs& a, hipStream_t s) {
   const dim3 grid((a.R * (kSharpPerRing + kFlatPerRing) + 255) / 256, a.B);
diff --git a/a-loam_amd/csrc/odometry_kernels.hpp b/a-loam_amd/csrc/odometry_kernels.hpp
--- a/a-loam_amd/csrc/odometry_kernels.hpp
+++ b/a-loam_amd/csrc/odometry_kernels.hpp
@@ -4,7 +4,7 @@
 namespace aloam {
 size_t build_grids_lds_bytes(int H, int R);
 int prepare_build_grids(int H_surf);
-void launch_build_grids(const OdomArgs& a, hipStream_t s);
+void launch_build_grids(const OdomArgs& a, bool next, int cus, hipStream_t s);
 void launch_transform_queries(const OdomArgs& a, hipStream_t s);
 void launch_associate(const OdomArgs& a, bool plane, hipStream_t s);
 void launch_solve(const OdomArgs& a, hipStream_t s);
```

Measured after the change: 130,500 (median of 6 runs). 5.8% higher.
